# Wx-Alliance-Alliance-Meteo/paradis_model

Measured on AMD Instinct MI355X. Metric: training samples/sec (whole node) on 5.625° ERA5 grid, 1/2/4/8 MI355X, higher is better.
Workload: dtype f32; 1 GPU; era5_5.625deg_32x64_S1_B32; grid=32x64, rollout_steps=1, per_gpu_batch=32, global_batch=32, parameters=60038475, optimizer=adamw, parallelism=dp1, gemm_arithmetic=bf16x3, mode=train, hip_graph=False, activation_checkpointing=False

## Files before the change

include/paradis_hip.h:

```cpp
#ifndef PARADIS_HIP_H
#define PARADIS_HIP_H

#include <stddef.h>
#include <stdint.h>

#ifdef __cplusplus
extern "C" {
#endif

#define PARADIS_ACT_NONE 0
#define PARADIS_ACT_SILU 1
#define PARADIS_ACT_GELU 2
#define PARADIS_INTERP_BILINEAR 1
#define PARADIS_INTERP_BICUBIC 2
#define PARADIS_ADVECT_AUTO 0
#define PARADIS_ADVECT_GENERIC 1
#define PARADIS_ADVECT_TILED 2
#define PARADIS_ADVECT_SEPARABLE 4
#define PARADIS_ADVECT_TILES 8
#define PARADIS_ADVECT_STRIPS 16
#define PARADIS_ADVECT_HALO_SHIFT 8
#define PARADIS_ADVECT_HALO_BWD_SHIFT 16
#define PARADIS_ADVECT_HALO(h) (((h) + 1) << PARADIS_ADVECT_HALO_SHIFT)

int paradis_abi_version(void);
const char* paradis_last_error(void);

int paradis_geocyclic_pad_fwd(const float* x, float* y, int64_t planes, int H, int W, int p, void* stream);
int paradis_geocyclic_pad_bwd(const float* gy, float* gx, int64_t planes, int H, int W, int p, void* stream);

int paradis_sl_advect_fwd(const float* field, const float* u, const float* v, float* out,
                          const float* sin_lat, const float* cos_lat, const float* lat_cells, const float* lon,
                          int B, int K, int H, int W, int64_t f_bs, int64_t uv_bs, int64_t o_bs,
                          float dt, float min_lat, float min_lon, float d_lat, float d_lon,
                          int mode, int flags, void* workspace, void* stream);
size_t paradis_sl_advect_ws_bytes(int B, int K, int H, int W, int flags);
int paradis_sl_advect_bwd(const float* gout, const float* field, const float* u, const float* v,
                          float* gfield, float* gu, float* gv,
                          const float* sin_lat, const float* cos_lat, const float* lat_cells, const float* lon,
                          int B, int K, int H, int W, int64_t go_bs, int64_t f_bs, int64_t uv_bs,
                          int64_t gf_bs, int64_t guv_bs,
                          float dt, float min_lat, float min_lon, float d_lat, float d_lon,
                          int mode, int flags, void* workspace, void* stream);

int paradis_dwconv_geo_fwd(const float* x, const float* w, const float* bias, float* y,
                           int B, int C, int H, int W, int k, void* stream);
int paradis_dwconv_geo_dgrad(const float* gy, const float* w, float* gx,
                             int B, int C, int H, int W, int k, void* stream);
int paradis_dwconv_geo_dgrad_add(const float* gy, const float* w, const float* addend, float* gx,
                                 int B, int C, int H, int W, int k, void* stream);
int paradis_dwconv_geo_bwd(const float* gy, const float* x, const float* w, const float* addend, float* gx,
                           float* gw, float* gbias, int B, int C, int H, int W, int k, void* workspace, void* stream);
size_t paradis_dwconv_geo_wgrad_ws_bytes(int B, int C, int H, int W, int k);
int paradis_dwconv_geo_wgrad(const float* gy, const float* x, float* gw, float* gbias,
                             int B, int C, int H, int W, int k, void* workspace, void* stream);

int paradis_avgpool_geo_fwd(const float* x, float* y, int64_t planes, int H, int W, int stride, void* stream);
int paradis_avgpool_geo_bwd(const float* gy, float* gx, int64_t planes, int H, int W, int stride, void* stream);

int paradis_upsample_lonp_fwd(const float* x, float* y, int64_t planes, int Hc, int Wc, int H, int W, void* stream);
int paradis_upsample_lonp_bwd(const float* gy, float* gx, int64_t planes, int Hc, int Wc, int H, int W, void* stream);

#define PARADIS_GEMM_EXACT 0
#define PARADIS_GEMM_BF16 1
#define PARADIS_GEMM_F16X2 2
#define PARADIS_GEMM_BF16X3 3
#define PARADIS_AMAX_PARTIALS 1024
int paradis_amax_partials(const float* x, int B, int64_t inner, int64_t bs, uint32_t* partials, void* stream);
size_t paradis_pw_gemm_split_bytes(int M, int K, int scheme);
int paradis_pw_gemm_split_weights(const float* W, int M, int K, int transpose, int scheme, void* out, void* stream);
int paradis_pw_gemm_split_weights_pair(const float* W, int M, int K, void* out, void* out_t, void* stream);
int paradis_pw_gemm_split_weights_pair_scheme(const float* W, int M, int K, int scheme, void* out, void* out_t, void* stream);
int paradis_pw_gemm_fwd(const float* Wt, const float* WtT ,
                        const void* Wsplit ,
                        int scheme, const uint32_t* x_amax ,
                        const float* X, const float* bias, const float* map,
                        const float* m8 , const float* pwT , int cin,
                        const float* res, float* Y, float* zpre,
                        int B, int M, int K, int N, int64_t x_bs, int64_t res_bs, int64_t y_bs,
                        int act, void* stream);
int paradis_pw_gemm_fwd_gated(const float* Wt, const float* WtT, const void* Wsplit, int scheme, const uint32_t* x_amax,
                              const float* X, const float* bias, const float* map, const float* m8, const float* pwT,
                              int cin, const float* res, const float* gate, float* Y, float* zpre,
                              int B, int M, int K, int N, int64_t x_bs, int64_t res_bs, int64_t y_bs,
                              int act, void* stream);
int paradis_pw_gemm_dgrad(const float* Wt, const void* WTsplit, int scheme,
                          const uint32_t* dy_amax ,
                          const float* dY, const float* zpre,
                          const float* addend, float* dX, int B, int M, int K, int N, int64_t dy_bs,
                          int64_t z_bs, int64_t add_bs, int64_t dx_bs, int act, void* stream);
size_t paradis_pw_gemm_wgrad_ws_bytes(int B, int M, int K, int N);
int paradis_pw_gemm_wgrad_slabs(int B, int M, int K, int N);
int paradis_pw_gemm_wgrad(const float* dY, const float* X, float* dW, float* gbias,
                          int B, int M, int K, int N, int64_t dy_bs, int64_t x_bs, int scheme,
                          const uint32_t* dy_amax, const uint32_t* x_amax ,
                          void* workspace, void* stream);

#define PARADIS_IO_X16 1
#define PARADIS_IO_Y16 2
#define PARADIS_IO_Z16 4
#define PARADIS_IO_DY16 8
int paradis_pw_gemm_fwd16(const void* Wsplit, const void* X, const float* bias, const float* map, const float* m8,
                          const float* pwT, int cin, const float* res, const float* gate , void* Y,
                          void* zpre, int B, int M, int K, int N, int64_t x_bs, int64_t res_bs, int64_t y_bs, int act,
                          int io16, void* stream);
int paradis_pw_gemm_dgrad16(const void* WTsplit, const void* dY, const void* zpre, void* dX, int B, int M, int K, int N,
                            int64_t dy_bs, int64_t z_bs, int64_t dx_bs, int act, int io16, void* stream);
int paradis_pw_gemm_wgrad16(const void* dY, const void* X, float* dW, float* gbias, int B, int M, int K, int N,
                            int64_t dy_bs, int64_t x_bs, int io16, void* workspace, void* stream);
int paradis_channel_norm_fwd16(const float* x1, const float* x2, const float* w, const float* b, void* y ,
                               float* mean, float* rstd, int B, int C1, int C2, int P, int64_t x1_bs, int64_t x2_bs,
                               float eps, void* stream);
int paradis_dwconv_geo_fwd16(const float* x, const float* w, const float* bias, void* y , int B, int C, int H,
                             int W, int k, void* stream);
int paradis_channel_norm_bwd16_ok(int B, int C, int P);
int paradis_channel_norm_bwd16(const void* gy , const float* x1, const float* x2, const float* w, const float* mean,
                               const float* rstd, float* gx1, float* gx2, float* gw, float* gb, int B, int C1, int C2, int P,
                               int64_t x1_bs, int64_t x2_bs, int64_t gx1_bs, int64_t gx2_bs, const float* addend1,
                               int64_t add1_bs, void* workspace, void* stream);
int paradis_dwconv_geo_bwd16_ok(int H, int W, int k);
int paradis_dwconv_geo_bwd16(const void* gy , const float* x, const float* w, const float* addend, float* gx, float* gw,
                             float* gbias, int B, int C, int H, int W, int k, void* workspace, void* stream);
int paradis_act_bwd16(const float* gy, const float* x, void* gx , int64_t n, int act, void* stream);
int paradis_bias_grads16(const void* dz, float* gmap, float* gbias, int B, int C, int P, int64_t dz_bs, void* stream);

int paradis_channel_norm_fwd(const float* x1, const float* x2, const float* w, const float* b,
                             float* y, float* mean, float* rstd,
                             int B, int C1, int C2, int P, int64_t x1_bs, int64_t x2_bs,
                             float eps, void* stream);
size_t paradis_channel_norm_bwd_ws_bytes(int B, int C, int P);
int paradis_channel_norm_bwd(const float* gy, const float* x1, const float* x2, const float* w,
                             const float* mean, const float* rstd, float* gx1, float* gx2,
                             float* gw, float* gb, int B, int C1, int C2, int P,
                             int64_t x1_bs, int64_t x2_bs, int64_t gx1_bs, int64_t gx2_bs,
                             const float* addend1, int64_t add1_bs, void* workspace, void* stream);

int paradis_global_bias_map_fwd(const float* A, const float* U, const float* V, const float* Pw,
                                float* m8, float* map, int Cin, int Co, int R, int H, int W, void* stream);
size_t paradis_global_bias_map_bwd_ws_bytes(int Cin, int Co, int R, int H, int W);
int paradis_global_bias_map_bwd(const float* gmap, const float* A, const float* U, const float* V,
                                const float* Pw, const float* m8, float* gA, float* gU, float* gV,
                                float* gPw, int Cin, int Co, int R, int H, int W,
                                void* workspace, void* stream);

int paradis_global_bias_m8_fwd(const float* A, const float* U, const float* V, float* m8,
                               int Cin, int R, int H, int W, void* stream);
int paradis_global_bias_m8_bwd(const float* gm8, const float* A, const float* U, const float* V,
                               float* gA, float* gU, float* gV, int Cin, int R, int H, int W,
                               void* workspace, void* stream);
int paradis_global_bias_proj_bwd(const float* gmap, const float* m8, const float* Pw, float* gPw,
                                 float* gm8, int Cin, int Co, int64_t P, void* stream);

int paradis_act_fwd(const float* x, float* y, int64_t n, int act, void* stream);
int paradis_act_bwd(const float* gy, const float* x, float* gx, int64_t n, int act, void* stream);
int paradis_gated_blend_fwd(const float* h, const float* adv, const float* alpha, float* out,
                            int B, int C, int P, void* stream);
size_t paradis_gated_blend_bwd_ws_bytes(int B, int C, int P);
int paradis_gated_blend_bwd(const float* gout, const float* h, const float* adv, const float* alpha,
                            float* gh, float* gadv, float* galpha, int B, int C, int P,
                            void* workspace, void* stream);
int paradis_gated_blend_bwd_out(const float* gout, const float* h, const float* out, const float* alpha,
                                float* gh, float* gadv, float* galpha, int B, int C, int P,
                                void* workspace, void* stream);
int paradis_bias_grads(const float* dz, float* gmap, float* gbias, int B, int C, int P,
                       int64_t dz_bs, void* stream);
int paradis_add(const float* a, const float* b, float* y, int64_t n, void* stream);
int paradis_transpose(const float* in, float* out, int rows, int cols, void* stream);
int paradis_add_bcast(const float* x, const float* m, float* y, int64_t per_sample, int B, void* stream);

int paradis_loss_blocks(int64_t total);
int paradis_loss_fwd_bwd(const float* pred, const float* target, const float* wf, const float* wl,
                         float* loss, float* grad, float* partial, int B, int C, int H, int W,
                         int kind, float delta, void* stream);
int paradis_scale(const float* x, const float* scalar, float* y, int64_t n, void* stream);
int paradis_copy_channels(const float* src, int64_t src_bs, float* dst, int64_t dst_bs, int B,
                          int64_t per_sample, void* stream);
int paradis_adamw_step(float* p, const float* g, float* m, float* v, int64_t n, float lr, float beta1,
                       float beta2, float eps, float weight_decay, int step, void* stream);
int paradis_adamw_chunk(void);
int paradis_adamw_multi(const int64_t* ptrs, const int64_t* numel, const int* chunk_tensor,
                        const int64_t* chunk_off, int n_tensors, int n_chunks, float lr, float beta1,
                        float beta2, float eps, float weight_decay, int step, const int* dev_state, void* stream);
int paradis_adamw_tick(int* dev_state, void* stream);
int paradis_adamw_step_d(float* p, const float* g, float* m, float* v, int64_t n, double lr, double beta1,
                         double beta2, double eps, double weight_decay, int step, void* stream);
int paradis_adamw_multi_d(const int64_t* ptrs, const int64_t* numel, const int* chunk_tensor,
                          const int64_t* chunk_off, int n_tensors, int n_chunks, double lr, double beta1,
                          double beta2, double eps, double weight_decay, int step, const int* dev_state, void* stream);

size_t paradis_amse_table_floats(int H);
size_t paradis_amse_tables_ws_bytes(int H);
int paradis_amse_tables(float* leg, float* twiddle, double* ws, int H, int W, void* stream);
size_t paradis_amse_ws_bytes(int N, int H);
int paradis_amse_loss(const float* pred, const float* target, const float* leg, const float* twiddle, float* loss,
                      float* grad, void* ws, int N, int H, int W, void* stream);

size_t paradis_muon_ws_bytes(int T, int rows, int cols);
int paradis_muon_step(const int64_t* ptrs, int table_stride, int T, int rows, int cols, float lr,
                      float lr_adj, float mu, float beta2, float weight_decay, float eps, int nesterov,
                      int normuon, int split ,
                      void* workspace, void* stream);
int paradis_bgemm(const float* A, const float* AT, const float* B, float* C, int nbatch, int M, int K, int N,
                  int64_t a_bs, int64_t at_bs, int64_t b_bs, int64_t c_bs, void* split_ws, void* stream);

size_t paradis_forcings_ws_bytes(int B, int T);
int paradis_forcings(const int64_t* times_us , const double* lat_deg, const double* lon_deg,
                     int lat_is_f32, int B, int T, int H, int W, int n_time_inputs, const int* var_codes, int n_vars,
                     double toa_mean, double toa_std, float* out, void* workspace, void* stream);
int paradis_normalize_features(float* data, const int* kind, const float* p0, const float* p1,
                               int64_t rows, int C, float eps_q, int inverse, void* stream);

int paradis_forecast_post(const float* output, int64_t out_bs, float* chunk, int64_t chunk_bs, int64_t chunk_off,
                          float* dew, int64_t dew_bs, int64_t dew_off, const int* kind, const float* p0,
                          const float* p1, float eps_q, const int* units, int n_units, const double* plev,
                          int n_levels, const double* trig, int B, int C, int H, int W, void* stream);

size_t paradis_val_score_ws_bytes(int B, int C, int H, int W);
int paradis_val_score(const float* pred, int64_t pred_bs, const float* target, int64_t target_bs, const float* wf,
                      const float* wl, const float* lat_w, int kind, float delta, const int* rep_chan,
                      const int* rep_class, int R, const int* rflag, const int* rcls, const float* rp0,
                      const float* rp1, const int* rchan, float* out, void* workspace, int B, int C, int H, int W,
                      void* stream);

#ifdef __cplusplus
}
#endif
#endif
```

paradis_model_amd/_lib.py:

```python
from __future__ import annotations

import ctypes
import os
from ctypes import c_char_p, c_double, c_float, c_int, c_int64, c_size_t, c_void_p

import torch

_HERE = os.path.dirname(os.path.abspath(__file__))
LIB_PATH = os.environ.get("PARADIS_HIP_LIB") or os.path.join(_HERE, "libparadis_hip.so")

if not os.path.exists(LIB_PATH):
    raise ImportError(
        f"{LIB_PATH} not found: the HIP extension is not built. Run "
        "`python -c 'import __graft_entry__ as g; g.build()'` (or `make -C paradis_model_amd/csrc`). "
        "paradis_model_amd has no CPU/eager fallback by design.")

lib = ctypes.CDLL(LIB_PATH)

P, I, L, F, S, D = c_void_p, c_int, c_int64, c_float, c_size_t, c_double

SIGNATURES = {
    "paradis_abi_version": (I, []),
    "paradis_last_error": (c_char_p, []),
    "paradis_geocyclic_pad_fwd": (I, [P, P, L, I, I, I, P]),
    "paradis_geocyclic_pad_bwd": (I, [P, P, L, I, I, I, P]),
    "paradis_sl_advect_fwd": (I, [P, P, P, P, P, P, P, P, I, I, I, I, L, L, L, F, F, F, F, F, I, I, P, P]),
    "paradis_sl_advect_ws_bytes": (S, [I, I, I, I, I]),
    "paradis_sl_advect_bwd": (I, [P, P, P, P, P, P, P, P, P, P, P, I, I, I, I, L, L, L, L, L,
                                  F, F, F, F, F, I, I, P, P]),
    "paradis_dwconv_geo_fwd": (I, [P, P, P, P, I, I, I, I, I, P]),
    "paradis_dwconv_geo_dgrad": (I, [P, P, P, I, I, I, I, I, P]),
    "paradis_dwconv_geo_dgrad_add": (I, [P, P, P, P, I, I, I, I, I, P]),
    "paradis_dwconv_geo_bwd": (I, [P, P, P, P, P, P, P, I, I, I, I, I, P, P]),
    "paradis_dwconv_geo_wgrad_ws_bytes": (S, [I, I, I, I, I]),
    "paradis_dwconv_geo_wgrad": (I, [P, P, P, P, I, I, I, I, I, P, P]),
    "paradis_avgpool_geo_fwd": (I, [P, P, L, I, I, I, P]),
    "paradis_avgpool_geo_bwd": (I, [P, P, L, I, I, I, P]),
    "paradis_upsample_lonp_fwd": (I, [P, P, L, I, I, I, I, P]),
    "paradis_upsample_lonp_bwd": (I, [P, P, L, I, I, I, I, P]),
    "paradis_amax_partials": (I, [P, I, L, L, P, P]),
    "paradis_pw_gemm_split_bytes": (S, [I, I, I]),
    "paradis_pw_gemm_split_weights": (I, [P, I, I, I, I, P, P]),
    "paradis_pw_gemm_split_weights_pair": (I, [P, I, I, P, P, P]),
    "paradis_pw_gemm_split_weights_pair_scheme": (I, [P, I, I, I, P, P, P]),
    "paradis_pw_gemm_fwd": (I, [P, P, P, I, P, P, P, P, P, P, I, P, P, P, I, I, I, I, L, L, L, I, P]),
    "paradis_pw_gemm_fwd_gated": (I, [P, P, P, I, P, P, P, P, P, P, I, P, P, P, P, I, I, I, I, L, L, L, I, P]),
    "paradis_forcings_ws_bytes": (ctypes.c_size_t, [I, I]),
    "paradis_forcings": (I, [P, P, P, I, I, I, I, I, I, P, I, ctypes.c_double, ctypes.c_double, P, P, P]),
    "paradis_normalize_features": (I, [P, P, P, P, L, I, ctypes.c_float, I, P]),
    "paradis_global_bias_m8_fwd": (I, [P, P, P, P, I, I, I, I, P]),
    "paradis_global_bias_m8_bwd": (I, [P, P, P, P, P, P, P, I, I, I, I, P, P]),
    "paradis_global_bias_proj_bwd": (I, [P, P, P, P, P, I, I, L, P]),
    "paradis_transpose": (I, [P, P, I, I, P]),
    "paradis_pw_gemm_dgrad": (I, [P, P, I, P, P, P, P, P, I, I, I, I, L, L, L, L, I, P]),
    "paradis_pw_gemm_wgrad_ws_bytes": (S, [I, I, I, I]),
    "paradis_pw_gemm_wgrad_slabs": (I, [I, I, I, I]),
    "paradis_pw_gemm_wgrad": (I, [P, P, P, P, I, I, I, I, L, L, I, P, P, P, P]),
    "paradis_pw_gemm_fwd16": (I, [P, P, P, P, P, P, I, P, P, P, P, I, I, I, I, L, L, L, I, I, P]),
    "paradis_pw_gemm_dgrad16": (I, [P, P, P, P, I, I, I, I, L, L, L, I, I, P]),
    "paradis_pw_gemm_wgrad16": (I, [P, P, P, P, I, I, I, I, L, L, I, P, P]),
    "paradis_bias_grads16": (I, [P, P, P, I, I, I, L, P]),
    "paradis_channel_norm_fwd16": (I, [P, P, P, P, P, P, P, I, I, I, I, L, L, F, P]),
    "paradis_dwconv_geo_fwd16": (I, [P, P, P, P, I, I, I, I, I, P]),
    "paradis_channel_norm_bwd16_ok": (I, [I, I, I]),
    "paradis_channel_norm_bwd16": (I, [P, P, P, P, P, P, P, P, P, P, I, I, I, I, L, L, L, L, P, L, P, P]),
    "paradis_dwconv_geo_bwd16_ok": (I, [I, I, I]),
    "paradis_dwconv_geo_bwd16": (I, [P, P, P, P, P, P, P, I, I, I, I, I, P, P]),
    "paradis_channel_norm_fwd": (I, [P, P, P, P, P, P, P, I, I, I, I, L, L, F, P]),
    "paradis_channel_norm_bwd_ws_bytes": (S, [I, I, I]),
    "paradis_channel_norm_bwd": (I, [P, P, P, P, P, P, P, P, P, P, I, I, I, I, L, L, L, L, P, L, P, P]),
    "paradis_global_bias_map_fwd": (I, [P, P, P, P, P, P, I, I, I, I, I, P]),
    "paradis_global_bias_map_bwd_ws_bytes": (S, [I, I, I, I, I]),
    "paradis_global_bias_map_bwd": (I, [P, P, P, P, P, P, P, P, P, P, I, I, I, I, I, P, P]),
    "paradis_act_fwd": (I, [P, P, L, I, P]),
    "paradis_act_bwd": (I, [P, P, P, L, I, P]),
    "paradis_act_bwd16": (I, [P, P, P, L, I, P]),
    "paradis_gated_blend_fwd": (I, [P, P, P, P, I, I, I, P]),
    "paradis_gated_blend_bwd_ws_bytes": (S, [I, I, I]),
    "paradis_gated_blend_bwd": (I, [P, P, P, P, P, P, P, I, I, I, P, P]),
    "paradis_gated_blend_bwd_out": (I, [P, P, P, P, P, P, P, I, I, I, P, P]),
    "paradis_bias_grads": (I, [P, P, P, I, I, I, L, P]),
    "paradis_add": (I, [P, P, P, L, P]),
    "paradis_add_bcast": (I, [P, P, P, L, I, P]),
    "paradis_loss_blocks": (I, [L]),
    "paradis_loss_fwd_bwd": (I, [P, P, P, P, P, P, P, I, I, I, I, I, F, P]),
    "paradis_scale": (I, [P, P, P, L, P]),
    "paradis_copy_channels": (I, [P, L, P, L, I, L, P]),
    "paradis_adamw_step": (I, [P, P, P, P, L, F, F, F, F, F, I, P]),
    "paradis_muon_ws_bytes": (S, [I, I, I]),
    "paradis_muon_step": (I, [P, I, I, I, I, F, F, F, F, F, F, I, I, I, P, P]),
    "paradis_bgemm": (I, [P, P, P, P, I, I, I, I, L, L, L, L, P, P]),
    "paradis_adamw_chunk": (I, []),
    "paradis_adamw_multi": (I, [P, P, P, P, I, I, F, F, F, F, F, I, P, P]),
    "paradis_adamw_tick": (I, [P, P]),
    "paradis_adamw_step_d": (I, [P, P, P, P, L, D, D, D, D, D, I, P]),
    "paradis_adamw_multi_d": (I, [P, P, P, P, I, I, D, D, D, D, D, I, P, P]),
    "paradis_amse_table_floats": (S, [I]),
    "paradis_amse_tables_ws_bytes": (S, [I]),
    "paradis_amse_tables": (I, [P, P, P, I, I, P]),
    "paradis_amse_ws_bytes": (S, [I, I]),
    "paradis_amse_loss": (I, [P, P, P, P, P, P, P, I, I, I, P]),
    "paradis_forecast_post": (I, [P, L, P, L, L, P, L, L, P, P, P, F, P, I, P, I, P, I, I, I, I, P]),
    "paradis_val_score_ws_bytes": (S, [I, I, I, I]),
    "paradis_val_score": (I, [P, L, P, L, P, P, P, I, F, P, P, I, P, P, P, P, P, P, P, I, I, I, I, P]),
}

_missing = []
for _name, (_res, _args) in SIGNATURES.items():
    try:
        _fn = getattr(lib, _name)
    except AttributeError:
        _missing.append(_name)
        continue
    _fn.restype = _res
    _fn.argtypes = _args
if _missing and os.environ.get("PARADIS_DEV_PARTIAL") != "1":
    raise ImportError(f"{LIB_PATH} lacks symbols {_missing}; rebuild the HIP extension")


def last_error() -> str:
    msg = lib.paradis_last_error()
    return msg.decode() if msg else ""


def check(rc: int, name: str) -> None:
    if rc != 0:
        raise RuntimeError(f"{name} failed (code {rc}): {last_error()}")


def dptr(t):
    if t is None:
        return None
    return ctypes.c_void_p(t.data_ptr())


_raw_stream = getattr(torch._C, "_cuda_getCurrentRawStream", None)


def stream_ptr():
    if _raw_stream is not None:
        return ctypes.c_void_p(_raw_stream(torch.cuda.current_device()))
    return ctypes.c_void_p(torch.cuda.current_stream().cuda_stream)


def require_hip(*tensors, any_dtype: bool = False) -> None:
    for t in tensors:
        if t is None:
            continue
        if not t.is_cuda:
            raise RuntimeError("paradis_model_amd ops run on the MI355X only: got a CPU tensor "
                               "(there is no CPU fallback; use oracle/ for CPU checks)")
        if t.dtype != torch.float32 and not any_dtype:
            raise RuntimeError(f"paradis_model_amd ops are fp32; got {t.dtype}")


class LaunchProfiler:

    def __init__(self):
        self.records = {}

    def add(self, name, work, ev0, ev1):
        rec = self.records.setdefault(name, [0.0, []])
        rec[0] += work
        rec[1].append((ev0, ev1))

    def summary(self):
        out = {}
        for name, (work, evs) in self.records.items():
            ms = sum(a.elapsed_time(b) for a, b in evs)
            out[name] = {"launches": len(evs), "work": work, "ms": ms}
        return out


PROFILER = None


def call(name: str, work: float, *args, symbol: str = None) -> None:
    fn = getattr(lib, "paradis_" + (symbol or name))
    prof = PROFILER
    if prof is None:
        check(fn(*args), name)
        return
    ev0 = torch.cuda.Event(enable_timing=True)
    ev1 = torch.cuda.Event(enable_timing=True)
    ev0.record()
    rc = fn(*args)
    ev1.record()
    check(rc, name)
    prof.add(name, work, ev0, ev1)
```

paradis_model_amd/csrc/gemm.hip:

```cpp
#include <algorithm>
#include <cstdlib>
#include "gemm_common.h"


namespace {

constexpr int ld_of(bool kc) { return kc ? BM + 1 : BM + 4; }
constexpr int stage_floats(int bk) { return bk * (BM + 4); }
constexpr size_t lds_bytes(int bk) { return (size_t)4 * stage_floats(bk) * sizeof(float); }
constexpr int nv_of(int bk) { return BM * bk / (256 * 4); }

int g_bk = 16;
int g_wg_per_cu = 4;
int g_stagger = 0;
int g_dma_stages = 3;
int g_wgrad_dma_stages = 2;


template <bool KC, int BK>
__device__ __forceinline__ void slab_load(const float* __restrict__ base, int64_t ld, int row0,
                                          int k0, int rows, int K, bool vec_ok,
                                          float4 (&r)[nv_of(BK)]) {
  constexpr int NV = nv_of(BK);
  constexpr int TPR = BK / 4;
// ... 208 lines not shown
    float a0 = As[0], a1 = As[32], b0 = Bs[0], b1 = Bs[32];
#pragma unroll
    for (int kk = 0; kk < DBK / 2; ++kk) {
      float na0 = 0.f, na1 = 0.f, nb0 = 0.f, nb1 = 0.f;
      if (kk + 1 < DBK / 2) {
        na0 = As[(2 * kk + 2) * BM]; na1 = As[(2 * kk + 2) * BM + 32];
        nb0 = Bs[(2 * kk + 2) * BN]; nb1 = Bs[(2 * kk + 2) * BN + 32];
      }
      acc[0][0] = __builtin_amdgcn_mfma_f32_32x32x2f32(a0, b0, acc[0][0], 0, 0, 0);
      acc[0][1] = __builtin_amdgcn_mfma_f32_32x32x2f32(a0, b1, acc[0][1], 0, 0, 0);
      acc[1][0] = __builtin_amdgcn_mfma_f32_32x32x2f32(a1, b0, acc[1][0], 0, 0, 0);
      acc[1][1] = __builtin_amdgcn_mfma_f32_32x32x2f32(a1, b1, acc[1][1], 0, 0, 0);
      a0 = na0; a1 = na1; b0 = nb0; b1 = nb1;
    }
  }
  gemm_epilogue(g, acc, bz, m0, n0, wm, wn, li, lh);
}

template <int S>
__global__ void __launch_bounds__(256, 4)
pw_gemm_wgrad_dma_kernel(GemmArgs g) {
  extern __shared__ __attribute__((aligned(16))) float lds[];
  const int tid = threadIdx.x, lane = tid & 63, wave = tid >> 6;
  const int wm = wave >> 1, wn = wave & 1;
  const int li = lane & 31, lh = lane >> 5;

  const int MT = (g.M + BM - 1) / BM, NT = (g.N + BN - 1) / BN;
  int L;
  {
    const int nwg = gridDim.x, id = blockIdx.x;
    const int q = nwg >> 3, r = nwg & 7, xcd = id & 7;
    L = (xcd < r ? xcd * (q + 1) : r * (q + 1) + (xcd - r) * q) + (id >> 3);
  }
  const int mt = L % MT, nt = (L / MT) % NT, bz = L / (MT * NT);
  const int m0 = mt * BM, n0 = nt * BN;
  const int KT = g.K / DBK;
  const int64_t total = (int64_t)g.inner * KT;
  const int t_begin = (int)(total * bz / g.nbatch);
  const int T = (int)(total * (bz + 1) / g.nbatch) - t_begin;

  const int prow = lane >> 2, pslot = lane & 3;
  const int chunk = pslot ^ ((prow >> 2) & 3);
  const int ra0 = min(m0 + 16 * (2 * wave) + prow, g.M - 1), ra1 = min(m0 + 16 * (2 * wave + 1) + prow, g.M - 1);
  const int rb0 = min(n0 + 16 * (2 * wave) + prow, g.N - 1), rb1 = min(n0 + 16 * (2 * wave + 1) + prow, g.N - 1);
  const float* pa0 = g.A + (int64_t)ra0 * g.lda + 4 * chunk;
  const float* pa1 = g.A + (int64_t)ra1 * g.lda + 4 * chunk;
  const float* pb0 = g.B + (int64_t)rb0 * g.ldb + 4 * chunk;
  const float* pb1 = g.B + (int64_t)rb1 * g.ldb + 4 * chunk;

  auto issue = [&](int t) {
    const int tt = t_begin + t;
    const int ib = tt / KT, kt = tt - ib * KT;
    const int64_t oa = (int64_t)ib * g.a_is + (int64_t)kt * DBK, ob = (int64_t)ib * g.b_is + (int64_t)kt * DBK;
    float* st = lds + (t % S) * (2 * DTILE);
    float* la = st + (2 * wave) * 256;
    float* lb = st + DTILE + (2 * wave) * 256;
    __builtin_amdgcn_global_load_lds((gbl_ptr_t)(pa0 + oa), (lds_ptr_t)la, 16, 0, 0);
    __builtin_amdgcn_global_load_lds((gbl_ptr_t)(pa1 + oa), (lds_ptr_t)(la + 256), 16, 0, 0);
    __builtin_amdgcn_global_load_lds((gbl_ptr_t)(pb0 + ob), (lds_ptr_t)lb, 16, 0, 0);
    __builtin_amdgcn_global_load_lds((gbl_ptr_t)(pb1 + ob), (lds_ptr_t)(lb + 256), 16, 0, 0);
  };

  f32x16 acc[2][2];
#pragma unroll
  for (int i = 0; i < 2; ++i)
#pragma unroll
    for (int j = 0; j < 2; ++j)
#pragma unroll
      for (int r = 0; r < 16; ++r) acc[i][j][r] = 0.f;

#pragma unroll
  for (int t = 0; t < S - 1; ++t)
    if (t < T) issue(t);

  const bool do_rowsum = g.rowsum != nullptr && nt == 0;
  float rs = 0.f;
  const int rs_off = (tid >> 1) * DBK + (tid & 1) * 8;

  const int sw = (li >> 2) & 3;
  const int offA = (wm * 64 + li) * DBK, offB = DTILE + (wn * 64 + li) * DBK;
  const int s0 = ((0 + lh) ^ sw) * 4, s1 = ((2 + lh) ^ sw) * 4;

  for (int t = 0; t < T; ++t) {
    const int pending = min(S - 2, T - 1 - t);
    if (pending >= 2) asm volatile("s_waitcnt vmcnt(8)\n\ts_barrier" ::: "memory");
    else if (pending == 1) asm volatile("s_waitcnt vmcnt(4)\n\ts_barrier" ::: "memory");
    else asm volatile("s_waitcnt vmcnt(0)\n\ts_barrier" ::: "memory");
    if (t + S - 1 < T) issue(t + S - 1);
    const float* st = lds + (t % S) * (2 * DTILE);
    if (do_rowsum) {
      const float4 q0 = *reinterpret_cast<const float4*>(st + rs_off);
      const float4 q1 = *reinterpret_cast<const float4*>(st + rs_off + 4);
      rs += ((q0.x + q0.y) + (q0.z + q0.w)) + ((q1.x + q1.y) + (q1.z + q1.w));
    }
    const float4 a00 = *reinterpret_cast<const float4*>(st + offA + s0);
    const float4 a10 = *reinterpret_cast<const float4*>(st + offA + 32 * DBK + s0);
    const float4 b00 = *reinterpret_cast<const float4*>(st + offB + s0);
    const float4 b10 = *reinterpret_cast<const float4*>(st + offB + 32 * DBK + s0);
    const float4 a01 = *reinterpret_cast<const float4*>(st + offA + s1);
    const float4 a11 = *reinterpret_cast<const float4*>(st + offA + 32 * DBK + s1);
    const float4 b01 = *reinterpret_cast<const float4*>(st + offB + s1);
    const float4 b11 = *reinterpret_cast<const float4*>(st + offB + 32 * DBK + s1);
#define MFMA4(A0, A1, B0, B1)                                                       \
    acc[0][0] = __builtin_amdgcn_mfma_f32_32x32x2f32(A0, B0, acc[0][0], 0, 0, 0);   \
    acc[0][1] = __builtin_amdgcn_mfma_f32_32x32x2f32(A0, B1, acc[0][1], 0, 0, 0);   \
    acc[1][0] = __builtin_amdgcn_mfma_f32_32x32x2f32(A1, B0, acc[1][0], 0, 0, 0);   \
    acc[1][1] = __builtin_amdgcn_mfma_f32_32x32x2f32(A1, B1, acc[1][1], 0, 0, 0);
    MFMA4(a00.x, a10.x, b00.x, b10.x)
    MFMA4(a00.y, a10.y, b00.y, b10.y)
    MFMA4(a00.z, a10.z, b00.z, b10.z)
    MFMA4(a00.w, a10.w, b00.w, b10.w)
    MFMA4(a01.x, a11.x, b01.x, b11.x)
    MFMA4(a01.y, a11.y, b01.y, b11.y)
    MFMA4(a01.z, a11.z, b01.z, b11.z)
    MFMA4(a01.w, a11.w, b01.w, b11.w)
#undef MFMA4
  }
  if (do_rowsum) {
    rs += __shfl_xor(rs, 1, 64);
    const int m = m0 + (tid >> 1);
    if ((tid & 1) == 0 && m < g.M) g.rowsum[(int64_t)bz * g.M + m] = rs;
  }
  gemm_epilogue(g, acc, bz, m0, n0, wm, wn, li, lh);
}

constexpr int SIMG = simg(3);

__global__ void __launch_bounds__(256)
amax_partials_kernel(const float* __restrict__ x, int B, int64_t inner, int64_t bs, int vec, uint32_t* __restrict__ out) {
  uint32_t m = 0;
  if (vec) {
    const int64_t n4 = inner >> 2, total = n4 * B;
    for (int64_t i = (int64_t)blockIdx.x * 256 + threadIdx.x; i < total; i += (int64_t)gridDim.x * 256) {
      const int64_t b = i / n4, j = i - b * n4;
      const uint4 q = *reinterpret_cast<const uint4*>(x + b * bs + 4 * j);
      m = max(max(m, q.x & 0x7fffffffu), max(q.y & 0x7fffffffu, max(q.z & 0x7fffffffu, q.w & 0x7fffffffu)));
    }
  } else {
    const int64_t total = inner * B;
    for (int64_t i = (int64_t)blockIdx.x * 256 + threadIdx.x; i < total; i += (int64_t)gridDim.x * 256) {
      const int64_t b = i / inner, j = i - b * inner;
      m = max(m, __float_as_uint(x[b * bs + j]) & 0x7fffffffu);
    }
  }
  m = wave_umax_lane63(m);
  __shared__ uint32_t red[4];
  if ((threadIdx.x & 63) == 63) red[threadIdx.x >> 6] = m;
  __syncthreads();
  if (threadIdx.x == 0) out[blockIdx.x] = max(max(red[0], red[1]), max(red[2], red[3]));
}


template <int NP = 3>
__device__ __forceinline__ void split_weights_body(const float* __restrict__ Wb, int64_t rs, int64_t cs, int M, int K,
                                                   int KT, int64_t units, u32x4* __restrict__ ob) {
  for (int64_t u = (int64_t)blockIdx.x * 256 + threadIdx.x; u < units; u += (int64_t)gridDim.x * 256) {
    const int row = (int)(u & 127), half = (int)((u >> 7) & 1);
    const int64_t tile = u >> 8;
    const int kt = (int)(tile % KT), mt = (int)(tile / KT);
    const int m = mt * BM + row;
    float x[8];
#pragma unroll
    for (int j = 0; j < 8; ++j) {
      const int k = kt * SBK + half * 8 + j;
      x[j] = (m < M && k < K) ? Wb[(int64_t)m * rs + (int64_t)k * cs] : 0.f;
      if (SPLIT_SIGNED && (row & 32)) x[j] = -x[j];
    }
    if constexpr (NP == 3) {
      u32x4 h, mm, l;
      split8(x, h, mm, l);
      u32x4* o = ob + tile * SIMG + half * SCH + row;
      o[0] = h; o[2 * SCH] = mm; o[4 * SCH] = l;
    } else {
      ob[tile * simg(1) + half * SCH + row] = round8(x);
    }
  }
}

template <int NP>
__global__ void __launch_bounds__(256)
split_weights_kernel(const float* __restrict__ W, int64_t rs, int64_t cs, int M, int K, int KT, int64_t units,
                     int64_t w_bs, int64_t out_bs, u32x4* __restrict__ out) {
  split_weights_body<NP>(W + (int64_t)blockIdx.y * w_bs, rs, cs, M, K, KT, units, out + (int64_t)blockIdx.y * out_bs);
}

template <int NP>
__global__ void __launch_bounds__(256)
split_weights_pair_kernel(const float* __restrict__ W, int M, int K, int KT, int KTt, int64_t units, int64_t units_t,
                          u32x4* __restrict__ out, u32x4* __restrict__ out_t) {
  if (blockIdx.y == 0) split_weights_body<NP>(W, K, 1, M, K, KT, units, out);
  else split_weights_body<NP>(W, 1, K, K, M, KTt, units_t, out_t);
}

__global__ void __launch_bounds__(256)
split_weights_f16_kernel(const float* __restrict__ W, int64_t rs, int64_t cs, int M, int K, int KT, int64_t units,
                         u32x4* __restrict__ out, uint32_t* __restrict__ tail) {
  const uint32_t amax = reduce_amax_partials(tail + 4);
  if (blockIdx.x == 0 && threadIdx.x == 0) tail[0] = amax;
  float sc, inv;
  scale_from_amax(amax, sc, inv);
  for (int64_t u = (int64_t)blockIdx.x * 256 + threadIdx.x; u < units; u += (int64_t)gridDim.x * 256) {
    const int row = (int)(u & 127), half = (int)((u >> 7) & 1);
    const int64_t tile = u >> 8;
    const int kt = (int)(tile % KT), mt = (int)(tile / KT);
    const int m = mt * BM + row;
    float x[8];
#pragma unroll
    for (int j = 0; j < 8; ++j) {
      const int k = kt * SBK + half * 8 + j;
      x[j] = (m < M && k < K) ? W[(int64_t)m * rs + (int64_t)k * cs] : 0.f;
    }
    u32x4 h, l;
    split8_f16(x, (SPLIT_SIGNED && (row & 32)) ? -sc : sc, h, l);
    u32x4* o = out + tile * simg(2) + half * SCH + row;
    o[0] = h; o[2 * SCH] = l;
  }
}

#ifndef SPLIT_ASTAGES_F16
#define SPLIT_ASTAGES_F16 2
#endif
constexpr int split_astages(int np) { return np == 2 ? SPLIT_ASTAGES_F16 : 2; }
template <int NP>
__global__ void __launch_bounds__(256, 3)
pw_gemm_split_kernel(GemmArgs g) {
  extern __shared__ __attribute__((aligned(16))) float lds[];
  constexpr int SIMG = simg(NP);
  u32x4* img = reinterpret_cast<u32x4*>(lds);
  constexpr int SA = split_astages(NP), DA = SA - 1;
  const int tid = threadIdx.x, lane = tid & 63, wave = tid >> 6;
  const int wm = wave >> 1, wn = wave & 1;
  const int li = lane & 31, lh = lane >> 5;

  const int MT = (g.M + BM - 1) / BM, NT = (g.N + BN - 1) / BN;
  int L;
  {
    const int nwg = gridDim.x, id = blockIdx.x;
    const int q = nwg >> 3, r = nwg & 7, xcd = id & 7;
    L = (xcd < r ? xcd * (q + 1) : r * (q + 1) + (xcd - r) * q) + (id >> 3);
  }
  const int mt = L % MT, nt = (L / MT) % NT, bz = L / (MT * NT);
  const int m0 = mt * BM, n0 = nt * BN;
  const int T = (g.K + SBK - 1) / SBK;

  const u32x4* Ag = reinterpret_cast<const u32x4*>(g.A) + (int64_t)bz * g.a_bs + (int64_t)mt * T * SIMG + tid;
  const int bh = __builtin_amdgcn_readfirstlane(tid >> 7);
  const float* Bb;
  {
    const uint64_t a = reinterpret_cast<uint64_t>(g.B + (int64_t)bz * g.b_bs);
    const uint32_t lo = __builtin_amdgcn_readfirstlane((uint32_t)a), hi = __builtin_amdgcn_readfirstlane((uint32_t)(a >> 32));
    Bb = reinterpret_cast<const float*>(((uint64_t)hi << 32) | lo);
  }
  const int bn = min(n0 + (tid & 127), g.N - 1);

  float sc_b = 1.f, inv_a = 1.f, inv_b = 1.f;
  if constexpr (NP == 2) {
    float sc_a;
    scale_from_amax(reduce_amax_partials(g.b_amax), sc_b, inv_b);
    scale_from_amax(g.a_amax[0], sc_a, inv_a);
  }

  const uint32_t flip = split_flip_mask(tid & 127);
  if constexpr (NP == 2) sc_b = __uint_as_float(__float_as_uint(sc_b) ^ flip);
  float xb[2][8] = {};
  auto issueA = [&](int t) __attribute__((always_inline)) {
    const u32x4* a = Ag + (int64_t)t * SIMG;
    u32x4* la = img + (2 + t % SA) * SIMG + wave * 64;
#pragma unroll
    for (int i = 0; i < NP; ++i)
      __builtin_amdgcn_global_load_lds((gbl_ptr_t)(a + i * 256), (lds_ptr_t)(la + i * 256), 16, 0, 0);
  };
  auto split_store = [&](const float (&x)[8], u32x4* o) __attribute__((always_inline)) {
    if constexpr (NP == 3) {
      u32x4 h, m, l;
      float xs[8];
      flip8(xs, x, flip);
      split8(xs, h, m, l);
      o[0] = h; o[2 * SCH] = m; o[4 * SCH] = l;
    } else {
      u32x4 h, l;
      split8_f16(x, sc_b, h, l);
      o[0] = h; o[2 * SCH] = l;
    }
  };
  const uint32_t boff = (uint32_t)bn * 4u;
  auto fetchB = [&](int t, float (&x)[8]) __attribute__((always_inline)) {
    const int k0 = t * SBK + bh * 8;
    const float* p = Bb + (int64_t)min(k0, g.K - 1) * g.ldb;
#pragma unroll
    for (int j = 0; j < 8; ++j) {
      asm volatile("global_load_dword %0, %1, %2" : "=&v"(x[j]) : "v"(boff), "s"(p) : "memory");
      p += (k0 + j + 1 < g.K) ? g.ldb : 0;
    }
  };
#define USE_X(x, N) do { asm volatile("s_waitcnt vmcnt(" #N ")" :: "v"(x[0]), "v"(x[1]), "v"(x[2]), "v"(x[3]), \
                                      "v"(x[4]), "v"(x[5]), "v"(x[6]), "v"(x[7]) : "memory");                  \
                         __builtin_amdgcn_sched_barrier(0); } while (0)
  u32x4* const Bst = img + bh * SCH + (tid & 127);

  f32x16 acc[2][2];
#pragma unroll
  for (int i = 0; i < 2; ++i)
#pragma unroll
    for (int j = 0; j < 2; ++j)
#pragma unroll
      for (int r = 0; r < 16; ++r) acc[i][j][r] = 0.f;

  for (int u = 0; u < DA && u < T; ++u) issueA(u);
  fetchB(0, xb[0]);
  USE_X(xb[0], 0);
  if (T > 1) fetchB(1, xb[1]);
  split_store(xb[0], Bst);
  if (T > 1) asm volatile("s_waitcnt vmcnt(8) lgkmcnt(0)\n\ts_barrier" ::: "memory");
  else asm volatile("s_waitcnt vmcnt(0) lgkmcnt(0)\n\ts_barrier" ::: "memory");
  auto step = [&](int t, int cur, float (&xload)[8], float (&xsplit)[8]) __attribute__((always_inline)) {
    const u32x4* As = img + (2 + t % SA) * SIMG + lh * SCH + wm * 64 + li;
    const u32x4* Bs = img + cur * SIMG + lh * SCH + wn * 64 + li;
    const bool dmaA = t + DA < T, ldB = t + 2 < T;
    if (dmaA) issueA(t + DA);
    if (ldB) fetchB(t + 2, xload);
    if (dmaA && ldB) { if constexpr (NP == 3) USE_X(xsplit, 11); else USE_X(xsplit, 10); }
    else if (ldB) USE_X(xsplit, 8);
    else USE_X(xsplit, 0);
    SplitFrags<NP> f;
    split_tile_read<NP, 2 * SCH, 2 * SCH>(As, Bs, f);
    split_tile_mfma<NP>(f, acc);
    split_store(xsplit, Bst + (cur ^ 1) * SIMG);
    __builtin_amdgcn_sched_group_barrier(0x100, 4 * NP, 0);
#pragma unroll
// ... 293 lines not shown
  return 0;
}

template <bool A_KC, bool B_KC>
int launch_gemm(const GemmArgs& g, int grid, hipStream_t st) {
  return g_bk == 32 ? launch_gemm_bk<A_KC, B_KC, 32>(g, grid, st)
                    : launch_gemm_bk<A_KC, B_KC, 16>(g, grid, st);
}

constexpr size_t split_lds(int np) { return (size_t)(2 + split_astages(np)) * simg(np) * 16; }
constexpr size_t split_lds_wgrad(int np) { return (size_t)2 * 2 * simgp(np) * 16; }
constexpr int AMAX_WORDS = PARADIS_AMAX_PARTIALS;
constexpr size_t F16_TAIL_BYTES = 16 + (size_t)AMAX_WORDS * 4;

int split_image_ktiles(int K, int np) {
  const int kt = (K + SBK - 1) / SBK;
  return np == 1 ? (kt + 1) & ~1 : kt;
}
int64_t split_image_chunks(int M, int K, int np = 3) {
  return (int64_t)((M + BM - 1) / BM) * split_image_ktiles(K, np) * simg(np);
}

bool known_scheme(int scheme) {
  return scheme == PARADIS_GEMM_EXACT || scheme == PARADIS_GEMM_BF16X3 || scheme == PARADIS_GEMM_F16X2 ||
         scheme == PARADIS_GEMM_BF16;
}

int launch_amax(const float* x, int B, int64_t inner, int64_t bs, uint32_t* out, hipStream_t st) {
  const int vec = (inner % 4 == 0) && (bs % 4 == 0) && ((reinterpret_cast<uintptr_t>(x) & 15) == 0);
  hipLaunchKernelGGL(amax_partials_kernel, dim3(AMAX_WORDS), dim3(256), 0, st, x, B, inner, bs, vec, out);
  return 0;
}

template <int NP>
int launch_split_np(const GemmArgs& d, hipStream_t st) {
  const int grid = ((d.M + BM - 1) / BM) * ((d.N + BN - 1) / BN) * d.nbatch;
  static PerDeviceOnce once;
  if (split_lds(NP) > 64 * 1024)
    if (int e = reserve_lds(once, {&pw_gemm_split_kernel<NP>}, split_lds(NP), "pw_gemm(split)")) return e;
  hipLaunchKernelGGL(pw_gemm_split_kernel<NP>, dim3(grid), dim3(256), split_lds(NP), st, d);
  return 0;
}
constexpr size_t split_wide_lds(int nsub, int np = 2) { return (size_t)(2 * nsub + 2) * simg(np) * 16; }
constexpr int SPLIT_WIDE_NSUB = 2;
#ifndef SPLIT_WIDE_BF16X3
#define SPLIT_WIDE_BF16X3 1
#endif
template <int NP>
int launch_split_wide(const GemmArgs& d, int NT, hipStream_t st) {
  constexpr int NSUB = SPLIT_WIDE_NSUB;
  static PerDeviceOnce once;
  if (split_wide_lds(NSUB, NP) > 64 * 1024)
    if (int e = reserve_lds(once, {&pw_gemm_split_wide_kernel<NSUB, NP>}, split_wide_lds(NSUB, NP), "pw_gemm(split)")) return e;
  const int grid = ((d.M + BM - 1) / BM) * ((NT + NSUB - 1) / NSUB) * d.nbatch;
  hipLaunchKernelGGL((pw_gemm_split_wide_kernel<NSUB, NP>), dim3(grid), dim3(256 * NSUB), split_wide_lds(NSUB, NP), st, d);
  return 0;
}
int launch_split(const GemmArgs& d, int scheme, hipStream_t st) {
  const int NT = (d.N + BN - 1) / BN;
  if (scheme == PARADIS_GEMM_BF16) return pd_amp_launch_fwd(d, st);
  if (scheme != PARADIS_GEMM_F16X2) {
#if SPLIT_WIDE_BF16X3
    if (NT >= 2) return launch_split_wide<3>(d, NT, st);
#endif
    return launch_split_np<3>(d, st);
  }
  if (NT < 2) return launch_split_np<2>(d, st);
  return launch_split_wide<2>(d, NT, st);
}

int check_gemm(const char* name, int B, int M, int K, int N) {
  PD_REQUIRE(B >= 0 && M >= 1 && K >= 1 && N >= 1, "%s: bad shape B=%d M=%d K=%d N=%d", name, B, M, K, N);
  const int64_t tiles = (int64_t)((M + BM - 1) / BM) * ((N + BN - 1) / BN) * std::max(B, 1);
  PD_REQUIRE(tiles < (1ll << 31), "%s: too many tiles", name);
  return 0;
}

}

#ifdef PARADIS_DEV_KNOBS
extern "C" void paradis_debug_set_gemm(int bk, int wg_per_cu) {
  if (bk == 16 || bk == 32) g_bk = bk;
  if (wg_per_cu >= 1 && wg_per_cu <= 4) g_wg_per_cu = wg_per_cu;
}
extern "C" void paradis_debug_set_gemm_stagger(int units) { g_stagger = units < 0 ? 0 : units; }
extern "C" void paradis_debug_set_gemm_dma(int stages) { g_dma_stages = stages < 2 ? 0 : (stages > 4 ? 4 : stages); }
extern "C" void paradis_debug_set_wgrad_dma(int stages) { g_wgrad_dma_stages = stages < 2 ? 0 : (stages > 3 ? 3 : stages); }
#endif

extern "C" size_t paradis_pw_gemm_split_bytes(int M, int K, int scheme) {
  if (M < 1 || K < 1) return 0;
  if (scheme == PARADIS_GEMM_F16X2) return (size_t)split_image_chunks(M, K, 2) * 16 + F16_TAIL_BYTES;
  if (scheme == PARADIS_GEMM_BF16) return (size_t)split_image_chunks(M, K, 1) * 16;
  return scheme == PARADIS_GEMM_BF16X3 ? (size_t)split_image_chunks(M, K, 3) * 16 : 0;
}

extern "C" int paradis_amax_partials(const float* x, int B, int64_t inner, int64_t bs, uint32_t* partials,
                                     void* stream) {
  PD_REQUIRE(partials != nullptr && B >= 0 && inner >= 0 && (x != nullptr || B == 0 || inner == 0),
             "amax_partials: bad arguments");
  launch_amax(x, B, inner, bs, partials, (hipStream_t)stream);
  PD_CHECK_LAUNCH("amax_partials");
  return 0;
}

extern "C" int paradis_pw_gemm_split_weights(const float* W, int M, int K, int transpose, int scheme, void* out,
                                             void* stream) {
  PD_REQUIRE(W != nullptr && out != nullptr && M >= 1 && K >= 1, "pw_gemm_split_weights: bad arguments");
  PD_REQUIRE(scheme == PARADIS_GEMM_BF16X3 || scheme == PARADIS_GEMM_F16X2 || scheme == PARADIS_GEMM_BF16,
             "pw_gemm_split_weights: unknown scheme %d", scheme);
  const int AM = transpose ? K : M, AK = transpose ? M : K;
  const int KT = split_image_ktiles(AK, scheme == PARADIS_GEMM_BF16 ? 1 : 3);
  const int64_t units = (int64_t)((AM + BM - 1) / BM) * KT * 256;
  const int blocks = (int)std::min<int64_t>((units + 255) / 256, 4096);
  if (scheme == PARADIS_GEMM_F16X2) {
    uint32_t* tail = reinterpret_cast<uint32_t*>((char*)out + (size_t)split_image_chunks(AM, AK, 2) * 16);
    launch_amax(W, 1, (int64_t)M * K, 0, tail + 4, (hipStream_t)stream);
    hipLaunchKernelGGL(split_weights_f16_kernel, dim3(blocks), dim3(256), 0, (hipStream_t)stream, W,
                       (int64_t)(transpose ? 1 : K), (int64_t)(transpose ? K : 1), AM, AK, KT, units, (u32x4*)out, tail);
  } else if (scheme == PARADIS_GEMM_BF16) {
    hipLaunchKernelGGL(split_weights_kernel<1>, dim3(blocks, 1), dim3(256), 0, (hipStream_t)stream, W,
                       (int64_t)(transpose ? 1 : K), (int64_t)(transpose ? K : 1), AM, AK, KT, units,
                       (int64_t)0, (int64_t)0, (u32x4*)out);
  } else {
    hipLaunchKernelGGL(split_weights_kernel<3>, dim3(blocks, 1), dim3(256), 0, (hipStream_t)stream, W,
                       (int64_t)(transpose ? 1 : K), (int64_t)(transpose ? K : 1), AM, AK, KT, units,
                       (int64_t)0, (int64_t)0, (u32x4*)out);
  }
  PD_CHECK_LAUNCH("pw_gemm_split_weights");
  return 0;
}

extern "C" int paradis_pw_gemm_split_weights_pair_scheme(const float* W, int M, int K, int scheme, void* out, void* out_t,
                                                         void* stream) {
  PD_REQUIRE(W != nullptr && out != nullptr && out_t != nullptr && out != out_t && M >= 1 && K >= 1,
             "pw_gemm_split_weights_pair: bad arguments");
  PD_REQUIRE(scheme == PARADIS_GEMM_BF16X3 || scheme == PARADIS_GEMM_BF16,
             "pw_gemm_split_weights_pair: scheme %d has no paired images", scheme);
  const int np = scheme == PARADIS_GEMM_BF16 ? 1 : 3;
  const int KT = split_image_ktiles(K, np), KTt = split_image_ktiles(M, np);
  const int64_t units = (int64_t)((M + BM - 1) / BM) * KT * 256, units_t = (int64_t)((K + BM - 1) / BM) * KTt * 256;
  const int blocks = (int)std::min<int64_t>((std::max(units, units_t) + 255) / 256, 4096);
  if (scheme == PARADIS_GEMM_BF16X3)
    hipLaunchKernelGGL(split_weights_pair_kernel<3>, dim3(blocks, 2), dim3(256), 0, (hipStream_t)stream, W, M, K, KT, KTt,
                       units, units_t, (u32x4*)out, (u32x4*)out_t);
  else
    hipLaunchKernelGGL(split_weights_pair_kernel<1>, dim3(blocks, 2), dim3(256), 0, (hipStream_t)stream, W, M, K, KT, KTt,
                       units, units_t, (u32x4*)out, (u32x4*)out_t);
  PD_CHECK_LAUNCH("pw_gemm_split_weights_pair");
  return 0;
}
extern "C" int paradis_pw_gemm_split_weights_pair(const float* W, int M, int K, void* out, void* out_t, void* stream) {
  return paradis_pw_gemm_split_weights_pair_scheme(W, M, K, PARADIS_GEMM_BF16X3, out, out_t, stream);
}

namespace {
int run_split(GemmArgs d, const void* img, int AM, int AK, int scheme, const uint32_t* b_amax, const char* what,
              hipStream_t st) {
  d.A = (const float*)img; d.a_bs = 0;
  if (scheme == PARADIS_GEMM_F16X2) {
    if (b_amax == nullptr) { paradis_set_error(what); return 1; }
    d.a_amax = reinterpret_cast<const uint32_t*>((const char*)img + (size_t)split_image_chunks(AM, AK, 2) * 16);
    d.b_amax = b_amax;
  }
  return launch_split(d, scheme, st);
}
int check_io16(const char* name, int io16, int scheme, const void* Bop, int64_t b_bs, int N, bool has_res) {
  if (io16 == 0) return 0;
  PD_REQUIRE(scheme == PARADIS_GEMM_BF16, "%s: bf16-stored tensors need the PARADIS_GEMM_BF16 scheme", name);
  PD_REQUIRE((io16 & ~(IO_B16 | IO_C16 | IO_ZM16 | IO_A16)) == 0, "%s: unknown io16 bits %d", name, io16);
  PD_REQUIRE(!(io16 & IO_C16) || !has_res, "%s: a bf16 output cannot carry the fp32 residual", name);
  if (io16 & IO_B16)
    PD_REQUIRE(N % 8 == 0 && N >= 8 && b_bs % 8 == 0 && (reinterpret_cast<uintptr_t>(Bop) & 15) == 0,
               "%s: a bf16 activation operand needs N %% 8 == 0 and 16-byte aligned planes", name);
  return 0;
}
}

static int pw_gemm_fwd_impl(const float* Wt, const float* WtT, const void* Wsplit, int scheme,
                            const uint32_t* x_amax, const float* X,
                            const float* bias, const float* map, const float* m8,
                            const float* pwT, int cin, const float* res, const float* gate, float* Y, float* zpre,
                            int B, int M, int K, int N, int64_t x_bs, int64_t res_bs,
                            int64_t y_bs, int act, void* stream, int io16 = 0) {
  if (int e = check_gemm("pw_gemm_fwd", B, M, K, N)) return e;
  if (int e = check_io16("pw_gemm_fwd", io16, scheme, X, x_bs, N, res != nullptr)) return e;
  PD_REQUIRE(gate == nullptr || res != nullptr || B == 0, "pw_gemm_fwd: a gate needs the tensor it blends with (res)");
  PD_REQUIRE(act >= 0 && act <= 2, "pw_gemm_fwd: unknown activation code %d", act);
  PD_REQUIRE(known_scheme(scheme) && (Wsplit != nullptr) == (scheme != PARADIS_GEMM_EXACT),
             "pw_gemm_fwd: scheme %d needs %s weight image", scheme, scheme ? "a" : "no");
  PD_REQUIRE((m8 == nullptr) == (pwT == nullptr) && (pwT == nullptr || (cin >= 1 && M % 4 == 0)),
             "pw_gemm_fwd: projected bias needs m8, pwT, cin >= 1 and M %% 4 == 0");
  if (B == 0) return 0;
  GemmArgs g{};
  g.m8 = m8; g.pw = pwT; g.cin = cin;
  g.A = Wt; g.B = X; g.C = Y; g.M = M; g.N = N; g.K = K;
  g.lda = K; g.ldb = N; g.ldc = N;
  g.a_bs = 0; g.b_bs = x_bs; g.c_bs = y_bs; g.nbatch = B; g.inner = 0;
  g.bias = bias; g.map = map; g.res = res; g.res_bs = res_bs; g.zmul = nullptr; g.zout = zpre;
  g.zout_bs = (int64_t)M * N; g.act = act; g.gate = gate;
  g.stagger = g_stagger;
  g.io16 = io16;
  const int grid = ((M + BM - 1) / BM) * ((N + BN - 1) / BN) * B;
  if (Wsplit != nullptr) {
    if (int e = run_split(g, Wsplit, M, K, scheme, x_amax, "pw_gemm_fwd: the f16x2 scheme needs x_amax",
                          (hipStream_t)stream)) return e;
    PD_CHECK_LAUNCH("pw_gemm_fwd(split)");
    return 0;
  }
  if (WtT != nullptr) {
    GemmArgs d = g;
    d.A = WtT; d.lda = M;
    if (dma_eligible(d)) {
      launch_gemm_dma(d, grid, (hipStream_t)stream);
      PD_CHECK_LAUNCH("pw_gemm_fwd(dma)");
      return 0;
    }
  }
  if (int e = launch_gemm<true, false>(g, grid, (hipStream_t)stream)) return e;
  PD_CHECK_LAUNCH("pw_gemm_fwd");
  return 0;
}

extern "C" int paradis_pw_gemm_fwd(const float* Wt, const float* WtT, const void* Wsplit, int scheme,
                                   const uint32_t* x_amax, const float* X,
                                   const float* bias, const float* map, const float* m8,
                                   const float* pwT, int cin, const float* res, float* Y, float* zpre,
                                   int B, int M, int K, int N, int64_t x_bs, int64_t res_bs,
                                   int64_t y_bs, int act, void* stream) {
  return pw_gemm_fwd_impl(Wt, WtT, Wsplit, scheme, x_amax, X, bias, map, m8, pwT, cin, res, nullptr, Y, zpre, B, M, K, N,
                          x_bs, res_bs, y_bs, act, stream);
}

extern "C" int paradis_pw_gemm_fwd_gated(const float* Wt, const float* WtT, const void* Wsplit, int scheme,
                                         const uint32_t* x_amax, const float* X,
                                         const float* bias, const float* map, const float* m8,
                                         const float* pwT, int cin, const float* res, const float* gate, float* Y,
                                         float* zpre, int B, int M, int K, int N, int64_t x_bs, int64_t res_bs,
                                         int64_t y_bs, int act, void* stream) {
  PD_REQUIRE(gate != nullptr && (res != nullptr || B == 0), "pw_gemm_fwd_gated: gate [M] and res required");
  return pw_gemm_fwd_impl(Wt, WtT, Wsplit, scheme, x_amax, X, bias, map, m8, pwT, cin, res, gate, Y, zpre, B, M, K, N,
                          x_bs, res_bs, y_bs, act, stream);
}

extern "C" int paradis_pw_gemm_fwd16(const void* Wsplit, const void* X, const float* bias, const float* map,
                                     const float* m8, const float* pwT, int cin, const float* res, const float* gate,
                                     void* Y, void* zpre, int B, int M, int K, int N, int64_t x_bs, int64_t res_bs,
                                     int64_t y_bs, int act, int io16, void* stream) {
  PD_REQUIRE((io16 & ~(IO_B16 | IO_C16)) == 0, "pw_gemm_fwd16: io16 may name X (1) and Y (2)");
  PD_REQUIRE(Wsplit != nullptr, "pw_gemm_fwd16: weight image required");
  return pw_gemm_fwd_impl(nullptr, nullptr, Wsplit, PARADIS_GEMM_BF16, nullptr, (const float*)X, bias, map, m8, pwT, cin,
                          res, gate, (float*)Y, (float*)zpre, B, M, K, N, x_bs, res_bs, y_bs, act, stream, io16);
}

extern "C" int paradis_bgemm(const float* A, const float* AT, const float* Bm, float* C, int nbatch, int M,
                             int K, int N, int64_t a_bs, int64_t at_bs, int64_t b_bs, int64_t c_bs,
                             void* split_ws, void* stream) {
  PD_REQUIRE(nbatch >= 0 && M >= 1 && K >= 1 && N >= 1, "bgemm: bad shape");
  if (nbatch == 0) return 0;
  GemmArgs g{};
  g.A = A; g.B = Bm; g.C = C; g.M = M; g.N = N; g.K = K;
  g.lda = K; g.ldb = N; g.ldc = N;
  g.a_bs = a_bs; g.b_bs = b_bs; g.c_bs = c_bs; g.nbatch = nbatch; g.inner = 0;
  g.stagger = g_stagger;
  const int64_t tiles = (int64_t)((M + BM - 1) / BM) * ((N + BN - 1) / BN) * nbatch;
  PD_REQUIRE(tiles < (1ll << 31), "bgemm: too many tiles");
  const int grid = (int)tiles;
  if (split_ws != nullptr) {
    PD_REQUIRE(nbatch <= 65535, "bgemm: too many batches for the split path");
    const int KT = (K + SBK - 1) / SBK;
    const int64_t chunks = split_image_chunks(M, K), units = (int64_t)((M + BM - 1) / BM) * KT * 256;
    const int blocks = (int)std::min<int64_t>((units + 255) / 256, 1024);
    hipLaunchKernelGGL(split_weights_kernel<3>, dim3(blocks, nbatch), dim3(256), 0, (hipStream_t)stream, A,
                       (int64_t)K, (int64_t)1, M, K, KT, units, a_bs, chunks, (u32x4*)split_ws);
    GemmArgs d = g;
    d.A = (const float*)split_ws; d.a_bs = chunks;
    if (int e = launch_split(d, PARADIS_GEMM_BF16X3, (hipStream_t)stream)) return e;
    PD_CHECK_LAUNCH("bgemm(split)");
    return 0;
  }
  if (AT != nullptr) {
    GemmArgs d = g;
    d.A = AT; d.lda = M; d.a_bs = at_bs;
    if (dma_eligible(d)) {
      launch_gemm_dma(d, grid, (hipStream_t)stream);
      PD_CHECK_LAUNCH("bgemm(dma)");
      return 0;
    }
  }
  if (int e = launch_gemm<true, false>(g, grid, (hipStream_t)stream)) return e;
  PD_CHECK_LAUNCH("bgemm");
  return 0;
}

static int pw_gemm_dgrad_impl(const float* Wt, const void* WTsplit, int scheme, const uint32_t* dy_amax,
                              const float* dY, const float* zpre,
                              const float* addend, float* dX, int B, int M, int K, int N,
                              int64_t dy_bs, int64_t z_bs, int64_t add_bs, int64_t dx_bs,
                              int act, void* stream, int io16) {
  if (int e = check_gemm("pw_gemm_dgrad", B, K, M, N)) return e;
  if (int e = check_io16("pw_gemm_dgrad", io16, scheme, dY, dy_bs, N, addend != nullptr)) return e;
  PD_REQUIRE(act >= 0 && act <= 2, "pw_gemm_dgrad: unknown activation code %d", act);
  PD_REQUIRE(known_scheme(scheme) && (WTsplit != nullptr) == (scheme != PARADIS_GEMM_EXACT),
             "pw_gemm_dgrad: scheme %d needs %s weight image", scheme, scheme ? "a" : "no");
  if (B == 0) return 0;
  GemmArgs g{};
// ... 144 lines not shown
```

paradis_model_amd/csrc/misc.hip:

```cpp
#include <algorithm>
#include "common.h"

namespace {

inline int stream_blocks(int64_t n_items) {
  return (int)std::max<int64_t>(1, std::min<int64_t>((n_items + 255) / 256, 256 * 16));
}

__global__ void __launch_bounds__(256)
gbias_m8_kernel(const float* __restrict__ A, const float* __restrict__ U, const float* __restrict__ V,
                float* __restrict__ m8, int Cin, int R, int H, int W) {
  __shared__ float part[4][64];
  const int tx = threadIdx.x & 63, q = threadIdx.x >> 6;
  const int w = min(blockIdx.x * 64 + tx, W - 1), h = blockIdx.y, c = blockIdx.z;
  const int rq = (R + 3) / 4, r1 = min(R, (q + 1) * rq);
  float acc = 0.f;
  int r = q * rq;
  for (; r + 8 <= r1; r += 8) {
    float a[8], u[8], v[8];
#pragma unroll
    for (int j = 0; j < 8; ++j) { a[j] = A[c * R + r + j]; u[j] = U[(r + j) * H + h]; v[j] = V[(r + j) * W + w]; }
#pragma unroll
    for (int j = 0; j < 8; ++j) acc += a[j] * u[j] * v[j];
  }
  for (; r < r1; ++r) acc += A[c * R + r] * U[r * H + h] * V[r * W + w];
  part[q][tx] = acc;
  __syncthreads();
  if (q == 0 && blockIdx.x * 64 + tx < W)
    m8[((int64_t)c * H + h) * W + w] = ((part[0][tx] + part[1][tx]) + part[2][tx]) + part[3][tx];
}

constexpr int GM8_MAXR = 256;
template <int ROWS>
__global__ void __launch_bounds__(256)
gbias_m8_rows_kernel(const float* __restrict__ A, const float* __restrict__ U, const float* __restrict__ V,
                     float* __restrict__ m8, int Cin, int R, int H, int W) {
  __shared__ float part[4][ROWS][64];
  __shared__ float coef[GM8_MAXR][ROWS];
  const int tx = threadIdx.x & 63, q = threadIdx.x >> 6;
  const int w = min(blockIdx.x * 64 + tx, W - 1), h0 = blockIdx.y * ROWS, c = blockIdx.z;
  for (int i = threadIdx.x; i < R * ROWS; i += 256) {
    const int r = i / ROWS, j = i - r * ROWS;
    coef[r][j] = A[c * R + r] * U[r * H + min(h0 + j, H - 1)];
  }
  __syncthreads();
  const int rq = (R + 3) / 4, r1 = min(R, (q + 1) * rq);
  float acc[ROWS];
#pragma unroll
  for (int j = 0; j < ROWS; ++j) acc[j] = 0.f;
  int r = q * rq;
  for (; r + 8 <= r1; r += 8) {
    float v[8];
#pragma unroll
    for (int k = 0; k < 8; ++k) v[k] = V[(r + k) * W + w];
#pragma unroll
    for (int k = 0; k < 8; ++k)
#pragma unroll
      for (int j = 0; j < ROWS; ++j) acc[j] += coef[r + k][j] * v[k];
  }
  for (; r < r1; ++r) {
    const float v = V[r * W + w];
#pragma unroll
    for (int j = 0; j < ROWS; ++j) acc[j] += coef[r][j] * v;
  }
#pragma unroll
  for (int j = 0; j < ROWS; ++j) part[q][j][tx] = acc[j];
  __syncthreads();
  if (q == 0 && blockIdx.x * 64 + tx < W) {
#pragma unroll
    for (int j = 0; j < ROWS; ++j)
      if (h0 + j < H)
        m8[((int64_t)c * H + h0 + j) * W + w] = ((part[0][j][tx] + part[1][j][tx]) + part[2][j][tx]) + part[3][j][tx];
  }
}

__global__ void __launch_bounds__(256)
small_mix_kernel(const float* __restrict__ Wm, int ldo, int ldc, const float* __restrict__ in,
                 float* __restrict__ out, int Cout, int Cin, int64_t P) {
  const int64_t p = (int64_t)blockIdx.x * 256 + threadIdx.x;
  const int o = blockIdx.y;
  if (p >= P) return;
  float acc = 0.f;
  for (int c = 0; c < Cin; ++c) acc += Wm[(int64_t)o * ldo + (int64_t)c * ldc] * in[(int64_t)c * P + p];
  out[(int64_t)o * P + p] = acc;
}

constexpr int GM8_SLICES = 16;
#ifndef GM8_BATCH
#define GM8_BATCH 16
#endif
template <int CIN>
__global__ void __launch_bounds__(64 * GM8_SLICES)
gbias_gm8_kernel(const float* __restrict__ Pw, const float* __restrict__ gmap, float* __restrict__ gm8,
                 int Cin, int Co, int64_t P) {
  __shared__ float part[GM8_SLICES][CIN][64];
  const int px = threadIdx.x & 63;
  const int slice = __builtin_amdgcn_readfirstlane(threadIdx.x >> 6);
  const int64_t p = (int64_t)blockIdx.x * 64 + px;
  const int64_t pc = min(p, P - 1);
  const int per = (Co + GM8_SLICES - 1) / GM8_SLICES, o0 = slice * per, o1 = min(o0 + per, Co);
  float acc[CIN];
#pragma unroll
  for (int c = 0; c < CIN; ++c) acc[c] = 0.f;
  int o = o0;
  for (; o + GM8_BATCH <= o1; o += GM8_BATCH) {
    float g[GM8_BATCH];
#pragma unroll
    for (int j = 0; j < GM8_BATCH; ++j) g[j] = gmap[(int64_t)(o + j) * P + pc];
#pragma unroll
    for (int j = 0; j < GM8_BATCH; ++j)
#pragma unroll
      for (int c = 0; c < CIN; ++c)
        if (c < Cin) acc[c] += Pw[(int64_t)(o + j) * Cin + c] * g[j];
  }
  for (; o + 8 <= o1; o += 8) {
    float g[8];
#pragma unroll
    for (int j = 0; j < 8; ++j) g[j] = gmap[(int64_t)(o + j) * P + pc];
#pragma unroll
    for (int j = 0; j < 8; ++j)
#pragma unroll
      for (int c = 0; c < CIN; ++c)
        if (c < Cin) acc[c] += Pw[(int64_t)(o + j) * Cin + c] * g[j];
  }
  for (; o < o1; ++o) {
    const float g = gmap[(int64_t)o * P + pc];
#pragma unroll
    for (int c = 0; c < CIN; ++c)
      if (c < Cin) acc[c] += Pw[(int64_t)o * Cin + c] * g;
  }
#pragma unroll
  for (int c = 0; c < CIN; ++c) part[slice][c][px] = acc[c];
  __syncthreads();
  if (slice < Cin && p < P) {
    float s = 0.f;
#pragma unroll
    for (int k = 0; k < GM8_SLICES; ++k) s += part[k][slice][px];
    gm8[(int64_t)slice * P + p] = s;
  }
}

__global__ void __launch_bounds__(256)
gbias_gpw_kernel(const float* __restrict__ gmap, const float* __restrict__ m8,
                 float* __restrict__ gPw, int Cin, int64_t P) {
  __shared__ float red[4];
  const int o = blockIdx.x / Cin, c = blockIdx.x - o * Cin;
  float acc = 0.f;
  for (int64_t p = threadIdx.x; p < P; p += 256) acc += gmap[(int64_t)o * P + p] * m8[(int64_t)c * P + p];
  acc = wave_sum(acc);
  if ((threadIdx.x & 63) == 0) red[threadIdx.x >> 6] = acc;
  __syncthreads();
  if (threadIdx.x == 0) gPw[blockIdx.x] = red[0] + red[1] + red[2] + red[3];
}

template <int RW, int CIN>
__global__ void __launch_bounds__(256)
gbias_gpw_rows_kernel(const float* __restrict__ gmap, const float* __restrict__ m8, float* __restrict__ gPw, int Cin,
                      int Co, int64_t P4) {
  __shared__ float red[4][RW * CIN];
  const int o0 = blockIdx.x * RW;
  float acc[RW][CIN];
#pragma unroll
  for (int j = 0; j < RW; ++j)
#pragma unroll
    for (int c = 0; c < CIN; ++c) acc[j][c] = 0.f;
  const float4* g4 = reinterpret_cast<const float4*>(gmap);
  const float4* m4 = reinterpret_cast<const float4*>(m8);
  for (int64_t q = threadIdx.x; q < P4; q += 256) {
    float4 m[CIN], g[RW];
#pragma unroll
    for (int c = 0; c < CIN; ++c) m[c] = m4[(int64_t)min(c, Cin - 1) * P4 + q];
#pragma unroll
    for (int j = 0; j < RW; ++j) g[j] = g4[(int64_t)min(o0 + j, Co - 1) * P4 + q];
#pragma unroll
    for (int j = 0; j < RW; ++j)
#pragma unroll
      for (int c = 0; c < CIN; ++c)
        acc[j][c] += (g[j].x * m[c].x + g[j].y * m[c].y) + (g[j].z * m[c].z + g[j].w * m[c].w);
  }
  const int lane = threadIdx.x & 63, wave = threadIdx.x >> 6;
#pragma unroll
  for (int j = 0; j < RW; ++j)
#pragma unroll
    for (int c = 0; c < CIN; ++c) {
      const float sum = wave_sum_dpp(acc[j][c]);
      if (lane == 0) red[wave][j * CIN + c] = sum;
    }
  __syncthreads();
  if (threadIdx.x < RW * CIN) {
    const int j = threadIdx.x / CIN, c = threadIdx.x - j * CIN;
    if (o0 + j < Co && c < Cin)
      gPw[(int64_t)(o0 + j) * Cin + c] = (red[0][threadIdx.x] + red[1][threadIdx.x]) + (red[2][threadIdx.x] + red[3][threadIdx.x]);
  }
}

__global__ void __launch_bounds__(256)
gbias_t1_kernel(const float* __restrict__ gm8, const float* __restrict__ V, float* __restrict__ T1,
                int Cin, int R, int H, int W) {
  const int64_t wid = ((int64_t)blockIdx.x * 256 + threadIdx.x) >> 6;
  if (wid >= (int64_t)Cin * R * H) return;
  const int h = (int)(wid % H), r = (int)((wid / H) % R), c = (int)(wid / ((int64_t)H * R));
  float acc = 0.f;
  for (int w = threadIdx.x & 63; w < W; w += 64) acc += gm8[((int64_t)c * H + h) * W + w] * V[r * W + w];
  acc = wave_sum(acc);
  if ((threadIdx.x & 63) == 0) T1[wid] = acc;
}

__global__ void __launch_bounds__(256)
gbias_t2_kernel(const float* __restrict__ gm8, const float* __restrict__ U, float* __restrict__ T2,
                int Cin, int R, int H, int W) {
  const int64_t total = (int64_t)Cin * R * W;
  for (int64_t idx = (int64_t)blockIdx.x * 256 + threadIdx.x; idx < total;
       idx += (int64_t)gridDim.x * 256) {
    const int w = (int)(idx % W), r = (int)((idx / W) % R), c = (int)(idx / ((int64_t)W * R));
    float acc = 0.f;
    for (int h = 0; h < H; ++h) acc += gm8[((int64_t)c * H + h) * W + w] * U[r * H + h];
    T2[idx] = acc;
  }
}

__global__ void __launch_bounds__(256)
gbias_finish_kernel(const float* __restrict__ T1, const float* __restrict__ T2,
                    const float* __restrict__ A, const float* __restrict__ U,
                    float* __restrict__ gA, float* __restrict__ gU, float* __restrict__ gV, int Cin,
                    int R, int H, int W) {
  const int nA = Cin * R, nU = R * H, nV = R * W;
  const int wavesA = (nA + 3) / 4;
  if ((int)blockIdx.x < wavesA) {
    const int idx = blockIdx.x * 4 + (threadIdx.x >> 6), lane = threadIdx.x & 63;
    if (idx >= nA) return;
    const int c = idx / R, r = idx - c * R;
    float acc = 0.f;
    for (int h = lane; h < H; h += 64) acc += T1[((int64_t)c * R + r) * H + h] * U[r * H + h];
    acc = wave_sum_dpp(acc);
    if (lane == 0) gA[idx] = acc;
    return;
  }
  const int idx = ((int)blockIdx.x - wavesA) * 256 + threadIdx.x;
  if (idx < nU) {
    const int r = idx / H, h = idx - r * H;
    float acc = 0.f;
    for (int c = 0; c < Cin; ++c) acc += T1[((int64_t)c * R + r) * H + h] * A[c * R + r];
    gU[idx] = acc;
  } else if (idx < nU + nV) {
    const int j = idx - nU, r = j / W, w = j - r * W;
    float acc = 0.f;
    for (int c = 0; c < Cin; ++c) acc += T2[((int64_t)c * R + r) * W + w] * A[c * R + r];
    gV[j] = acc;
  }
}

template <bool BWD, bool O16 = false>
__global__ void __launch_bounds__(256)
act_kernel(const float* __restrict__ gy, const float* __restrict__ x, float* __restrict__ out,
           int64_t n, int act, bool vec) {
  if constexpr (O16) {
    const int64_t n4 = n >> 2;
    for (int64_t i = (int64_t)blockIdx.x * 256 + threadIdx.x; i < n4; i += (int64_t)gridDim.x * 256) {
      const float4 v = reinterpret_cast<const float4*>(x)[i], g = reinterpret_cast<const float4*>(gy)[i];
      const float o[4] = {g.x * act_grad(v.x, act), g.y * act_grad(v.y, act), g.z * act_grad(v.z, act), g.w * act_grad(v.w, act)};
      uint2 r;
      r.x = (uint32_t)__builtin_bit_cast(uint16_t, (__bf16)o[0]) | ((uint32_t)__builtin_bit_cast(uint16_t, (__bf16)o[1]) << 16);
      r.y = (uint32_t)__builtin_bit_cast(uint16_t, (__bf16)o[2]) | ((uint32_t)__builtin_bit_cast(uint16_t, (__bf16)o[3]) << 16);
      reinterpret_cast<uint2*>(out)[i] = r;
    }
    return;
  }
  if (vec) {
    const int64_t n4 = n >> 2;
    for (int64_t i = (int64_t)blockIdx.x * 256 + threadIdx.x; i < n4; i += (int64_t)gridDim.x * 256) {
      const float4 v = reinterpret_cast<const float4*>(x)[i];
      float4 o;
      if (BWD) {
        const float4 g = reinterpret_cast<const float4*>(gy)[i];
        o = make_float4(g.x * act_grad(v.x, act), g.y * act_grad(v.y, act), g.z * act_grad(v.z, act),
                        g.w * act_grad(v.w, act));
      } else {
        o = make_float4(act_apply(v.x, act), act_apply(v.y, act), act_apply(v.z, act), act_apply(v.w, act));
      }
      reinterpret_cast<float4*>(out)[i] = o;
    }
  } else {
    for (int64_t i = (int64_t)blockIdx.x * 256 + threadIdx.x; i < n; i += (int64_t)gridDim.x * 256) {
      const float o = BWD ? gy[i] * act_grad(x[i], act) : act_apply(x[i], act);
      out[i] = o;
    }
  }
}

__global__ void __launch_bounds__(256)
add_kernel(const float* __restrict__ a, const float* __restrict__ b, float* __restrict__ y, int64_t n,
           bool vec) {
  if (vec) {
    const int64_t n4 = n >> 2;
    for (int64_t i = (int64_t)blockIdx.x * 256 + threadIdx.x; i < n4; i += (int64_t)gridDim.x * 256) {
      const float4 u = reinterpret_cast<const float4*>(a)[i], v = reinterpret_cast<const float4*>(b)[i];
      reinterpret_cast<float4*>(y)[i] = make_float4(u.x + v.x, u.y + v.y, u.z + v.z, u.w + v.w);
    }
  } else {
    for (int64_t i = (int64_t)blockIdx.x * 256 + threadIdx.x; i < n; i += (int64_t)gridDim.x * 256)
      y[i] = a[i] + b[i];
  }
}

__global__ void __launch_bounds__(256)
add_bcast_kernel(const float* __restrict__ x, const float* __restrict__ m, float* __restrict__ y,
                 int64_t per, int64_t total) {
  for (int64_t i = (int64_t)blockIdx.x * 256 + threadIdx.x; i < total; i += (int64_t)gridDim.x * 256)
    y[i] = x[i] + m[i % per];
}

__global__ void __launch_bounds__(256)
transpose_kernel(const float* __restrict__ in, float* __restrict__ out, int rows, int cols) {
  __shared__ float tile[32][33];
  const int tx = threadIdx.x & 31, ty = threadIdx.x >> 5;
  const int c0 = blockIdx.x * 32, r0 = blockIdx.y * 32;
  for (int i = ty; i < 32; i += 8)
    if (r0 + i < rows && c0 + tx < cols) tile[i][tx] = in[(int64_t)(r0 + i) * cols + c0 + tx];
  __syncthreads();
  for (int i = ty; i < 32; i += 8)
    if (c0 + i < cols && r0 + tx < rows) out[(int64_t)(c0 + i) * rows + r0 + tx] = tile[tx][i];
}

__global__ void __launch_bounds__(256)
gated_blend_fwd_kernel(const float* __restrict__ h, const float* __restrict__ adv,
                       const float* __restrict__ alpha, float* __restrict__ out, int C, int P) {
  const int c = blockIdx.x % C;
  const float g = 1.0f / (1.0f + expf(-alpha[c]));
  const int64_t base = (int64_t)blockIdx.x * P;
  for (int p = threadIdx.x; p < P; p += 256) {
    const float hv = h[base + p];
    out[base + p] = fmaf(g, adv[base + p] - hv, hv);
  }
}

__global__ void __launch_bounds__(256)
gated_blend_bwd_kernel(const float* __restrict__ gout, const float* __restrict__ h,
                       const float* __restrict__ adv, const float* __restrict__ alpha,
                       float* __restrict__ gh, float* __restrict__ gadv, float* __restrict__ partial,
                       int C, int P) {
  __shared__ float red[4];
  const int c = blockIdx.x % C;
  const float g = 1.0f / (1.0f + expf(-alpha[c]));
  const int64_t base = (int64_t)blockIdx.x * P;
  float acc = 0.f;
  for (int p = threadIdx.x; p < P; p += 256) {
    const float go = gout[base + p];
    gh[base + p] = (1.0f - g) * go;
    gadv[base + p] = g * go;
    acc += go * (adv[base + p] - h[base + p]);
  }
  acc = wave_sum(acc);
  if ((threadIdx.x & 63) == 0) red[threadIdx.x >> 6] = acc;
  __syncthreads();
  if (threadIdx.x == 0) partial[blockIdx.x] = red[0] + red[1] + red[2] + red[3];
}

__global__ void __launch_bounds__(256)
gated_blend_finish(const float* __restrict__ partial, const float* __restrict__ alpha,
                   float* __restrict__ galpha, int B, int C, int from_out) {
  const int c = blockIdx.x * 256 + threadIdx.x;
  if (c >= C) return;
  float s = 0.f;
  for (int b = 0; b < B; ++b) s += partial[(int64_t)b * C + c];
  const float g = 1.0f / (1.0f + expf(-alpha[c]));
  galpha[c] = from_out ? s * (1.0f - g) : s * g * (1.0f - g);
}

__global__ void __launch_bounds__(256)
bias_grads_kernel(const float* __restrict__ dz, float* __restrict__ gmap, float* __restrict__ gbias,
                  int B, int C, int P, int64_t bs, int pchunks) {
  __shared__ float red[4];
  const int c = blockIdx.x / pchunks, chunk = blockIdx.x - c * pchunks;
  float acc = 0.f;
  for (int p = chunk * 256 + threadIdx.x; p < P; p += pchunks * 256) {
    float s = 0.f;
    for (int b = 0; b < B; ++b) s += dz[(int64_t)b * bs + (int64_t)c * P + p];
    if (gmap) gmap[(int64_t)c * P + p] = s;
    acc += s;
  }
  if (!gbias) return;
  acc = wave_sum(acc);
  if ((threadIdx.x & 63) == 0) red[threadIdx.x >> 6] = acc;
  __syncthreads();
  if (threadIdx.x == 0) atomicAdd(&gbias[c], red[0] + red[1] + red[2] + red[3]);
}

__global__ void __launch_bounds__(256)
bias_grads_vec4_kernel(const float* __restrict__ dz, float* __restrict__ gmap, float* __restrict__ gbias,
                       int B, int C, int P4, int64_t bs, int pchunks) {
  __shared__ float red[4];
  const int c = blockIdx.x / pchunks, chunk = blockIdx.x - c * pchunks;
  const float4* src = reinterpret_cast<const float4*>(dz + (int64_t)c * P4 * 4);
  const int64_t bs4 = bs / 4;
  float acc = 0.f;
  for (int q = chunk * 256 + threadIdx.x; q < P4; q += pchunks * 256) {
    float4 s = {0.f, 0.f, 0.f, 0.f};
    int b = 0;
    for (; b + 8 <= B; b += 8) {
      float4 v[8];
#pragma unroll
      for (int j = 0; j < 8; ++j) v[j] = src[(int64_t)(b + j) * bs4 + q];
#pragma unroll
      for (int j = 0; j < 8; ++j) { s.x += v[j].x; s.y += v[j].y; s.z += v[j].z; s.w += v[j].w; }
    }
    for (; b < B; ++b) {
      const float4 v = src[(int64_t)b * bs4 + q];
      s.x += v.x; s.y += v.y; s.z += v.z; s.w += v.w;
    }
    if (gmap) reinterpret_cast<float4*>(gmap + (int64_t)c * P4 * 4)[q] = s;
    acc += (s.x + s.y) + (s.z + s.w);
  }
  if (!gbias) return;
  acc = wave_sum_dpp(acc);
  if ((threadIdx.x & 63) == 0) red[threadIdx.x >> 6] = acc;
  __syncthreads();
  if (threadIdx.x == 0) atomicAdd(&gbias[c], red[0] + red[1] + red[2] + red[3]);
}

bool aligned16(const void* p) { return (reinterpret_cast<uintptr_t>(p) & 15) == 0; }

void launch_gm8(const float* Pw, const float* gmap, float* gm8, int Cin, int Co, int64_t P, hipStream_t st) {
  const dim3 grid((unsigned)((P + 63) / 64)), block(64 * GM8_SLICES);
  if (Cin <= 8) hipLaunchKernelGGL(gbias_gm8_kernel<8>, grid, block, 0, st, Pw, gmap, gm8, Cin, Co, P);
  else hipLaunchKernelGGL(gbias_gm8_kernel<16>, grid, block, 0, st, Pw, gmap, gm8, Cin, Co, P);
}
#ifndef GBIAS_GPW_ROWS
#define GBIAS_GPW_ROWS 1
#endif
#ifndef GBIAS_GPW_ROWS_MINP
#define GBIAS_GPW_ROWS_MINP 2048
#endif
void launch_gpw(const float* gmap, const float* m8, float* gPw, int Cin, int Co, int64_t P, hipStream_t st) {
  if (GBIAS_GPW_ROWS && Cin <= 8 && P % 4 == 0 && P >= GBIAS_GPW_ROWS_MINP && aligned16(gmap) && aligned16(m8)) {
    if (Co >= 1024)
      hipLaunchKernelGGL((gbias_gpw_rows_kernel<4, 8>), dim3((Co + 3) / 4), dim3(256), 0, st, gmap, m8, gPw, Cin, Co, P / 4);
    else
      hipLaunchKernelGGL((gbias_gpw_rows_kernel<2, 8>), dim3((Co + 1) / 2), dim3(256), 0, st, gmap, m8, gPw, Cin, Co, P / 4);
    return;
  }
  hipLaunchKernelGGL(gbias_gpw_kernel, dim3(Co * Cin), dim3(256), 0, st, gmap, m8, gPw, Cin, P);
}

}

extern "C" int paradis_global_bias_map_fwd(const float* A, const float* U, const float* V,
                                           const float* Pw, float* m8, float* map, int Cin, int Co,
                                           int R, int H, int W, void* stream) {
  PD_REQUIRE(Cin >= 1 && Co >= 1 && R >= 1 && H >= 1 && W >= 1, "global_bias_map_fwd: bad shape");
  PD_REQUIRE(Pw != nullptr || Cin == Co, "global_bias_map_fwd: projection required when Cin != Co");
  hipStream_t st = (hipStream_t)stream;
  const int64_t P = (int64_t)H * W;
  float* m8_dst = Pw ? m8 : map;
  PD_REQUIRE(H <= 65535 && Cin <= 65535 && Co <= 65535, "global_bias_map_fwd: grid too large");
  if ((int64_t)H * W >= (1 << 17) && R <= GM8_MAXR)
    hipLaunchKernelGGL(gbias_m8_rows_kernel<8>, dim3((W + 63) / 64, (H + 7) / 8, Cin), dim3(256), 0, st, A, U, V, m8_dst,
                       Cin, R, H, W);
  else
    hipLaunchKernelGGL(gbias_m8_kernel, dim3((W + 63) / 64, H, Cin), dim3(256), 0, st, A, U, V, m8_dst, Cin, R, H, W);
  if (Pw)
    hipLaunchKernelGGL(small_mix_kernel, dim3((unsigned)((P + 255) / 256), Co), dim3(256), 0, st, Pw, Cin, 1,
                       m8, map, Co, Cin, P);
  PD_CHECK_LAUNCH("global_bias_map_fwd");
  return 0;
}

extern "C" size_t paradis_global_bias_map_bwd_ws_bytes(int Cin, int Co, int R, int H, int W) {
  (void)Co;
  return ((size_t)Cin * H * W + (size_t)Cin * R * H + (size_t)Cin * R * W) * sizeof(float) + 256;
}

extern "C" int paradis_global_bias_map_bwd(const float* gmap, const float* A, const float* U,
                                           const float* V, const float* Pw, const float* m8, float* gA,
                                           float* gU, float* gV, float* gPw, int Cin, int Co, int R,
                                           int H, int W, void* workspace, void* stream) {
  PD_REQUIRE(Cin >= 1 && Co >= 1 && R >= 1 && H >= 1 && W >= 1, "global_bias_map_bwd: bad shape");
  PD_REQUIRE(workspace != nullptr, "global_bias_map_bwd: workspace required");
  PD_REQUIRE(Pw != nullptr || Cin == Co, "global_bias_map_bwd: projection required when Cin != Co");
  hipStream_t st = (hipStream_t)stream;
  const int64_t P = (int64_t)H * W;
  float* gm8 = (float*)workspace;
  float* T1 = gm8 + (size_t)Cin * P;
  float* T2 = T1 + (size_t)Cin * R * H;
  const float* gm8_src = gmap;
  if (Pw) {
    PD_REQUIRE(m8 != nullptr && gPw != nullptr, "global_bias_map_bwd: m8/gPw required with projection");
    launch_gpw(gmap, m8, gPw, Cin, Co, P, st);
    if (Cin <= 16) {
      launch_gm8(Pw, gmap, gm8, Cin, Co, P, st);
    } else {
      hipLaunchKernelGGL(small_mix_kernel, dim3((unsigned)((P + 255) / 256), Cin), dim3(256), 0, st, Pw, 1,
                         Cin, gmap, gm8, Cin, Co, P);
    }
    gm8_src = gm8;
  }
  const int64_t nwaves = (int64_t)Cin * R * H;
  hipLaunchKernelGGL(gbias_t1_kernel, dim3((unsigned)((nwaves * 64 + 255) / 256)), dim3(256), 0, st,
                     gm8_src, V, T1, Cin, R, H, W);
  hipLaunchKernelGGL(gbias_t2_kernel, dim3(stream_blocks((int64_t)Cin * R * W)), dim3(256), 0, st, gm8_src,
                     U, T2, Cin, R, H, W);
  const int nfin = (Cin * R + 3) / 4 + (R * H + R * W + 255) / 256;
  hipLaunchKernelGGL(gbias_finish_kernel, dim3(nfin), dim3(256), 0, st, T1, T2, A, U, gA, gU,
                     gV, Cin, R, H, W);
  PD_CHECK_LAUNCH("global_bias_map_bwd");
  return 0;
}

extern "C" int paradis_act_fwd(const float* x, float* y, int64_t n, int act, void* stream) {
  PD_REQUIRE(n >= 0 && act >= 0 && act <= 2, "act_fwd: bad arguments");
  if (n == 0) return 0;
  const bool vec = (n % 4 == 0) && aligned16(x) && aligned16(y);
  hipLaunchKernelGGL(act_kernel<false>, dim3(stream_blocks(vec ? n / 4 : n)), dim3(256), 0,
                     (hipStream_t)stream, nullptr, x, y, n, act, vec);
  PD_CHECK_LAUNCH("act_fwd");
  return 0;
}

extern "C" int paradis_act_bwd(const float* gy, const float* x, float* gx, int64_t n, int act, void* stream) {
  PD_REQUIRE(n >= 0 && act >= 0 && act <= 2, "act_bwd: bad arguments");
  if (n == 0) return 0;
  const bool vec = (n % 4 == 0) && aligned16(x) && aligned16(gy) && aligned16(gx);
  hipLaunchKernelGGL(act_kernel<true>, dim3(stream_blocks(vec ? n / 4 : n)), dim3(256), 0,
                     (hipStream_t)stream, gy, x, gx, n, act, vec);
  PD_CHECK_LAUNCH("act_bwd");
  return 0;
}

extern "C" int paradis_act_bwd16(const float* gy, const float* x, void* gx, int64_t n, int act, void* stream) {
  PD_REQUIRE(n >= 0 && act >= 0 && act <= 2, "act_bwd16: bad arguments");
  if (n == 0) return 0;
  PD_REQUIRE(n % 4 == 0 && aligned16(x) && aligned16(gy) && (reinterpret_cast<uintptr_t>(gx) & 7) == 0,
             "act_bwd16: n %% 4 == 0 and aligned tensors required");
  hipLaunchKernelGGL((act_kernel<true, true>), dim3(stream_blocks(n / 4)), dim3(256), 0, (hipStream_t)stream, gy, x,
                     (float*)gx, n, act, true);
  PD_CHECK_LAUNCH("act_bwd16");
  return 0;
}

extern "C" int paradis_add(const float* a, const float* b, float* y, int64_t n, void* stream) {
  PD_REQUIRE(n >= 0, "add: bad arguments");
  if (n == 0) return 0;
  const bool vec = (n % 4 == 0) && aligned16(a) && aligned16(b) && aligned16(y);
  hipLaunchKernelGGL(add_kernel, dim3(stream_blocks(vec ? n / 4 : n)), dim3(256), 0, (hipStream_t)stream,
                     a, b, y, n, vec);
  PD_CHECK_LAUNCH("add");
  return 0;
}

extern "C" int paradis_gated_blend_fwd(const float* h, const float* adv, const float* alpha,
                                       float* out, int B, int C, int P, void* stream) {
  PD_REQUIRE(B >= 0 && C >= 1 && P >= 1, "gated_blend_fwd: bad shape");
  if (B == 0) return 0;
  hipLaunchKernelGGL(gated_blend_fwd_kernel, dim3((unsigned)((int64_t)B * C)), dim3(256), 0,
                     (hipStream_t)stream, h, adv, alpha, out, C, P);
  PD_CHECK_LAUNCH("gated_blend_fwd");
  return 0;
}

extern "C" size_t paradis_gated_blend_bwd_ws_bytes(int B, int C, int P) {
  (void)P;
  return (size_t)std::max(B, 1) * C * sizeof(float) + 256;
}

static int gated_blend_bwd_impl(const float* gout, const float* h, const float* third, const float* alpha, float* gh,
                                float* gadv, float* galpha, int B, int C, int P, void* workspace, void* stream,
                                int from_out) {
  PD_REQUIRE(B >= 0 && C >= 1 && P >= 1, "gated_blend_bwd: bad shape");
  PD_REQUIRE(workspace != nullptr, "gated_blend_bwd: workspace required");
  hipStream_t st = (hipStream_t)stream;
  float* partial = (float*)workspace;
  if (B > 0)
    hipLaunchKernelGGL(gated_blend_bwd_kernel, dim3((unsigned)((int64_t)B * C)), dim3(256), 0, st, gout, h,
                       third, alpha, gh, gadv, partial, C, P);
  hipLaunchKernelGGL(gated_blend_finish, dim3((C + 255) / 256), dim3(256), 0, st, partial, alpha, galpha, B, C,
                     from_out);
  PD_CHECK_LAUNCH("gated_blend_bwd");
  return 0;
}

extern "C" int paradis_gated_blend_bwd(const float* gout, const float* h, const float* adv,
                                       const float* alpha, float* gh, float* gadv, float* galpha, int B,
                                       int C, int P, void* workspace, void* stream) {
  return gated_blend_bwd_impl(gout, h, adv, alpha, gh, gadv, galpha, B, C, P, workspace, stream, 0);
}

__global__ void __launch_bounds__(256)
bias_grads_b16_kernel(const uint16_t* __restrict__ dz, float* __restrict__ gmap, float* __restrict__ gbias,
                      int B, int C, int P8, int64_t bs, int pchunks) {
  __shared__ float red[4];
  const int c = blockIdx.x / pchunks, chunk = blockIdx.x - c * pchunks;
  const uint4* src = reinterpret_cast<const uint4*>(dz + (int64_t)c * P8 * 8);
  const int64_t bs8 = bs / 8;
  float acc = 0.f;
  for (int q = chunk * 256 + threadIdx.x; q < P8; q += pchunks * 256) {
    float s[8] = {0.f, 0.f, 0.f, 0.f, 0.f, 0.f, 0.f, 0.f};
    for (int b0 = 0; b0 < B; b0 += 8) {
      uint4 v[8];
#pragma unroll
      for (int j = 0; j < 8; ++j) v[j] = src[(int64_t)min(b0 + j, B - 1) * bs8 + q];
#pragma unroll
      for (int j = 0; j < 8; ++j) {
        if (b0 + j < B) {
          const uint32_t w[4] = {v[j].x, v[j].y, v[j].z, v[j].w};
#pragma unroll
          for (int i = 0; i < 4; ++i) {
            s[2 * i] += __uint_as_float(w[i] << 16);
            s[2 * i + 1] += __uint_as_float(w[i] & 0xffff0000u);
          }
        }
      }
    }
    if (gmap) {
      float4* o = reinterpret_cast<float4*>(gmap + (int64_t)c * P8 * 8) + 2 * q;
      o[0] = make_float4(s[0], s[1], s[2], s[3]);
      o[1] = make_float4(s[4], s[5], s[6], s[7]);
    }
    acc += ((s[0] + s[1]) + (s[2] + s[3])) + ((s[4] + s[5]) + (s[6] + s[7]));
  }
  if (!gbias) return;
  acc = wave_sum_dpp(acc);
  if ((threadIdx.x & 63) == 0) red[threadIdx.x >> 6] = acc;
  __syncthreads();
  if (threadIdx.x == 0) atomicAdd(&gbias[c], red[0] + red[1] + red[2] + red[3]);
}

extern "C" int paradis_gated_blend_bwd_out(const float* gout, const float* h, const float* out,
                                           const float* alpha, float* gh, float* gadv, float* galpha, int B,
                                           int C, int P, void* workspace, void* stream) {
  return gated_blend_bwd_impl(gout, h, out, alpha, gh, gadv, galpha, B, C, P, workspace, stream, 1);
}

extern "C" int paradis_bias_grads(const float* dz, float* gmap, float* gbias, int B, int C, int P,
                                  int64_t dz_bs, void* stream) {
  PD_REQUIRE(B >= 0 && C >= 1 && P >= 1, "bias_grads: bad shape");
  hipStream_t st = (hipStream_t)stream;
  if (gbias && pd_zero_async(gbias, (size_t)C * sizeof(float), st) != hipSuccess) {
    paradis_set_error("bias_grads: memset failed");
    return 2;
  }
  if (!gmap && !gbias) return 0;
  if (P % 4 == 0 && dz_bs % 4 == 0 && aligned16(dz) && (!gmap || aligned16(gmap))) {
    const int P4 = P / 4;
    int pch = std::max(1, std::min(2, std::min((P4 + 255) / 256, std::max(1, 2048 / C))));
    if (paradis_deterministic()) pch = 1;
    hipLaunchKernelGGL(bias_grads_vec4_kernel, dim3((unsigned)((int64_t)C * pch)), dim3(256), 0, st, dz, gmap,
                       gbias, B, C, P4, dz_bs, pch);
    PD_CHECK_LAUNCH("bias_grads");
    return 0;
  }
  int pchunks = std::max(1, std::min(2, std::min((P + 255) / 256, std::max(1, 2048 / C))));
  if (paradis_deterministic()) pchunks = 1;
  hipLaunchKernelGGL(bias_grads_kernel, dim3((unsigned)((int64_t)C * pchunks)), dim3(256), 0, st, dz, gmap,
                     gbias, B, C, P, dz_bs, pchunks);
  PD_CHECK_LAUNCH("bias_grads");
  return 0;
}

extern "C" int paradis_bias_grads16(const void* dz, float* gmap, float* gbias, int B, int C, int P,
                                    int64_t dz_bs, void* stream) {
  PD_REQUIRE(B >= 0 && C >= 1 && P >= 1, "bias_grads16: bad shape");
// ... 60 lines not shown
```

paradis_model_amd/model/blocks.py:

```python
from collections import OrderedDict
from collections.abc import Sequence
from typing import Optional, Tuple, Type, Union

import torch
from torch import nn

from .. import ops
from .padding import GeoCyclicPadding

_ACT_TYPES = (nn.SiLU, nn.GELU)


def init_conv2d_default(conv: nn.Conv2d, *, scale: float = 1.0) -> None:
    nn.init.kaiming_normal_(conv.weight, mode="fan_in", nonlinearity="relu")
    if scale != 1.0:
        with torch.no_grad():
            conv.weight.mul_(scale)
    if conv.bias is not None:
        nn.init.constant_(conv.bias, 0.0)


def init_module_convs(m: nn.Module, *, last_conv_scale: float = 1.0) -> None:
    convs = [mod for mod in m.modules()
             if not isinstance(mod, GlobalBias) and isinstance(mod, nn.Conv2d)]
    for i, conv in enumerate(convs):
        init_conv2d_default(conv, scale=last_conv_scale if i == len(convs) - 1 else 1.0)


class PhysicalDownsample(nn.Module):

    def __init__(self, stride=4):
        super().__init__()
        self.stride = stride
        self.pool = nn.AvgPool2d(kernel_size=5, stride=stride, count_include_pad=False)
        self.padding = GeoCyclicPadding(2)

    def forward(self, x: torch.Tensor) -> torch.Tensor:
        return ops.avgpool_geo(x, self.stride)


FUSE_BIAS_PROJECTION = True
FUSE_BIAS_PROJECTION_MIN_POINTS = 8192


class CLinear(nn.Module):

    def __init__(self, input_dim: int, output_dim: int, mesh_size: tuple, kernel_size: int = 1,
                 bias: bool = True):
        super().__init__()
        self.conv = nn.Conv2d(input_dim, output_dim, kernel_size=1, bias=bias)

    def forward(self, x, bias_map=None, act: Optional[str] = None, residual=None, x_pre=None,
                x_act=None, defer_act_grad=False, bias_proj=None, gate=None, out_bf16: bool = False):
        return ops.pointwise(x, self.conv.weight, self.conv.bias, bias_map, residual, act, x_pre, x_act,
                             defer_act_grad, bias_proj, gate=gate, out_bf16=out_bf16)


class SepConv(nn.Module):

    def __init__(self, input_dim: int, output_dim: int, mesh_size: tuple, kernel_size: int = 3,
                 bias: bool = True):
        super().__init__()
        if kernel_size % 2 == 0 or not 1 <= kernel_size <= 11:
            raise NotImplementedError("SepConv: the HIP depthwise stencil supports odd kernel_size 1..11; "
                                      f"got {kernel_size}")
        self.padding = (kernel_size - 1) // 2
        self.geo_padding = GeoCyclicPadding(self.padding)
        self.depthwise = nn.Conv2d(input_dim, input_dim, kernel_size, groups=input_dim, bias=False)
        self.pointwise = nn.Conv2d(input_dim, output_dim, kernel_size=1, bias=bias)

    def forward(self, x, bias_map=None, act: Optional[str] = None, residual=None, bias_proj=None,
                with_skip: bool = False, gate=None):
        skip = None
        if with_skip:
            x, skip = ops.dwconv_geo_skip(x, self.depthwise.weight, self.depthwise.bias, out_bf16=True)
        else:
            x = ops.dwconv_geo(x, self.depthwise.weight, self.depthwise.bias, out_bf16=True)
        out = ops.pointwise(x, self.pointwise.weight, self.pointwise.bias, bias_map, residual, act,
                            bias_proj=bias_proj, gate=gate)
        return (out, skip) if with_skip else out


class ChannelNorm(nn.Module):

    def __init__(self, input_dim: int, output_dim: int):
        super().__init__()
        assert input_dim == output_dim
        self.eps = 1e-5
        self.weight = nn.Parameter(torch.ones(input_dim), requires_grad=True)
        self.bias = nn.Parameter(torch.zeros(input_dim), requires_grad=True)

    def forward(self, x, x_extra=None, with_skip: bool = False, out_bf16: bool = False):
        if with_skip:
            return ops.channel_norm_skip(x, self.weight, self.bias, self.eps, x_extra, out_bf16=out_bf16)
        return ops.channel_norm(x, self.weight, self.bias, self.eps, x_extra, out_bf16=out_bf16)


class GlobalBias(nn.Module):

    def __init__(self, input_dim: int, output_dim: int, *, bias: bool = True, kernel_size: int = 0,
                 mesh_size: Tuple[int, int], rank: int = 128):
        super().__init__()
        self.input_dim = input_dim
        self.output_dim = output_dim
        self.rank = rank
        self.height, self.width = mesh_size
        self.A = nn.Parameter(torch.zeros(input_dim, rank), requires_grad=True)
        self.U = nn.Parameter(torch.zeros(rank, self.height), requires_grad=True)
        self.V = nn.Parameter(torch.zeros(rank, self.width), requires_grad=True)
        with torch.no_grad():
            nn.init.normal_(self.A, mean=0.0, std=1e-3)
            nn.init.normal_(self.U, mean=0.0, std=1e-3)
            nn.init.normal_(self.V, mean=0.0, std=1e-3)
        self.projection = (nn.Linear(input_dim, output_dim, bias=False)
                           if input_dim != output_dim else None)

    def bias_terms(self):
        big = self.U.shape[1] * self.V.shape[1] >= FUSE_BIAS_PROJECTION_MIN_POINTS
        if (FUSE_BIAS_PROJECTION and big and self.projection is not None and self.input_dim <= 16
                and self.output_dim % 4 == 0):
            return None, (ops.global_bias_m8(self.A, self.U, self.V), self.projection.weight)
        return self.bias_map(), None

    def bias_map(self) -> torch.Tensor:
        pw = self.projection.weight if self.projection is not None else None
        return ops.global_bias_map(self.A, self.U, self.V, pw)

    def forward(self, x: torch.Tensor) -> torch.Tensor:
        return ops.add_bias_map(x, self.bias_map())


BLOCK_REGISTRY = {
    "SepConv": SepConv,
    "CLinear": CLinear,
    "ChannelNorm": ChannelNorm,
    "GlobalBias": GlobalBias,
}


class GMBlock(nn.Sequential):

    def __init__(self, layers: Sequence[Union[str, Type[nn.Module]]], input_dim: int, output_dim: int,
                 mesh_size: Tuple[int, int], kernel_size: Union[Sequence[int], int] = 5,
                 hidden_dim: Union[Sequence, int] = 0, activation_fn: Type[nn.Module] = nn.SiLU,
                 bias_channels: int = 0, activation: Union[Sequence, bool] = False,
                 pre_normalize: bool = False):
        depth = len(layers)
        if depth == 0:
            raise ValueError("GMBlock: must specify at least one layer")

        def per_layer(value, count, what):
            if isinstance(value, Sequence) and not isinstance(value, str):
                if len(value) != count:
                    raise AssertionError(f"GMBlock: {what} needs {count} entries, got {len(value)}")
                return tuple(value)
            return (value,) * count

        activation = (per_layer(activation, depth, "activation") if isinstance(activation, Sequence)
                      else (True,) * (depth - 1) + (bool(activation),))
        if not isinstance(hidden_dim, Sequence) and hidden_dim <= 0:
            hidden_dim = max(input_dim, output_dim)
        hidden_dim = per_layer(hidden_dim, depth - 1, "hidden_dim")
        kernel_size = per_layer(kernel_size, depth, "kernel_size")
        num_layers = depth

        children = []
        if pre_normalize:
            children.append(("0-ChannelNorm", ChannelNorm(input_dim=input_dim, output_dim=input_dim)))
        width_in = input_dim
        for idx, spec in enumerate(layers):
            if isinstance(spec, str):
                if spec not in BLOCK_REGISTRY:
                    raise ValueError(
                        f"Unknown layer type: {spec}. Available: {list(BLOCK_REGISTRY.keys())}")
                cls = BLOCK_REGISTRY[spec]
            else:
                cls = spec
            width_out = output_dim if idx == num_layers - 1 else hidden_dim[idx]
            children.append((f"{idx}-{cls.__name__}",
                             cls(input_dim=width_in, output_dim=width_out, mesh_size=mesh_size,
                                 kernel_size=kernel_size[idx])))
            if idx == 0 and bias_channels > 0:
                children.append(("0-GlobalBias", GlobalBias(input_dim=bias_channels,
                                                            output_dim=width_out,
                                                            mesh_size=mesh_size)))
            if activation[idx]:
                children.append((f"{idx}-{activation_fn.__name__}", activation_fn()))
            width_in = width_out

        super().__init__(OrderedDict(children))
        init_module_convs(self, last_conv_scale=0.1)

    def forward(self, x, residual=None, x_extra=None, return_skip: bool = False, gate=None):
        if gate is not None and residual is None:
            raise ValueError("GMBlock: a gate needs the residual it blends with")
        mods = list(self.children())
        n = len(mods)
        i = 0
        skip, x_in = None, x
        fuse_skip = (n > 0 and isinstance(mods[0], ChannelNorm) and torch.is_grad_enabled()
                     and x.requires_grad and (return_skip or residual is x))
        stencil_skip = (n > 0 and isinstance(mods[0], SepConv) and torch.is_grad_enabled() and x.requires_grad
                        and return_skip and residual is None and x_extra is None)
        if x_extra is not None and not (n and isinstance(mods[0], ChannelNorm)):
            x = torch.cat([x, x_extra], dim=1)
            x_extra = None
        pre = pre_act = None
        while i < n:
            m = mods[i]
            if isinstance(m, ChannelNorm):
                to_gemm = i + 1 < n and isinstance(mods[i + 1], CLinear)
                if i == 0 and fuse_skip:
                    res_is_x = residual is x
                    x, skip = m(x, x_extra, with_skip=True, out_bf16=to_gemm)
                    if res_is_x:
                        residual = skip
                else:
                    x = m(x, x_extra, out_bf16=to_gemm)
                x_extra = None
                i += 1
            elif isinstance(m, (CLinear, SepConv)):
                j = i + 1
                bias_map = bias_proj = act = None
                if j < n and isinstance(mods[j], GlobalBias):
                    bias_map, bias_proj = mods[j].bias_terms()
                    j += 1
                if j < n and isinstance(mods[j], _ACT_TYPES):
                    act = type(mods[j]).__name__
                    j += 1
                res = residual if j == n else None
                hand_off = (act is not None and res is None and j < n and isinstance(mods[j], CLinear)
                            and isinstance(m, CLinear) and torch.is_grad_enabled())
                g = gate if res is not None else None
                chain16 = (act is not None and res is None and j < n and isinstance(mods[j], CLinear)
                           and isinstance(m, CLinear))
                if isinstance(m, CLinear):
                    out = m(x, bias_map=bias_map, act=act, residual=res, x_pre=pre, x_act=pre_act,
                            defer_act_grad=hand_off, bias_proj=bias_proj, gate=g, out_bf16=chain16)
                elif i == 0 and stencil_skip:
                    out, skip = m(x, bias_map=bias_map, act=act, residual=res, bias_proj=bias_proj, with_skip=True)
                else:
                    out = m(x, bias_map=bias_map, act=act, residual=res, bias_proj=bias_proj, gate=g)
                if hand_off:
                    x, pre = out
                    pre_act = act
                else:
                    x, pre, pre_act = out, None, None
                if res is not None:
                    residual = None
                i = j
            elif isinstance(m, _ACT_TYPES):
                x = ops.activation(x, type(m).__name__)
                i += 1
            else:
                x = m(x)
                i += 1
        if residual is not None:
            x = ops.add(x, residual) if gate is None else ops.gated_blend(residual, x, gate)
        if return_skip:
            return x, (skip if skip is not None else x_in)
        return x
```

paradis_model_amd/model/paradis.py:

```python
import torch
from torch import nn
from torch.utils.checkpoint import checkpoint

from .. import ops
from .advection import NeuralSemiLagrangian
from .blocks import GMBlock, PhysicalDownsample, SepConv
from .padding import GeoCyclicPadding

EARTH_ROTATION_RATE = 7.29212e-5


def get_scaled_timestep(original_timestep_seconds: float) -> float:
    return original_timestep_seconds * EARTH_ROTATION_RATE


_ACTIVATIONS = {"SiLU": nn.SiLU, "GELU": nn.GELU}


def _get_activation_cls(name: str):
    if name not in _ACTIVATIONS:
        raise ValueError(f"Unknown activation_fn '{name}'. Allowed: {list(_ACTIVATIONS.keys())}")
    return _ACTIVATIONS[name]


class StaticEncoder(nn.Sequential):

    def __init__(self, n_static: int, static_dim: int, mesh_size):
        super().__init__(
            SepConv(n_static, 64, mesh_size, kernel_size=7),
            nn.SiLU(),
            GeoCyclicPadding(3),
            nn.Conv2d(64, 64, groups=64, kernel_size=7),
            nn.SiLU(),
            SepConv(64, static_dim, mesh_size, kernel_size=5),
        )

    def forward(self, x):
        x = self[0](x, act="SiLU")
        x = ops.dwconv_geo(x, self[3].weight, self[3].bias)
        x = ops.activation(x, "SiLU")
        return self[5](x)


class Paradis(nn.Module):

    def __init__(self, datamodule, cfg, lat_grid, lon_grid):
        super().__init__()
        mcfg, pb = cfg.model, cfg.model.physblock
        self.nlat, self.nlon = (int(n) for n in lat_grid.shape)
        mesh_size = (self.nlat, self.nlon)
        stride = mcfg.get("coarsening_factor", 1)
        if stride < 1:
            raise ValueError("Coarsening factor must be >=1")
        self.nlat_coarse, self.nlon_coarse = (self.nlat - 1) // stride + 1, self.nlon // stride
        mesh_coarse = (self.nlat_coarse, self.nlon_coarse)

        self.num_layers = max(1, mcfg.num_layers)
        self.num_vels = mcfg.get("velocity_vectors")
        self.dt = get_scaled_timestep(mcfg.get("base_dt")) / self.num_layers
        self.activation_function = act = _get_activation_cls(mcfg.activation)
        hidden_dim, bias_channels = mcfg.get("latent_size"), mcfg.get("bias_channels", 4)
        adv_interpolation = mcfg.get("adv_interpolation")
        static_dim = 128

        ds = datamodule.dataset
        input_dim = ds.num_in_dyn_features + ds.num_in_static_features
        self.num_common_features, self.n_inputs = datamodule.num_common_features, cfg.dataset.n_time_inputs
        self.n_static = len(cfg.features.input.constants)

        self.gradient_checkpoint = bool(cfg.compute.get("gradient_checkpointing", False))
        self.step_fn = self._checkpointed_step if self.gradient_checkpoint else self._layer_step

        self.input_proj = GMBlock(layers=pb.input_proj.layers, input_dim=input_dim,
                                  output_dim=hidden_dim, hidden_dim=pb.input_proj.hidden_dim,
                                  mesh_size=mesh_size, activation=True, activation_fn=act,
                                  pre_normalize=False, bias_channels=0)
        self.velocity_nets = nn.ModuleList([
            GMBlock(layers=pb.velocity_net.layers, input_dim=hidden_dim,
                    output_dim=2 * self.num_vels, hidden_dim=pb.velocity_net.hidden_dim,
                    mesh_size=mesh_coarse, bias_channels=bias_channels, activation_fn=act,
                    pre_normalize=True)
            for _ in range(self.num_layers)])
        self.advection = nn.ModuleList([
            NeuralSemiLagrangian(cfg, hidden_dim, mesh_coarse, num_vels=self.num_vels,
                                 lat_grid=lat_grid[::stride, ::stride],
                                 lon_grid=lon_grid[::stride, ::stride],
                                 interpolation=adv_interpolation)
            for _ in range(self.num_layers)])
        self.diffusion = nn.ModuleList([
            GMBlock(layers=pb.diffusion.layers, input_dim=hidden_dim, output_dim=hidden_dim,
                    hidden_dim=pb.diffusion.hidden_dim, mesh_size=mesh_coarse, pre_normalize=True,
                    activation_fn=act, bias_channels=bias_channels)
            for _ in range(self.num_layers)])
        self.reaction = nn.ModuleList([
            GMBlock(layers=pb.reaction.layers, input_dim=hidden_dim + static_dim,
                    output_dim=hidden_dim, hidden_dim=pb.reaction.hidden_dim, mesh_size=mesh_coarse,
                    pre_normalize=True, activation_fn=act, bias_channels=bias_channels)
            for _ in range(self.num_layers)])
        self.output_proj = GMBlock(pre_normalize=True, layers=pb.output_proj.layers,
                                   input_dim=hidden_dim, output_dim=datamodule.num_out_features,
                                   hidden_dim=pb.output_proj.hidden_dim, mesh_size=mesh_size,
                                   activation=False, activation_fn=act, bias_channels=bias_channels)

        self.alpha_adv = nn.Parameter(torch.full((self.num_layers, hidden_dim), -1.0))
        self.downsample = PhysicalDownsample(stride=stride)
        self.static_encoder = StaticEncoder(self.n_static, static_dim, mesh_size)

    def _checkpointed_step(self, i, h, hs):
        return checkpoint(self._layer_step, i, h, hs, use_reentrant=False)

    def _compile(self):
        self._layer_step = torch.compile(self._layer_step)
        self.static_encoder = torch.compile(self.static_encoder)
        self.input_proj = torch.compile(self.input_proj)
        self.output_proj = torch.compile(self.output_proj)
        self.step_fn = self._checkpointed_step if self.gradient_checkpoint else self._layer_step


    def upsample(self, x: torch.Tensor) -> torch.Tensor:
        return ops.upsample_lonp(x, self.nlat, self.nlon)

    def _apply_checkpoint(self, func, *args):
        if self.gradient_checkpoint:
            return checkpoint(func, *args, use_reentrant=False)
        return func(*args)

    def _layer_step(self, i: int, hidden: torch.Tensor, hidden_static: torch.Tensor) -> torch.Tensor:
        velocities, hidden = self.velocity_nets[i](hidden, return_skip=True)

        hidden = self.advection[i].transport(hidden, velocities, self.dt, self.alpha_adv[i])

        hidden = self.diffusion[i](hidden, residual=hidden)

        hidden = self.reaction[i](hidden, residual=hidden, x_extra=hidden_static)
        return hidden

    def forward(self, fields):
        hidden = self._apply_checkpoint(self.input_proj, fields)
        hidden_static = self._apply_checkpoint(self.static_encoder, fields[:, -self.n_static:])

        skip = hidden
        hidden = self.downsample(hidden)
        hidden_static = self.downsample(hidden_static)

        for i in range(self.num_layers):
            hidden = self.step_fn(i, hidden, hidden_static)

        hidden = ops.add(self.upsample(hidden), skip)
        return self._apply_checkpoint(self.output_proj, hidden)
```

paradis_model_amd/ops.py:

```python
from __future__ import annotations

import os
import threading
import weakref
from typing import List, Optional, Sequence, Tuple

import torch
from torch import Tensor

from . import _lib
from ._lib import check, dptr, lib, stream_ptr

ACT_CODES = {None: 0, "none": 0, "SiLU": 1, "GELU": 2}
MODE_CODES = {"bilinear": 1, "bicubic": 2}

_DEF = torch.library.Library("paradis", "DEF")
OPS = {}
RAW = {}


_dispatch_modes = getattr(torch._C, "_len_torch_dispatch_stack", None)
_functorch_top = getattr(getattr(torch._C, "_functorch", None), "peek_interpreter_stack", None)
_CAN_BE_PLAIN = _dispatch_modes is not None and _functorch_top is not None


def _plain(t) -> bool:
    return (_CAN_BE_PLAIN and type(t) is Tensor and not torch.is_grad_enabled()
            and _dispatch_modes() == 0
            and _functorch_top() is None)


def _all_plain(args) -> bool:
    if not (_CAN_BE_PLAIN and _dispatch_modes() == 0 and _functorch_top() is None):
        return False
    for a in args:
        if isinstance(a, Tensor) and type(a) is not Tensor and type(a) is not torch.nn.Parameter:
            return False
    return True


def _widen_for_autocast(args):
    if not torch.is_autocast_enabled("cuda"):
        return args
    return tuple(a.float() if (isinstance(a, Tensor) and a.is_floating_point() and a.dtype != torch.float32) else a
                 for a in args)


def _eager_forward(name: str, op, *args):
    if not torch.is_grad_enabled() and _all_plain(args) and (name == "pointwise" or not torch.is_autocast_enabled("cuda")):
        return RAW[name](*args)
    return op(*args)


def _selective_autocast(name: str, keep16: Tuple[int, ...], scheme_idx: Optional[int]) -> None:
    op = getattr(torch.ops.paradis, name).default
    keyset = (torch._C.DispatchKeySet(torch._C.DispatchKey.AutocastCPU)
              | torch._C.DispatchKeySet(torch._C.DispatchKey.AutocastCUDA))

    def cast(args):
        mixed = scheme_idx is None or args[scheme_idx] == GEMM_BF16
        return tuple(a.float() if (isinstance(a, Tensor) and a.is_floating_point() and a.dtype != torch.float32
                                   and not (mixed and i in keep16 and a.dtype == torch.bfloat16)) else a
                     for i, a in enumerate(args))

    def py_impl(*args, **kwargs):
        assert not kwargs, "custom ops take positional arguments here"
        with torch._C._ExcludeDispatchKeyGuard(keyset):
            return op(*cast(args))

    try:
        op.py_impl(torch._C.DispatchKey.AutocastCUDA)(py_impl)
    except Exception:
        pass
    _DEF.impl(name, lambda _ks, *args, **kwargs: py_impl(*args, **kwargs), "AutocastCUDA", with_keyset=True)


def _define(schema: str, autocast=True):
    name = schema[: schema.index("(")]
    _DEF.define(schema)

    def deco(fn):
        RAW[name] = fn
        _DEF.impl(name, fn, "CUDA")
        if autocast is True:
            torch.library.register_autocast(f"paradis::{name}", "cuda", torch.float32)
        elif autocast:
            _selective_autocast(name, tuple(autocast[0]), autocast[1])
        ov = getattr(torch.ops.paradis, name).default
        OPS[name] = ov
        return ov
    return deco


def _fake(name: str):
    return torch.library.register_fake(f"paradis::{name}")


def _autograd(name: str, setup, backward) -> None:
    torch.library.register_autograd(f"paradis::{name}", backward, setup_context=setup)


def require_hip(*tensors) -> None:
    for t in tensors:
        if t is not None and not t.is_cuda:
            raise RuntimeError("paradis_model_amd ops run on the MI355X only: got a CPU tensor "
                               "(there is no CPU fallback; use oracle/ for CPU checks)")


def _f32(*tensors) -> None:
    for t in tensors:
        if t is not None and t.dtype != torch.float32:
            raise RuntimeError(f"paradis_model_amd ops are fp32; got {t.dtype}")


def _f32_or_bf16(scheme: int, *tensors) -> None:
    for t in tensors:
        if t is not None and t.dtype != torch.float32 and not (t.dtype == torch.bfloat16 and scheme == GEMM_BF16):
            raise RuntimeError(f"paradis_model_amd ops are fp32 (bf16 tensors only in the bf16-mixed GEMM scheme); got {t.dtype}")


def _is16(t) -> bool:
    return t is not None and t.dtype == torch.bfloat16


def _cotangent(gy, takes_bf16: bool):
    if gy is None or gy.dtype == torch.float32 or (takes_bf16 and gy.dtype == torch.bfloat16):
        return gy
    return gy.float()


def _want_bf16_out(x: Tensor, out_bf16: bool) -> bool:
    return (bool(out_bf16) and BF16_STORAGE and autocast_scheme(GEMM_SCHEME) == GEMM_BF16
            and (x.shape[-2] * x.shape[-1]) % 16 == 0 and not torch.compiler.is_compiling())


def _ws(nbytes: int, device) -> Optional[Tensor]:
    if nbytes <= 0:
        return None
    return torch.empty((nbytes + 3) // 4, dtype=torch.float32, device=device)


def _planes_hw(x: Tensor) -> Tuple[int, int, int]:
    H, W = x.shape[-2:]
    return x.numel() // (H * W), H, W


def _none_if_empty(t: Tensor) -> Optional[Tensor]:
    return t if t.numel() else None


def _plane_view(t: Tensor) -> Tuple[Tensor, int]:
    B, C, H, W = t.shape
    if t.stride(3) == 1 and t.stride(2) == W and t.stride(1) == H * W:
        return t, (t.stride(0) if B > 1 else C * H * W)
# ... 728 lines not shown
@_define("global_bias_m8(Tensor A, Tensor U, Tensor V) -> Tensor")
def _global_bias_m8(A, U, V):
    _f32(A, U, V)
    A, U, V = A.contiguous(), U.contiguous(), V.contiguous()
    Cin, R = A.shape
    H, W = U.shape[1], V.shape[1]
    m8 = torch.empty(Cin, H, W, dtype=A.dtype, device=A.device)
    check(lib.paradis_global_bias_m8_fwd(dptr(A), dptr(U), dptr(V), dptr(m8), Cin, R, H, W, stream_ptr()),
          "global_bias_m8_fwd")
    return m8


@_fake("global_bias_m8")
def _(A, U, V):
    return A.new_empty(A.shape[0], U.shape[1], V.shape[1])


@_define("global_bias_m8_backward(Tensor gm8, Tensor A, Tensor U, Tensor V) -> (Tensor, Tensor, Tensor)")
def _global_bias_m8_backward(gm8, A, U, V):
    _f32(gm8)
    A, U, V = A.contiguous(), U.contiguous(), V.contiguous()
    Cin, R = A.shape
    H, W = U.shape[1], V.shape[1]
    gm8 = gm8.contiguous()
    gA, gU, gV = torch.empty_like(A), torch.empty_like(U), torch.empty_like(V)
    ws = _ws(lib.paradis_global_bias_map_bwd_ws_bytes(Cin, Cin, R, H, W), A.device)
    check(lib.paradis_global_bias_m8_bwd(dptr(gm8), dptr(A), dptr(U), dptr(V), dptr(gA), dptr(gU), dptr(gV),
                                         Cin, R, H, W, dptr(ws), stream_ptr()), "global_bias_m8_bwd")
    return gA, gU, gV


@_fake("global_bias_m8_backward")
def _(gm8, A, U, V):
    return A.new_empty(A.shape), U.new_empty(U.shape), V.new_empty(V.shape)


def _gb8_setup(ctx, inputs, output):
    ctx.save_for_backward(*inputs)


def _gb8_backward(ctx, gm8):
    return _global_bias_m8_backward(gm8, *ctx.saved_tensors)


_autograd("global_bias_m8", _gb8_setup, _gb8_backward)


def global_bias_m8(A, U, V):
    require_hip(A, U, V)
    return _global_bias_m8(A, U, V)


GEMM_EXACT, GEMM_BF16, GEMM_F16X2, GEMM_BF16X3 = 0, 1, 2, 3
BF16_STORAGE = os.environ.get("PARADIS_BF16_STORAGE", "1") != "0"
IO_X16, IO_Y16, IO_Z16, IO_DY16 = 1, 2, 4, 8
_SCHEMES = {"exact": GEMM_EXACT, "f16x2": GEMM_F16X2, "bf16x3": GEMM_BF16X3, "split": GEMM_BF16X3}
AMAX_PARTIALS = 1024


def _scheme_from_env() -> int:
    name = os.environ.get("PARADIS_GEMM", "bf16x3")
    if name not in _SCHEMES:
        raise ValueError(f"PARADIS_GEMM={name!r}: choose between {'|'.join(_SCHEMES)}")
    return _SCHEMES[name]


GEMM_SCHEME = _scheme_from_env()


def gemm_scheme_name() -> str:
    return {GEMM_EXACT: "exact", GEMM_BF16: "bf16", GEMM_F16X2: "f16x2", GEMM_BF16X3: "bf16x3"}[GEMM_SCHEME]


def autocast_scheme(default: int) -> int:
    if torch.is_autocast_enabled("cuda") and torch.get_autocast_dtype("cuda") == torch.bfloat16:
        return GEMM_BF16
    return default


WEIGHT_EPOCH = 0
FROZEN_WEIGHTS = False
_IMAGES = {}
_TLS = threading.local()


class frozen_weights:

    def __init__(self, enabled: bool = True):
        self.enabled = bool(enabled)

    def __enter__(self):
        global FROZEN_WEIGHTS
        self.prev = FROZEN_WEIGHTS
        FROZEN_WEIGHTS = self.enabled
        return self

    def __exit__(self, *exc):
        global FROZEN_WEIGHTS
        FROZEN_WEIGHTS = self.prev
        if not FROZEN_WEIGHTS:
            _IMAGES.clear()
        return False


def weights_updated() -> None:
    global WEIGHT_EPOCH
    WEIGHT_EPOCH += 1


def _optimizer_step_hook(optimizer, args, kwargs) -> None:
    weights_updated()


_STEP_HOOK = None


def _ensure_step_hook() -> None:
    global _STEP_HOOK
    if _STEP_HOOK is None:
        from torch.optim.optimizer import register_optimizer_step_post_hook
        _STEP_HOOK = register_optimizer_step_post_hook(_optimizer_step_hook)


def _drop_images(wid: int) -> None:
    for scheme in (GEMM_BF16, GEMM_F16X2, GEMM_BF16X3):
        _IMAGES.pop((wid, False, scheme), None)
        _IMAGES.pop((wid, True, scheme), None)


def _version_of(t: Tensor) -> int:
    return 0 if t.is_inference() else t._version


_PAIRED_SCHEMES = (GEMM_BF16X3, GEMM_BF16)


def _build_images(weight: Tensor, Co: int, Ci: int, transpose: bool, scheme: int, pair: bool):
    w2 = weight.reshape(Co, Ci).contiguous()
    nbytes = lib.paradis_pw_gemm_split_bytes(Ci, Co, scheme) if transpose else \
        lib.paradis_pw_gemm_split_bytes(Co, Ci, scheme)
    out = torch.empty(nbytes, dtype=torch.uint8, device=weight.device)
    if pair and not transpose and scheme in _PAIRED_SCHEMES:
        out_t = torch.empty(lib.paradis_pw_gemm_split_bytes(Ci, Co, scheme), dtype=torch.uint8, device=weight.device)
        check(lib.paradis_pw_gemm_split_weights_pair_scheme(dptr(w2), Co, Ci, scheme, dptr(out), dptr(out_t), stream_ptr()),
              "pw_gemm_split_weights_pair")
        return out, out_t
    check(lib.paradis_pw_gemm_split_weights(dptr(w2), Co, Ci, 1 if transpose else 0, scheme, dptr(out),
                                            stream_ptr()), "pw_gemm_split_weights")
    return out, None


def _split_image(weight: Tensor, Co: int, Ci: int, transpose: bool, scheme: int, want_wt: bool = False):
    if not FROZEN_WEIGHTS:
        return _build_images(weight, Co, Ci, transpose, scheme, want_wt)
    key = (id(weight), transpose, scheme)
    ver = _version_of(weight)

    def valid(ent):
        return (ent is not None and ent[0]() is weight and ent[1] == weight.data_ptr() and ent[2] == ver
                and ent[3] == WEIGHT_EPOCH)
    ent = _IMAGES.get(key)
    ent_t = _IMAGES.get((id(weight), True, scheme)) if (want_wt and not transpose) else None
    if valid(ent) and (not (want_wt and not transpose and scheme in _PAIRED_SCHEMES) or valid(ent_t)):
        return ent[4], (ent_t[4] if valid(ent_t) else None)
    out, out_t = _build_images(weight, Co, Ci, transpose, scheme, want_wt)
    if isinstance(weight, torch.nn.Parameter) or weight.is_leaf:
        wid = id(weight)
        _ensure_step_hook()
        try:
            ref = weakref.ref(weight, lambda _r, wid=wid: _drop_images(wid))
            _IMAGES[key] = (ref, weight.data_ptr(), ver, WEIGHT_EPOCH, out)
            if out_t is not None:
                _IMAGES[(wid, True, scheme)] = (ref, weight.data_ptr(), ver, WEIGHT_EPOCH, out_t)
        except TypeError:
            pass
    return out, out_t


def _stash_wt(weight: Tensor, image: Optional[Tensor]) -> None:
    _TLS.wt = (weight, image) if image is not None else None


def _take_wt(weight: Tensor) -> Optional[Tensor]:
    ent = getattr(_TLS, "wt", None)
    _TLS.wt = None
    return ent[1] if (ent is not None and ent[0] is weight) else None


@_define("amax_partials(Tensor x) -> Tensor")
def _amax_partials(x):
    _f32(x)
    x, x_bs = _plane_view(x)
    B, C, H, W = x.shape
    out = torch.empty(AMAX_PARTIALS, dtype=torch.int32, device=x.device)
    check(lib.paradis_amax_partials(dptr(x), B, C * H * W, x_bs, dptr(out), stream_ptr()), "amax_partials")
    return out


@_fake("amax_partials")
def _(x):
    return x.new_empty(AMAX_PARTIALS, dtype=torch.int32)


@_define("pointwise(Tensor x, Tensor weight, Tensor? bias, Tensor? bmap, Tensor? residual, int act, "
         "Tensor? x_pre, int x_act, bool defer_act_grad, Tensor? m8, Tensor? pw, bool save_z, int scheme, "
         "Tensor? gate, bool want_wt_image=False, bool out_bf16=False) -> (Tensor, Tensor, Tensor)", autocast=((0, 6), 12))
def _pointwise(x, weight, bias, bmap, residual, act, x_pre, x_act, defer_act_grad, m8, pw, save_z, scheme, gate,
               want_wt_image=False, out_bf16=False):
    _f32(weight, bias, bmap, residual, m8, pw, gate)
    _f32_or_bf16(scheme, x)
    x, x_bs = _plane_view(x)
    B, Ci, H, W = x.shape
    Co = weight.shape[0]
    P = H * W
    assert weight.numel() == Co * Ci, "weight/in-channel mismatch"
    x16 = _is16(x)
    if x16 or out_bf16:
        if scheme != GEMM_BF16 or (out_bf16 and residual is not None):
            raise RuntimeError("bf16-stored tensors need the bf16-mixed GEMM scheme (and a bf16 output no residual)")
        if x16 and (P % 8 or x_bs % 8 or x.data_ptr() % 16):
            raise RuntimeError("a bf16-stored GEMM input needs H W % 8 == 0 and 16-byte aligned planes")
    if gate is not None:
        assert residual is not None and gate.numel() == Co, "a gate needs the residual it blends with, one value per channel"
        gate = gate.reshape(Co).contiguous()
    res_bs = 0
    if residual is not None:
        residual, res_bs = _plane_view(residual)
    if bmap is not None:
        bmap = bmap.contiguous()
    y = torch.empty(B, Co, H, W, dtype=torch.bfloat16 if out_bf16 else torch.float32, device=x.device)
    cin, pwt = 0, None
    if pw is not None:
        m8, pw = m8.contiguous(), pw.contiguous()
        cin = pw.shape[1]
        assert pw.shape[0] == Co and m8.shape == (cin, H, W) and bmap is None
        assert Co % 4 == 0 and cin <= 16, "fused GlobalBias projection needs Co % 4 == 0 and <= 16 bias channels"
        pwt = pw.t().contiguous()
    z = torch.empty_like(y) if (save_z and act != 0) else y.new_empty(0)
    w2 = w2t = wsp = None
    x_amax = x.new_empty(0, dtype=torch.int32)
    _stash_wt(weight, None)
    if scheme != GEMM_EXACT:
        wsp, wtsp_out = _split_image(weight, Co, Ci, False, scheme, bool(want_wt_image))
        _stash_wt(weight, wtsp_out)
        if scheme == GEMM_F16X2:
            x_amax = torch.empty(AMAX_PARTIALS, dtype=torch.int32, device=x.device)
            check(lib.paradis_amax_partials(dptr(x), B, Ci * P, x_bs, dptr(x_amax), stream_ptr()), "amax_partials")
    else:
        w2 = weight.reshape(Co, Ci).contiguous()
        if Ci % 16 == 0 and Co % 4 == 0 and Co * Ci >= 4096:
            w2t = torch.empty(Ci, Co, dtype=torch.float32, device=x.device)
            check(lib.paradis_transpose(dptr(w2), dptr(w2t), Co, Ci, stream_ptr()), "transpose")
    if w2 is None:
        w2 = weight.reshape(Co, Ci)
        if not w2.is_contiguous():
            w2 = w2.contiguous()
    head = (dptr(w2), dptr(w2t), dptr(wsp), scheme, dptr(x_amax) if x_amax.numel() else None, dptr(x), dptr(bias),
            dptr(bmap), dptr(m8) if cin else None, dptr(pwt) if cin else None, cin, dptr(residual))
    tail = (dptr(y), dptr(z) if z.numel() else None, B, Co, Ci, P, x_bs, res_bs, Co * P, act, stream_ptr())
    if x16 or out_bf16:
        _lib.call("pw_gemm_fwd", 2.0 * B * Co * Ci * P, dptr(wsp), dptr(x), dptr(bias), dptr(bmap),
                  dptr(m8) if cin else None, dptr(pwt) if cin else None, cin, dptr(residual), dptr(gate), dptr(y),
                  dptr(z) if z.numel() else None, B, Co, Ci, P, x_bs, res_bs, Co * P, act,
                  (IO_X16 if x16 else 0) | (IO_Y16 if out_bf16 else 0), stream_ptr(), symbol="pw_gemm_fwd16")
        return y, z, x_amax
    if gate is None:
        _lib.call("pw_gemm_fwd", 2.0 * B * Co * Ci * P, *head, *tail)
    else:
        _lib.call("pw_gemm_fwd", 2.0 * B * Co * Ci * P, *head, dptr(gate), *tail, symbol="pw_gemm_fwd_gated")
    return y, z, x_amax


@_fake("pointwise")
def _(x, weight, bias, bmap, residual, act, x_pre, x_act, defer_act_grad, m8, pw, save_z, scheme, gate,
      want_wt_image=False, out_bf16=False):
    B, _, H, W = x.shape
    y = x.new_empty(B, weight.shape[0], H, W, dtype=torch.bfloat16 if out_bf16 else torch.float32)
    return (y, (y.new_empty(y.shape) if (save_z and act != 0) else y.new_empty(0)),
            x.new_empty(AMAX_PARTIALS if scheme == GEMM_F16X2 else 0, dtype=torch.int32))


@_define("act_backward(Tensor gy, Tensor z, int act, bool out_bf16=False) -> Tensor")
def _act_backward(gy, z, act, out_bf16=False):
    _f32(gy, z)
    gy, z = gy.contiguous(), z.contiguous()
    if out_bf16 and gy.numel() % 4 == 0:
        dz = torch.empty(gy.shape, dtype=torch.bfloat16, device=gy.device)
        check(lib.paradis_act_bwd16(dptr(gy), dptr(z), dptr(dz), gy.numel(), act, stream_ptr()), "act_bwd16")
        return dz
    dz = torch.empty_like(gy)
    check(lib.paradis_act_bwd(dptr(gy), dptr(z), dptr(dz), gy.numel(), act, stream_ptr()), "act_bwd")
    return dz


@_fake("act_backward")
def _(gy, z, act, out_bf16=False):
    return gy.new_empty(gy.shape, dtype=torch.bfloat16 if (out_bf16 and gy.numel() % 4 == 0) else gy.dtype)


@_define("pw_gemm_dgrad(Tensor dz, Tensor weight, Tensor? zmul, int x_act, Tensor? dz_amax, int scheme, "
         "Tensor? wt_image=None, bool out_bf16=False) -> Tensor", autocast=((0, 2), 5))
def _pw_gemm_dgrad(dz, weight, zmul, x_act, dz_amax, scheme, wt_image=None, out_bf16=False):
    _f32(weight)
    _f32_or_bf16(scheme, dz, zmul)
    dz = dz.contiguous()
    B, Co, H, W = dz.shape
# ... 119 lines not shown
    ctx.wt_image = _take_wt(weight)
    ctx.mark_non_differentiable(z, x_amax)
    ctx.set_materialize_grads(False)


class WgradSide:
    LAG = 6
    enabled = os.environ.get("PARADIS_WGRAD_STREAM", "0") == "1"
    PRIORITY = int(os.environ.get("PARADIS_WGRAD_STREAM_PRIORITY", "0"))
    _streams = {}
    _pending = []
    _callback_queued = False

    @classmethod
    def stream(cls, device) -> "torch.cuda.Stream":
        idx = device.index if device.index is not None else torch.cuda.current_device()
        st = cls._streams.get(idx)
        if st is None:
            st = cls._streams[idx] = torch.cuda.Stream(device=idx, priority=cls.PRIORITY)
        return st

    @classmethod
    def launch(cls, fn, dz, x, *rest):
        side = cls.stream(dz.device)
        ready = torch.cuda.Event()
        ready.record()
        side.wait_event(ready)
        with torch.cuda.stream(side):
            out = fn(dz, x, *rest)
            done = torch.cuda.Event()
            done.record()
        cur = torch.cuda.current_stream()
        cls._pending.append((done, cur, (dz, x, rest)))
        while len(cls._pending) > cls.LAG:
            ev, st, _refs = cls._pending.pop(0)
            st.wait_event(ev)
        if not cls._callback_queued:
            try:
                torch.autograd.Variable._execution_engine.queue_callback(cls.join)
                cls._callback_queued = True
            except RuntimeError:
                cls.join()
        return out

    @classmethod
    def join(cls) -> None:
        cls._callback_queued = False
        for ev, st, _refs in cls._pending:
            st.wait_event(ev)
        cls._pending.clear()


def _pw_backward(ctx, gy, gz=None, gamax=None, raw=False):
    saved = ctx.saved_tensors
    if raw is None:
        raw = gy is not None and _plain(gy) and _all_plain(saved)
    K = RAW if raw else OPS
    x, weight, z, x_pre, m8, pw, x_amax, res_saved, y_saved, gate = saved
    act, has_bias, has_map, has_res, x_act, deferred, scheme = ctx.meta
    need = ctx.needs_input_grad
    if gy is None:
        return (None,) * 16
    want = torch.bfloat16 if getattr(ctx, "out16", False) else torch.float32
    if gy.dtype != want:
        gy = gy.to(want)
    has_proj = pw is not None
    ggate = None
    if gate is not None:
        gres, gy, ggate = K["gated_blend_backward_out"](gy, res_saved, y_saved, gate)
        ggate = ggate.reshape(gate.shape)
    else:
        gres = gy if has_res else None
    if act != 0 and not deferred:
        dz16 = (scheme == GEMM_BF16 and BF16_STORAGE and gy.dtype == torch.float32 and (gy.shape[-2] * gy.shape[-1]) % 16 == 0)
        dz = K["act_backward"](gy, z, act, dz16)
    else:
        dz = gy
    gx = gw = gb = gmap = gm8 = gpw = None
    dz_amax = K["amax_partials"](dz) if (scheme == GEMM_F16X2 and (need[0] or need[1])) else None
    if need[0]:
        gx = K["pw_gemm_dgrad"](dz, weight, x_pre if x_act != 0 else None, x_act, dz_amax, scheme,
                                getattr(ctx, "wt_image", None), x.dtype == torch.bfloat16)
    want_b = has_bias and need[2]
    want_p = has_proj and (need[9] or need[10])
    want_m = (has_map and need[3]) or want_p
    if need[1]:
        fused_b = want_b and not want_m
        if raw and WgradSide.enabled:
            gw, gbf = WgradSide.launch(K["pw_gemm_wgrad"], dz, x, fused_b, dz_amax, x_amax, scheme)
        else:
            gw, gbf = K["pw_gemm_wgrad"](dz, x, fused_b, dz_amax, x_amax, scheme)
        gw = gw.reshape(weight.shape)
        if fused_b:
            gb, want_b = gbf, False
    if want_b or want_m:
        gb2, gmap = K["bias_grads"](dz, want_b, want_m)
        if want_b:
            gb = gb2
        if not want_m:
            gmap = None
    if want_p:
        gpw, gm8 = K["global_bias_proj_backward"](gmap, m8, pw)
        gmap = None
    return gx, gw, gb, gmap, gres, None, None, None, None, gm8, gpw, None, None, ggate, None, None


_autograd("pointwise", _pw_setup, _pw_backward)


class _PointwiseEager(torch.autograd.Function):

    @staticmethod
    def forward(ctx, *args):
        out = _eager_forward("pointwise", _pointwise, *args)
        _pw_setup(ctx, args, out)
        return out

    @staticmethod
    def backward(ctx, gy, gz=None, gamax=None):
        return _pw_backward(ctx, gy, gz, gamax, raw=None)


def pointwise(x, weight, bias=None, bias_map=None, residual=None, act=None, x_pre=None, x_act=None,
              defer_act_grad=False, bias_proj=None, scheme: Optional[int] = None, gate=None, out_bf16: bool = False):
    if defer_act_grad and (act is None or residual is not None):
        raise ValueError("defer_act_grad needs an activation and no residual")
    if gate is not None and residual is None:
        raise ValueError("a gate needs the residual it blends with")
    m8, pw = bias_proj if bias_proj is not None else (None, None)
    require_hip(x, weight, bias, bias_map, residual, x_pre, m8, pw, gate)
    sch = autocast_scheme(GEMM_SCHEME) if scheme is None else int(scheme)
    P = x.shape[-2] * x.shape[-1]
    ok16 = sch == GEMM_BF16 and P % 16 == 0 and BF16_STORAGE
    if x.dtype != torch.float32 and not (ok16 and x.dtype == torch.bfloat16):
        x = x.float()
    if x_pre is not None and x_pre.dtype != torch.float32 and not (ok16 and x_pre.dtype == torch.bfloat16):
        x_pre = x_pre.float()
    weight, bias, bias_map, residual, m8, pw, gate = (
        t.float() if (t is not None and t.dtype != torch.float32) else t
        for t in (weight, bias, bias_map, residual, m8, pw, gate))
    out16 = bool(out_bf16) and ok16 and residual is None and (bool(defer_act_grad) or not torch.is_grad_enabled())
    code = ACT_CODES[act]
    save_z = bool(defer_act_grad)
    if code != 0 and not save_z and torch.is_grad_enabled():
        save_z = any(t is not None and t.requires_grad for t in (x, weight, bias, bias_map, m8, pw))
    eager = not torch.compiler.is_compiling()
    want_wt = eager and torch.is_grad_enabled() and (x.requires_grad or (x_pre is not None and x_pre.requires_grad))
    args = (x, weight, bias, bias_map, residual, code, x_pre, ACT_CODES[x_act], bool(defer_act_grad), m8, pw,
            save_z, sch, gate, bool(want_wt), out16)
    y, z, _ = _PointwiseEager.apply(*args) if (eager and torch.is_grad_enabled()) else _pointwise(*args)
    return (y, z) if defer_act_grad else y


@_define("activation(Tensor x, int act) -> Tensor")
def _activation(x, act):
    _f32(x)
    x = x.contiguous()
    y = torch.empty_like(x)
    check(lib.paradis_act_fwd(dptr(x), dptr(y), x.numel(), act, stream_ptr()), "act_fwd")
    return y


@_fake("activation")
def _(x, act):
    return x.new_empty(x.shape)


def _act_setup(ctx, inputs, output):
    ctx.save_for_backward(inputs[0])
    ctx.act = inputs[1]


def _act_bwd(ctx, gy):
    return _act_backward(gy, ctx.saved_tensors[0], ctx.act), None


_autograd("activation", _act_setup, _act_bwd)


def activation(x, name: str):
    if name not in ("SiLU", "GELU"):
        raise ValueError(f"Unknown activation_fn '{name}'. Allowed: ['SiLU', 'GELU']")
    require_hip(x)
    return _activation(x, ACT_CODES[name])


@_define("gated_blend(Tensor h, Tensor adv, Tensor alpha) -> Tensor")
def _gated_blend(h, adv, alpha):
    _f32(h, adv, alpha)
    h, adv, alpha = h.contiguous(), adv.contiguous(), alpha.contiguous()
    B, C, H, W = h.shape
    out = torch.empty_like(h)
    check(lib.paradis_gated_blend_fwd(dptr(h), dptr(adv), dptr(alpha), dptr(out), B, C, H * W, stream_ptr()),
          "gated_blend_fwd")
    return out


@_fake("gated_blend")
def _(h, adv, alpha):
    return h.new_empty(h.shape)


@_define("gated_blend_backward(Tensor gout, Tensor h, Tensor adv, Tensor alpha) -> (Tensor, Tensor, Tensor)")
def _gated_blend_backward(gout, h, adv, alpha):
    _f32(gout)
    h, adv, alpha, gout = h.contiguous(), adv.contiguous(), alpha.contiguous(), gout.contiguous()
    B, C, H, W = h.shape
    gh, gadv, galpha = torch.empty_like(h), torch.empty_like(h), torch.empty_like(alpha)
    ws = _ws(lib.paradis_gated_blend_bwd_ws_bytes(B, C, H * W), h.device)
    check(lib.paradis_gated_blend_bwd(dptr(gout), dptr(h), dptr(adv), dptr(alpha), dptr(gh), dptr(gadv),
                                      dptr(galpha), B, C, H * W, dptr(ws), stream_ptr()), "gated_blend_bwd")
    return gh, gadv, galpha


@_fake("gated_blend_backward")
def _(gout, h, adv, alpha):
    return h.new_empty(h.shape), h.new_empty(h.shape), alpha.new_empty(alpha.shape)


@_define("gated_blend_backward_out(Tensor gout, Tensor h, Tensor out, Tensor alpha) -> (Tensor, Tensor, Tensor)")
def _gated_blend_backward_out(gout, h, out, alpha):
    _f32(gout, h, out, alpha)
    gout, h, out = gout.contiguous(), h.contiguous(), out.contiguous()
    B, C, H, W = h.shape
    alpha = alpha.reshape(C).contiguous()
    gh, gadv = torch.empty_like(h), torch.empty_like(h)
    galpha = torch.empty(C, dtype=h.dtype, device=h.device)
    ws = _ws(lib.paradis_gated_blend_bwd_ws_bytes(B, C, H * W), h.device)
    check(lib.paradis_gated_blend_bwd_out(dptr(gout), dptr(h), dptr(out), dptr(alpha), dptr(gh), dptr(gadv),
                                          dptr(galpha), B, C, H * W, dptr(ws), stream_ptr()), "gated_blend_bwd_out")
    return gh, gadv, galpha


@_fake("gated_blend_backward_out")
def _(gout, h, out, alpha):
    return h.new_empty(h.shape), h.new_empty(h.shape), alpha.new_empty(alpha.numel())


def _blend_setup(ctx, inputs, output):
    ctx.save_for_backward(*inputs)


def _blend_backward(ctx, gout):
    return _gated_blend_backward(gout, *ctx.saved_tensors)


_autograd("gated_blend", _blend_setup, _blend_backward)


def gated_blend(h, adv, alpha):
    require_hip(h, adv, alpha)
    return _gated_blend(h, adv, alpha)


@_define("add(Tensor a, Tensor b) -> Tensor")
def _add(a, b):
    _f32(a, b)
    assert a.shape == b.shape
    a, b = a.contiguous(), b.contiguous()
    y = torch.empty_like(a)
    check(lib.paradis_add(dptr(a), dptr(b), dptr(y), a.numel(), stream_ptr()), "add")
    return y


@_fake("add")
def _(a, b):
    return a.new_empty(a.shape)


_autograd("add", lambda ctx, inputs, output: None, lambda ctx, gy: (gy, gy))


def add(a, b):
    require_hip(a, b)
    return _add(a, b)


@_define("add_bias_map(Tensor x, Tensor bmap) -> Tensor")
def _add_bias_map(x, bmap):
    _f32(x, bmap)
    x, bmap = x.contiguous(), bmap.contiguous()
    assert x.shape[1:] == bmap.shape
    y = torch.empty_like(x)
    check(lib.paradis_add_bcast(dptr(x), dptr(bmap), dptr(y), bmap.numel(), x.shape[0], stream_ptr()), "add_bcast")
    return y


@_fake("add_bias_map")
def _(x, bmap):
    return x.new_empty(x.shape)


def _abm_backward(ctx, gy):
    gmap = None
    if ctx.needs_input_grad[1]:
        gmap = _bias_grads(gy, False, True)[1]
    return gy, gmap


_autograd("add_bias_map", lambda ctx, inputs, output: None, _abm_backward)


def add_bias_map(x, bmap):
    require_hip(x, bmap)
    return _add_bias_map(x, bmap)

# ... 215 lines not shown
```

Measured before the change: 212.5 samples/s.

## Batch per-step weight splitting and global-bias maps into single multi-job launches

Adds plan-based multi-job kernels that split all GEMM weights into bf16x3 images (plus their transposes) in one launch per step, and compute every global-bias map (and its backward) in one grouped launch. A step-batch context caches the plans keyed on pointers and shapes and routes modules to the precomputed images and maps. This replaces many small per-layer launches and the host overhead that comes with them. In exchange it adds plan bookkeeping, dynamic job lookup inside the kernels, and cache-key fragility, and it is skipped during stream capture.

```diff
diff --git a/include/paradis_hip.h b/include/paradis_hip.h
--- a/include/paradis_hip.h
+++ b/include/paradis_hip.h
@@ -71,6 +71,10 @@
 int paradis_pw_gemm_split_weights(const float* W, int M, int K, int transpose, int scheme, void* out, void* stream);
 int paradis_pw_gemm_split_weights_pair(const float* W, int M, int K, void* out, void* out_t, void* stream);
 int paradis_pw_gemm_split_weights_pair_scheme(const float* W, int M, int K, int scheme, void* out, void* out_t, void* stream);
+size_t paradis_pw_gemm_split_multi_plan_bytes(int n);
+int paradis_pw_gemm_split_multi_plan(const float* const* W, const int* M, const int* K, int n, int scheme, int with_t,
+                                     void* plan, size_t* offsets, size_t* image_bytes);
+int paradis_pw_gemm_split_weights_multi(const void* plan_host, const void* plan_dev, void* images, void* stream);
 int paradis_pw_gemm_fwd(const float* Wt, const float* WtT ,
                         const void* Wsplit ,
                         int scheme, const uint32_t* x_amax ,
@@ -151,6 +155,18 @@
 int paradis_global_bias_proj_bwd(const float* gmap, const float* m8, const float* Pw, float* gPw,
                                  float* gm8, int Cin, int Co, int64_t P, void* stream);
 
+typedef struct {
+  const float *A, *U, *V, *Pw;
+  int Cin, Co, R, H, W;
+} paradis_gbias_desc;
+size_t paradis_global_bias_multi_plan_bytes(int n);
+int paradis_global_bias_multi_plan(const paradis_gbias_desc* desc, int n, void* plan);
+int paradis_global_bias_multi_offsets(const void* plan, int64_t* out);
+size_t paradis_global_bias_multi_bwd_ws_bytes(const void* plan);
+int paradis_global_bias_multi_fwd(const void* plan_host, const void* plan_dev, float* out, void* stream);
+int paradis_global_bias_multi_bwd(const void* plan_host, const void* plan_dev, const float* const* gmaps,
+                                  const float* fwd, float* grads, void* workspace, void* stream);
+
 int paradis_act_fwd(const float* x, float* y, int64_t n, int act, void* stream);
 int paradis_act_bwd(const float* gy, const float* x, float* gx, int64_t n, int act, void* stream);
 int paradis_gated_blend_fwd(const float* h, const float* adv, const float* alpha, float* out,
diff --git a/paradis_model_amd/_lib.py b/paradis_model_amd/_lib.py
--- a/paradis_model_amd/_lib.py
+++ b/paradis_model_amd/_lib.py
@@ -43,6 +43,9 @@
     "paradis_pw_gemm_split_weights": (I, [P, I, I, I, I, P, P]),
     "paradis_pw_gemm_split_weights_pair": (I, [P, I, I, P, P, P]),
     "paradis_pw_gemm_split_weights_pair_scheme": (I, [P, I, I, I, P, P, P]),
+    "paradis_pw_gemm_split_multi_plan_bytes": (S, [I]),
+    "paradis_pw_gemm_split_multi_plan": (I, [P, P, P, I, I, I, P, P, P]),
+    "paradis_pw_gemm_split_weights_multi": (I, [P, P, P, P]),
     "paradis_pw_gemm_fwd": (I, [P, P, P, I, P, P, P, P, P, P, I, P, P, P, I, I, I, I, L, L, L, I, P]),
     "paradis_pw_gemm_fwd_gated": (I, [P, P, P, I, P, P, P, P, P, P, I, P, P, P, P, I, I, I, I, L, L, L, I, P]),
     "paradis_forcings_ws_bytes": (ctypes.c_size_t, [I, I]),
@@ -72,6 +75,12 @@
     "paradis_global_bias_map_fwd": (I, [P, P, P, P, P, P, I, I, I, I, I, P]),
     "paradis_global_bias_map_bwd_ws_bytes": (S, [I, I, I, I, I]),
     "paradis_global_bias_map_bwd": (I, [P, P, P, P, P, P, P, P, P, P, I, I, I, I, I, P, P]),
+    "paradis_global_bias_multi_plan_bytes": (S, [I]),
+    "paradis_global_bias_multi_plan": (I, [P, I, P]),
+    "paradis_global_bias_multi_offsets": (I, [P, P]),
+    "paradis_global_bias_multi_bwd_ws_bytes": (S, [P]),
+    "paradis_global_bias_multi_fwd": (I, [P, P, P, P]),
+    "paradis_global_bias_multi_bwd": (I, [P, P, P, P, P, P, P]),
     "paradis_act_fwd": (I, [P, P, L, I, P]),
     "paradis_act_bwd": (I, [P, P, P, L, I, P]),
     "paradis_act_bwd16": (I, [P, P, P, L, I, P]),
diff --git a/paradis_model_amd/csrc/gemm.hip b/paradis_model_amd/csrc/gemm.hip
--- a/paradis_model_amd/csrc/gemm.hip
+++ b/paradis_model_amd/csrc/gemm.hip
@@ -384,9 +384,9 @@
 
 
 template <int NP = 3>
-__device__ __forceinline__ void split_weights_body(const float* __restrict__ Wb, int64_t rs, int64_t cs, int M, int K,
-                                                   int KT, int64_t units, u32x4* __restrict__ ob) {
-  for (int64_t u = (int64_t)blockIdx.x * 256 + threadIdx.x; u < units; u += (int64_t)gridDim.x * 256) {
+__device__ __forceinline__ void split_weights_unit(const float* __restrict__ Wb, int64_t rs, int64_t cs, int M, int K,
+                                                   int KT, int64_t u, u32x4* __restrict__ ob) {
+  {
     const int row = (int)(u & 127), half = (int)((u >> 7) & 1);
     const int64_t tile = u >> 8;
     const int kt = (int)(tile % KT), mt = (int)(tile / KT);
@@ -407,6 +407,36 @@
       ob[tile * simg(1) + half * SCH + row] = round8(x);
     }
   }
+}
+
+template <int NP = 3>
+__device__ __forceinline__ void split_weights_body(const float* __restrict__ Wb, int64_t rs, int64_t cs, int M, int K,
+                                                   int KT, int64_t units, u32x4* __restrict__ ob) {
+  for (int64_t u = (int64_t)blockIdx.x * 256 + threadIdx.x; u < units; u += (int64_t)gridDim.x * 256)
+    split_weights_unit<NP>(Wb, rs, cs, M, K, KT, u, ob);
+}
+
+struct SplitJob {
+  const float* W;
+  int64_t rs, cs;
+  int M, K, KT, pad;
+  int64_t units;
+  int64_t out_chunk;
+  int64_t pad2;
+};
+template <int NP>
+__global__ void __launch_bounds__(256)
+split_weights_multi_kernel(const SplitJob* __restrict__ jobs, const int* __restrict__ starts, int njobs,
+                           u32x4* __restrict__ images) {
+  __shared__ int found;
+  const int vb = blockIdx.x;
+  for (int j = threadIdx.x; j < njobs; j += 256)
+    if (vb >= starts[j] && vb < starts[j + 1]) found = j;
+  __syncthreads();
+  const int j = __builtin_amdgcn_readfirstlane(found);
+  const SplitJob jb = jobs[j];
+  const int64_t u = (int64_t)(vb - starts[j]) * 256 + threadIdx.x;
+  if (u < jb.units) split_weights_unit<NP>(jb.W, jb.rs, jb.cs, jb.M, jb.K, jb.KT, u, images + jb.out_chunk);
 }
 
 template <int NP>
@@ -1006,6 +1036,84 @@
 }
 extern "C" int paradis_pw_gemm_split_weights_pair(const float* W, int M, int K, void* out, void* out_t, void* stream) {
   return paradis_pw_gemm_split_weights_pair_scheme(W, M, K, PARADIS_GEMM_BF16X3, out, out_t, stream);
+}
+
+namespace {
+constexpr uint32_t SPLIT_PLAN_MAGIC = 0x504d5350u;
+struct SplitPlanHeader {
+  uint32_t magic;
+  int njobs, scheme, total_blocks;
+  uint64_t image_bytes;
+  int n, with_t;
+  uint64_t pad[4];
+};
+static_assert(sizeof(SplitPlanHeader) == 64 && sizeof(SplitJob) == 64, "split plan layout");
+}
+
+extern "C" size_t paradis_pw_gemm_split_multi_plan_bytes(int n) {
+  if (n < 1) return 0;
+  return (sizeof(SplitPlanHeader) + (size_t)2 * n * sizeof(SplitJob) + ((size_t)2 * n + 1) * sizeof(int) + 15) & ~(size_t)15;
+}
+
+extern "C" int paradis_pw_gemm_split_multi_plan(const float* const* W, const int* M, const int* K, int n, int scheme,
+                                                int with_t, void* plan, size_t* offsets, size_t* image_bytes) {
+  PD_REQUIRE(W != nullptr && M != nullptr && K != nullptr && plan != nullptr && offsets != nullptr &&
+                 image_bytes != nullptr && n >= 1,
+             "pw_gemm_split_multi_plan: bad arguments");
+  PD_REQUIRE(scheme == PARADIS_GEMM_BF16X3 || scheme == PARADIS_GEMM_BF16,
+             "pw_gemm_split_multi_plan: scheme %d has no paired images", scheme);
+  const int np = scheme == PARADIS_GEMM_BF16 ? 1 : 3;
+  SplitPlanHeader* hd = static_cast<SplitPlanHeader*>(plan);
+  SplitJob* jobs = reinterpret_cast<SplitJob*>(hd + 1);
+  const int njobs = with_t ? 2 * n : n;
+  int* starts = reinterpret_cast<int*>(jobs + 2 * n);
+  int64_t blocks = 0;
+  size_t bytes = 0;
+  int j = 0;
+  for (int i = 0; i < n; ++i) {
+    PD_REQUIRE(W[i] != nullptr && M[i] >= 1 && K[i] >= 1, "pw_gemm_split_multi_plan: bad weight %d", i);
+    for (int t = 0; t < (with_t ? 2 : 1); ++t, ++j) {
+      const int AM = t ? K[i] : M[i], AK = t ? M[i] : K[i];
+      SplitJob& jb = jobs[j];
+      jb.W = W[i];
+      jb.rs = t ? 1 : K[i];
+      jb.cs = t ? K[i] : 1;
+      jb.M = AM; jb.K = AK; jb.KT = split_image_ktiles(AK, np); jb.pad = 0; jb.pad2 = 0;
+      jb.units = (int64_t)((AM + BM - 1) / BM) * jb.KT * 256;
+      jb.out_chunk = (int64_t)(bytes / 16);
+      offsets[2 * i + t] = bytes;
+      starts[j] = (int)blocks;
+      blocks += jb.units / 256;
+      bytes += paradis_pw_gemm_split_bytes(AM, AK, scheme);
+      PD_REQUIRE(blocks < (int64_t)1 << 30, "pw_gemm_split_multi_plan: weight list too large");
+    }
+    if (!with_t) offsets[2 * i + 1] = (size_t)-1;
+  }
+  starts[njobs] = (int)blocks;
+  hd->magic = SPLIT_PLAN_MAGIC;
+  hd->njobs = njobs; hd->scheme = scheme; hd->total_blocks = (int)blocks;
+  hd->image_bytes = bytes; hd->n = n; hd->with_t = with_t ? 1 : 0;
+  for (uint64_t& p : hd->pad) p = 0;
+  *image_bytes = bytes;
+  return 0;
+}
+
+extern "C" int paradis_pw_gemm_split_weights_multi(const void* plan_host, const void* plan_dev, void* images, void* stream) {
+  PD_REQUIRE(plan_host != nullptr && plan_dev != nullptr && images != nullptr, "pw_gemm_split_weights_multi: bad arguments");
+  const SplitPlanHeader* hd = static_cast<const SplitPlanHeader*>(plan_host);
+  PD_REQUIRE(hd->magic == SPLIT_PLAN_MAGIC && hd->njobs >= 1 && hd->total_blocks >= 1 && hd->n >= 1,
+             "pw_gemm_split_weights_multi: not a plan of paradis_pw_gemm_split_multi_plan");
+  PD_REQUIRE((reinterpret_cast<uintptr_t>(images) & 15) == 0, "pw_gemm_split_weights_multi: image buffer not 16-byte aligned");
+  const SplitJob* jobs = reinterpret_cast<const SplitJob*>(static_cast<const char*>(plan_dev) + sizeof(SplitPlanHeader));
+  const int* starts = reinterpret_cast<const int*>(jobs + 2 * hd->n);
+  if (hd->scheme == PARADIS_GEMM_BF16X3)
+    hipLaunchKernelGGL(split_weights_multi_kernel<3>, dim3(hd->total_blocks), dim3(256), 0, (hipStream_t)stream, jobs, starts,
+                       hd->njobs, (u32x4*)images);
+  else
+    hipLaunchKernelGGL(split_weights_multi_kernel<1>, dim3(hd->total_blocks), dim3(256), 0, (hipStream_t)stream, jobs, starts,
+                       hd->njobs, (u32x4*)images);
+  PD_CHECK_LAUNCH("pw_gemm_split_weights_multi");
+  return 0;
 }
 
 namespace {
diff --git a/paradis_model_amd/csrc/misc.hip b/paradis_model_amd/csrc/misc.hip
--- a/paradis_model_amd/csrc/misc.hip
+++ b/paradis_model_amd/csrc/misc.hip
@@ -7,12 +7,12 @@
   return (int)std::max<int64_t>(1, std::min<int64_t>((n_items + 255) / 256, 256 * 16));
 }
 
-__global__ void __launch_bounds__(256)
-gbias_m8_kernel(const float* __restrict__ A, const float* __restrict__ U, const float* __restrict__ V,
-                float* __restrict__ m8, int Cin, int R, int H, int W) {
+__device__ __forceinline__ void
+gbias_m8_body(const float* __restrict__ A, const float* __restrict__ U, const float* __restrict__ V,
+              float* __restrict__ m8, int Cin, int R, int H, int W, int bx, int by, int bz) {
   __shared__ float part[4][64];
   const int tx = threadIdx.x & 63, q = threadIdx.x >> 6;
-  const int w = min(blockIdx.x * 64 + tx, W - 1), h = blockIdx.y, c = blockIdx.z;
+  const int w = min(bx * 64 + tx, W - 1), h = by, c = bz;
   const int rq = (R + 3) / 4, r1 = min(R, (q + 1) * rq);
   float acc = 0.f;
   int r = q * rq;
@@ -26,19 +26,24 @@
   for (; r < r1; ++r) acc += A[c * R + r] * U[r * H + h] * V[r * W + w];
   part[q][tx] = acc;
   __syncthreads();
-  if (q == 0 && blockIdx.x * 64 + tx < W)
+  if (q == 0 && bx * 64 + tx < W)
     m8[((int64_t)c * H + h) * W + w] = ((part[0][tx] + part[1][tx]) + part[2][tx]) + part[3][tx];
+}
+__global__ void __launch_bounds__(256)
+gbias_m8_kernel(const float* __restrict__ A, const float* __restrict__ U, const float* __restrict__ V,
+                float* __restrict__ m8, int Cin, int R, int H, int W) {
+  gbias_m8_body(A, U, V, m8, Cin, R, H, W, blockIdx.x, blockIdx.y, blockIdx.z);
 }
 
 constexpr int GM8_MAXR = 256;
 template <int ROWS>
-__global__ void __launch_bounds__(256)
-gbias_m8_rows_kernel(const float* __restrict__ A, const float* __restrict__ U, const float* __restrict__ V,
-                     float* __restrict__ m8, int Cin, int R, int H, int W) {
+__device__ __forceinline__ void
+gbias_m8_rows_body(const float* __restrict__ A, const float* __restrict__ U, const float* __restrict__ V,
+                   float* __restrict__ m8, int Cin, int R, int H, int W, int bx, int by, int bz) {
   __shared__ float part[4][ROWS][64];
   __shared__ float coef[GM8_MAXR][ROWS];
   const int tx = threadIdx.x & 63, q = threadIdx.x >> 6;
-  const int w = min(blockIdx.x * 64 + tx, W - 1), h0 = blockIdx.y * ROWS, c = blockIdx.z;
+  const int w = min(bx * 64 + tx, W - 1), h0 = by * ROWS, c = bz;
   for (int i = threadIdx.x; i < R * ROWS; i += 256) {
     const int r = i / ROWS, j = i - r * ROWS;
     coef[r][j] = A[c * R + r] * U[r * H + min(h0 + j, H - 1)];
@@ -66,23 +71,34 @@
 #pragma unroll
   for (int j = 0; j < ROWS; ++j) part[q][j][tx] = acc[j];
   __syncthreads();
-  if (q == 0 && blockIdx.x * 64 + tx < W) {
+  if (q == 0 && bx * 64 + tx < W) {
 #pragma unroll
     for (int j = 0; j < ROWS; ++j)
       if (h0 + j < H)
         m8[((int64_t)c * H + h0 + j) * W + w] = ((part[0][j][tx] + part[1][j][tx]) + part[2][j][tx]) + part[3][j][tx];
   }
 }
-
-__global__ void __launch_bounds__(256)
-small_mix_kernel(const float* __restrict__ Wm, int ldo, int ldc, const float* __restrict__ in,
-                 float* __restrict__ out, int Cout, int Cin, int64_t P) {
-  const int64_t p = (int64_t)blockIdx.x * 256 + threadIdx.x;
-  const int o = blockIdx.y;
+template <int ROWS>
+__global__ void __launch_bounds__(256)
+gbias_m8_rows_kernel(const float* __restrict__ A, const float* __restrict__ U, const float* __restrict__ V,
+                     float* __restrict__ m8, int Cin, int R, int H, int W) {
+  gbias_m8_rows_body<ROWS>(A, U, V, m8, Cin, R, H, W, blockIdx.x, blockIdx.y, blockIdx.z);
+}
+
+__device__ __forceinline__ void
+small_mix_body(const float* __restrict__ Wm, int ldo, int ldc, const float* __restrict__ in,
+               float* __restrict__ out, int Cout, int Cin, int64_t P, int bx, int by) {
+  const int64_t p = (int64_t)bx * 256 + threadIdx.x;
+  const int o = by;
   if (p >= P) return;
   float acc = 0.f;
   for (int c = 0; c < Cin; ++c) acc += Wm[(int64_t)o * ldo + (int64_t)c * ldc] * in[(int64_t)c * P + p];
   out[(int64_t)o * P + p] = acc;
+}
+__global__ void __launch_bounds__(256)
+small_mix_kernel(const float* __restrict__ Wm, int ldo, int ldc, const float* __restrict__ in,
+                 float* __restrict__ out, int Cout, int Cin, int64_t P) {
+  small_mix_body(Wm, ldo, ldc, in, out, Cout, Cin, P, blockIdx.x, blockIdx.y);
 }
 
 constexpr int GM8_SLICES = 16;
@@ -90,13 +106,13 @@
 #define GM8_BATCH 16
 #endif
 template <int CIN>
-__global__ void __launch_bounds__(64 * GM8_SLICES)
-gbias_gm8_kernel(const float* __restrict__ Pw, const float* __restrict__ gmap, float* __restrict__ gm8,
-                 int Cin, int Co, int64_t P) {
+__device__ __forceinline__ void
+gbias_gm8_body(const float* __restrict__ Pw, const float* __restrict__ gmap, float* __restrict__ gm8,
+               int Cin, int Co, int64_t P, int bx) {
   __shared__ float part[GM8_SLICES][CIN][64];
   const int px = threadIdx.x & 63;
   const int slice = __builtin_amdgcn_readfirstlane(threadIdx.x >> 6);
-  const int64_t p = (int64_t)blockIdx.x * 64 + px;
+  const int64_t p = (int64_t)bx * 64 + px;
   const int64_t pc = min(p, P - 1);
   const int per = (Co + GM8_SLICES - 1) / GM8_SLICES, o0 = slice * per, o1 = min(o0 + per, Co);
   float acc[CIN];
@@ -139,26 +155,37 @@
     gm8[(int64_t)slice * P + p] = s;
   }
 }
-
-__global__ void __launch_bounds__(256)
-gbias_gpw_kernel(const float* __restrict__ gmap, const float* __restrict__ m8,
-                 float* __restrict__ gPw, int Cin, int64_t P) {
+template <int CIN>
+__global__ void __launch_bounds__(64 * GM8_SLICES)
+gbias_gm8_kernel(const float* __restrict__ Pw, const float* __restrict__ gmap, float* __restrict__ gm8,
+                 int Cin, int Co, int64_t P) {
+  gbias_gm8_body<CIN>(Pw, gmap, gm8, Cin, Co, P, blockIdx.x);
+}
+
+__device__ __forceinline__ void
+gbias_gpw_body(const float* __restrict__ gmap, const float* __restrict__ m8,
+               float* __restrict__ gPw, int Cin, int64_t P, int bx) {
   __shared__ float red[4];
-  const int o = blockIdx.x / Cin, c = blockIdx.x - o * Cin;
+  const int o = bx / Cin, c = bx - o * Cin;
   float acc = 0.f;
   for (int64_t p = threadIdx.x; p < P; p += 256) acc += gmap[(int64_t)o * P + p] * m8[(int64_t)c * P + p];
   acc = wave_sum(acc);
   if ((threadIdx.x & 63) == 0) red[threadIdx.x >> 6] = acc;
   __syncthreads();
-  if (threadIdx.x == 0) gPw[blockIdx.x] = red[0] + red[1] + red[2] + red[3];
+  if (threadIdx.x == 0) gPw[bx] = red[0] + red[1] + red[2] + red[3];
+}
+__global__ void __launch_bounds__(256)
+gbias_gpw_kernel(const float* __restrict__ gmap, const float* __restrict__ m8,
+                 float* __restrict__ gPw, int Cin, int64_t P) {
+  gbias_gpw_body(gmap, m8, gPw, Cin, P, blockIdx.x);
 }
 
 template <int RW, int CIN>
-__global__ void __launch_bounds__(256)
-gbias_gpw_rows_kernel(const float* __restrict__ gmap, const float* __restrict__ m8, float* __restrict__ gPw, int Cin,
-                      int Co, int64_t P4) {
+__device__ __forceinline__ void
+gbias_gpw_rows_body(const float* __restrict__ gmap, const float* __restrict__ m8, float* __restrict__ gPw, int Cin,
+                    int Co, int64_t P4, int bx) {
   __shared__ float red[4][RW * CIN];
-  const int o0 = blockIdx.x * RW;
+  const int o0 = bx * RW;
   float acc[RW][CIN];
 #pragma unroll
   for (int j = 0; j < RW; ++j)
@@ -193,11 +220,17 @@
       gPw[(int64_t)(o0 + j) * Cin + c] = (red[0][threadIdx.x] + red[1][threadIdx.x]) + (red[2][threadIdx.x] + red[3][threadIdx.x]);
   }
 }
-
-__global__ void __launch_bounds__(256)
-gbias_t1_kernel(const float* __restrict__ gm8, const float* __restrict__ V, float* __restrict__ T1,
-                int Cin, int R, int H, int W) {
-  const int64_t wid = ((int64_t)blockIdx.x * 256 + threadIdx.x) >> 6;
+template <int RW, int CIN>
+__global__ void __launch_bounds__(256)
+gbias_gpw_rows_kernel(const float* __restrict__ gmap, const float* __restrict__ m8, float* __restrict__ gPw, int Cin,
+                      int Co, int64_t P4) {
+  gbias_gpw_rows_body<RW, CIN>(gmap, m8, gPw, Cin, Co, P4, blockIdx.x);
+}
+
+__device__ __forceinline__ void
+gbias_t1_body(const float* __restrict__ gm8, const float* __restrict__ V, float* __restrict__ T1,
+              int Cin, int R, int H, int W, int bx) {
+  const int64_t wid = ((int64_t)bx * 256 + threadIdx.x) >> 6;
   if (wid >= (int64_t)Cin * R * H) return;
   const int h = (int)(wid % H), r = (int)((wid / H) % R), c = (int)(wid / ((int64_t)H * R));
   float acc = 0.f;
@@ -205,29 +238,39 @@
   acc = wave_sum(acc);
   if ((threadIdx.x & 63) == 0) T1[wid] = acc;
 }
-
-__global__ void __launch_bounds__(256)
-gbias_t2_kernel(const float* __restrict__ gm8, const float* __restrict__ U, float* __restrict__ T2,
+__global__ void __launch_bounds__(256)
+gbias_t1_kernel(const float* __restrict__ gm8, const float* __restrict__ V, float* __restrict__ T1,
                 int Cin, int R, int H, int W) {
+  gbias_t1_body(gm8, V, T1, Cin, R, H, W, blockIdx.x);
+}
+
+__device__ __forceinline__ void
+gbias_t2_body(const float* __restrict__ gm8, const float* __restrict__ U, float* __restrict__ T2,
+              int Cin, int R, int H, int W, int bx, int nbx) {
   const int64_t total = (int64_t)Cin * R * W;
-  for (int64_t idx = (int64_t)blockIdx.x * 256 + threadIdx.x; idx < total;
-       idx += (int64_t)gridDim.x * 256) {
+  for (int64_t idx = (int64_t)bx * 256 + threadIdx.x; idx < total;
+       idx += (int64_t)nbx * 256) {
     const int w = (int)(idx % W), r = (int)((idx / W) % R), c = (int)(idx / ((int64_t)W * R));
     float acc = 0.f;
     for (int h = 0; h < H; ++h) acc += gm8[((int64_t)c * H + h) * W + w] * U[r * H + h];
     T2[idx] = acc;
   }
 }
-
-__global__ void __launch_bounds__(256)
-gbias_finish_kernel(const float* __restrict__ T1, const float* __restrict__ T2,
-                    const float* __restrict__ A, const float* __restrict__ U,
-                    float* __restrict__ gA, float* __restrict__ gU, float* __restrict__ gV, int Cin,
-                    int R, int H, int W) {
+__global__ void __launch_bounds__(256)
+gbias_t2_kernel(const float* __restrict__ gm8, const float* __restrict__ U, float* __restrict__ T2,
+                int Cin, int R, int H, int W) {
+  gbias_t2_body(gm8, U, T2, Cin, R, H, W, blockIdx.x, gridDim.x);
+}
+
+__device__ __forceinline__ void
+gbias_finish_body(const float* __restrict__ T1, const float* __restrict__ T2,
+                  const float* __restrict__ A, const float* __restrict__ U,
+                  float* __restrict__ gA, float* __restrict__ gU, float* __restrict__ gV, int Cin,
+                  int R, int H, int W, int bx) {
   const int nA = Cin * R, nU = R * H, nV = R * W;
   const int wavesA = (nA + 3) / 4;
-  if ((int)blockIdx.x < wavesA) {
-    const int idx = blockIdx.x * 4 + (threadIdx.x >> 6), lane = threadIdx.x & 63;
+  if (bx < wavesA) {
+    const int idx = bx * 4 + (threadIdx.x >> 6), lane = threadIdx.x & 63;
     if (idx >= nA) return;
     const int c = idx / R, r = idx - c * R;
     float acc = 0.f;
@@ -236,7 +279,7 @@
     if (lane == 0) gA[idx] = acc;
     return;
   }
-  const int idx = ((int)blockIdx.x - wavesA) * 256 + threadIdx.x;
+  const int idx = (bx - wavesA) * 256 + threadIdx.x;
   if (idx < nU) {
     const int r = idx / H, h = idx - r * H;
     float acc = 0.f;
@@ -248,6 +291,13 @@
     for (int c = 0; c < Cin; ++c) acc += T2[((int64_t)c * R + r) * W + w] * A[c * R + r];
     gV[j] = acc;
   }
+}
+__global__ void __launch_bounds__(256)
+gbias_finish_kernel(const float* __restrict__ T1, const float* __restrict__ T2,
+                    const float* __restrict__ A, const float* __restrict__ U,
+                    float* __restrict__ gA, float* __restrict__ gU, float* __restrict__ gV, int Cin,
+                    int R, int H, int W) {
+  gbias_finish_body(T1, T2, A, U, gA, gU, gV, Cin, R, H, W, blockIdx.x);
 }
 
 template <bool BWD, bool O16 = false>
@@ -441,6 +491,119 @@
   }
   hipLaunchKernelGGL(gbias_gpw_kernel, dim3(Co * Cin), dim3(256), 0, st, gmap, m8, gPw, Cin, P);
 }
+bool gpw_takes_rows(int Cin, int64_t P) {
+  return GBIAS_GPW_ROWS && Cin <= 8 && P % 4 == 0 && P >= GBIAS_GPW_ROWS_MINP;
+}
+
+constexpr int GB_MAX = 64;
+enum { GK_M8, GK_M8ROWS, GK_MIX, GK_GPW4, GK_GPW2, GK_GPW, GK_GM8_8, GK_GM8_16, GK_GM8_MIX, GK_T1, GK_T2, GK_FIN, GK_COUNT };
+constexpr uint32_t GB_PLAN_MAGIC = 0x50424750u;
+struct GbPlanHeader {
+  uint32_t magic;
+  int n;
+  int64_t fwd_floats, grad_floats, ws_floats;
+  int total[GK_COUNT];
+  int pad[12];
+};
+struct GbInst {
+  const float *A, *U, *V, *Pw;
+  int Cin, Co, R, H, W, pad;
+  int64_t m8_off, map_off;
+  int64_t gA_off, gU_off, gV_off, gPw_off;
+  int64_t ws_off;
+  int64_t pad2[2];
+};
+static_assert(sizeof(GbPlanHeader) == 128 && sizeof(GbInst) == 128, "GlobalBias plan layout");
+struct GbPtrs { const float* p[GB_MAX]; };
+
+__device__ __forceinline__ int gb_find(const int* __restrict__ starts, int n, int vb) {
+  __shared__ int found;
+  for (int j = threadIdx.x; j < n; j += blockDim.x)
+    if (vb >= starts[j] && vb < starts[j + 1]) found = j;
+  __syncthreads();
+  return __builtin_amdgcn_readfirstlane(found);
+}
+
+template <int ROWS>
+__global__ void __launch_bounds__(256)
+gbias_m8_multi_kernel(const GbInst* __restrict__ inst, const int* __restrict__ starts, int n, float* __restrict__ out) {
+  const int i = gb_find(starts, n, blockIdx.x);
+  const GbInst g = inst[i];
+  const int local = blockIdx.x - starts[i];
+  const int nbx = (g.W + 63) / 64, nby = (g.H + ROWS - 1) / ROWS;
+  const int bx = local % nbx, t = local / nbx, by = t % nby, bz = t / nby;
+  float* dst = out + (g.Pw ? g.m8_off : g.map_off);
+  if constexpr (ROWS == 1) gbias_m8_body(g.A, g.U, g.V, dst, g.Cin, g.R, g.H, g.W, bx, by, bz);
+  else gbias_m8_rows_body<ROWS>(g.A, g.U, g.V, dst, g.Cin, g.R, g.H, g.W, bx, by, bz);
+}
+
+__global__ void __launch_bounds__(256)
+gbias_mix_multi_kernel(const GbInst* __restrict__ inst, const int* __restrict__ starts, int n, float* __restrict__ out) {
+  const int i = gb_find(starts, n, blockIdx.x);
+  const GbInst g = inst[i];
+  const int local = blockIdx.x - starts[i];
+  const int64_t P = (int64_t)g.H * g.W;
+  const int nbx = (int)((P + 255) / 256);
+  small_mix_body(g.Pw, g.Cin, 1, out + g.m8_off, out + g.map_off, g.Co, g.Cin, P, local % nbx, local / nbx);
+}
+
+template <int RW>
+__global__ void __launch_bounds__(256)
+gbias_gpw_multi_kernel(const GbInst* __restrict__ inst, const int* __restrict__ starts, int n, GbPtrs gm,
+                       const float* __restrict__ fwd, float* __restrict__ grads) {
+  const int i = gb_find(starts, n, blockIdx.x);
+  const float* gmap = gm.p[i];
+  if (!gmap) return;
+  const GbInst g = inst[i];
+  const int local = blockIdx.x - starts[i];
+  const int64_t P = (int64_t)g.H * g.W;
+  if constexpr (RW == 0) gbias_gpw_body(gmap, fwd + g.m8_off, grads + g.gPw_off, g.Cin, P, local);
+  else gbias_gpw_rows_body<RW, 8>(gmap, fwd + g.m8_off, grads + g.gPw_off, g.Cin, g.Co, P / 4, local);
+}
+
+template <int CIN>
+__global__ void __launch_bounds__(CIN ? 64 * GM8_SLICES : 256)
+gbias_gm8_multi_kernel(const GbInst* __restrict__ inst, const int* __restrict__ starts, int n, GbPtrs gm,
+                       float* __restrict__ ws) {
+  const int i = gb_find(starts, n, blockIdx.x);
+  const float* gmap = gm.p[i];
+  if (!gmap) return;
+  const GbInst g = inst[i];
+  const int local = blockIdx.x - starts[i];
+  const int64_t P = (int64_t)g.H * g.W;
+  if constexpr (CIN == 0) {
+    const int nbx = (int)((P + 255) / 256);
+    small_mix_body(g.Pw, 1, g.Cin, gmap, ws + g.ws_off, g.Cin, g.Co, P, local % nbx, local / nbx);
+  } else {
+    gbias_gm8_body<CIN>(g.Pw, gmap, ws + g.ws_off, g.Cin, g.Co, P, local);
+  }
+}
+
+template <int STAGE>
+__global__ void __launch_bounds__(256)
+gbias_adj_multi_kernel(const GbInst* __restrict__ inst, const int* __restrict__ starts, int n, GbPtrs gm,
+                       float* __restrict__ grads, float* __restrict__ ws) {
+  const int i = gb_find(starts, n, blockIdx.x);
+  const float* gmap = gm.p[i];
+  if (!gmap) return;
+  const GbInst g = inst[i];
+  const int local = blockIdx.x - starts[i];
+  float* gm8 = ws + g.ws_off;
+  float* T1 = gm8 + (int64_t)g.Cin * g.H * g.W;
+  float* T2 = T1 + (int64_t)g.Cin * g.R * g.H;
+  const float* src = g.Pw ? gm8 : gmap;
+  if constexpr (STAGE == 1) gbias_t1_body(src, g.V, T1, g.Cin, g.R, g.H, g.W, local);
+  else if constexpr (STAGE == 2) gbias_t2_body(src, g.U, T2, g.Cin, g.R, g.H, g.W, local, starts[i + 1] - starts[i]);
+  else gbias_finish_body(T1, T2, g.A, g.U, grads + g.gA_off, grads + g.gU_off, grads + g.gV_off, g.Cin, g.R, g.H, g.W, local);
+}
+
+inline const GbInst* gb_insts(const void* plan) {
+  return reinterpret_cast<const GbInst*>(static_cast<const char*>(plan) + sizeof(GbPlanHeader));
+}
+inline const int* gb_starts(const void* plan, int n, int k) {
+  return reinterpret_cast<const int*>(gb_insts(plan) + n) + (size_t)k * (n + 1);
+}
+inline int64_t gb_align(int64_t floats) { return (floats + 63) & ~(int64_t)63; }
 
 }
 
@@ -506,6 +669,150 @@
   return 0;
 }
 
+extern "C" size_t paradis_global_bias_multi_plan_bytes(int n) {
+  if (n < 1 || n > GB_MAX) return 0;
+  return (sizeof(GbPlanHeader) + (size_t)n * sizeof(GbInst) + (size_t)GK_COUNT * (n + 1) * sizeof(int) + 15) & ~(size_t)15;
+}
+
+extern "C" int paradis_global_bias_multi_plan(const paradis_gbias_desc* desc, int n, void* plan) {
+  PD_REQUIRE(desc != nullptr && plan != nullptr && n >= 1 && n <= GB_MAX,
+             "global_bias_multi_plan: bad arguments (1 .. %d instances)", GB_MAX);
+  GbPlanHeader* hd = static_cast<GbPlanHeader*>(plan);
+  GbInst* inst = const_cast<GbInst*>(gb_insts(plan));
+  int64_t fwd = 0, grad = 0, ws = 0, blocks[GK_COUNT] = {0};
+  for (int i = 0; i < n; ++i) {
+    const paradis_gbias_desc& d = desc[i];
+    PD_REQUIRE(d.Cin >= 1 && d.Co >= 1 && d.R >= 1 && d.H >= 1 && d.W >= 1, "global_bias_multi_plan: bad shape (instance %d)", i);
+    PD_REQUIRE(d.A != nullptr && d.U != nullptr && d.V != nullptr, "global_bias_multi_plan: null parameter (instance %d)", i);
+    PD_REQUIRE(d.Pw != nullptr || d.Cin == d.Co, "global_bias_multi_plan: projection required when Cin != Co (instance %d)", i);
+    PD_REQUIRE(d.H <= 65535 && d.Cin <= 65535 && d.Co <= 65535, "global_bias_multi_plan: grid too large (instance %d)", i);
+    const int64_t P = (int64_t)d.H * d.W;
+    GbInst& g = inst[i];
+    g.A = d.A; g.U = d.U; g.V = d.V; g.Pw = d.Pw;
+    g.Cin = d.Cin; g.Co = d.Co; g.R = d.R; g.H = d.H; g.W = d.W; g.pad = 0;
+    g.pad2[0] = g.pad2[1] = 0;
+    g.m8_off = -1;
+    if (d.Pw) { g.m8_off = fwd; fwd += gb_align(d.Cin * P); }
+    g.map_off = fwd; fwd += gb_align(d.Co * P);
+    g.gA_off = grad; grad += gb_align((int64_t)d.Cin * d.R);
+    g.gU_off = grad; grad += gb_align((int64_t)d.R * d.H);
+    g.gV_off = grad; grad += gb_align((int64_t)d.R * d.W);
+    g.gPw_off = -1;
+    if (d.Pw) { g.gPw_off = grad; grad += gb_align((int64_t)d.Co * d.Cin); }
+    g.ws_off = ws;
+    ws += gb_align(d.Cin * P + (int64_t)d.Cin * d.R * d.H + (int64_t)d.Cin * d.R * d.W);
+    int64_t nb[GK_COUNT] = {0};
+    const int64_t nbx = (d.W + 63) / 64;
+    if (P >= (1 << 17) && d.R <= GM8_MAXR) nb[GK_M8ROWS] = nbx * ((d.H + 7) / 8) * d.Cin;
+    else nb[GK_M8] = nbx * d.H * d.Cin;
+    if (d.Pw) {
+      nb[GK_MIX] = ((P + 255) / 256) * d.Co;
+      if (gpw_takes_rows(d.Cin, P)) {
+        if (d.Co >= 1024) nb[GK_GPW4] = (d.Co + 3) / 4;
+        else nb[GK_GPW2] = (d.Co + 1) / 2;
+      } else {
+        nb[GK_GPW] = (int64_t)d.Co * d.Cin;
+      }
+      if (d.Cin <= 8) nb[GK_GM8_8] = (P + 63) / 64;
+      else if (d.Cin <= 16) nb[GK_GM8_16] = (P + 63) / 64;
+      else nb[GK_GM8_MIX] = ((P + 255) / 256) * d.Cin;
+    }
+    nb[GK_T1] = ((int64_t)d.Cin * d.R * d.H * 64 + 255) / 256;
+    nb[GK_T2] = stream_blocks((int64_t)d.Cin * d.R * d.W);
+    nb[GK_FIN] = (d.Cin * d.R + 3) / 4 + (d.R * d.H + d.R * d.W + 255) / 256;
+    for (int k = 0; k < GK_COUNT; ++k) {
+      const_cast<int*>(gb_starts(plan, n, k))[i] = (int)blocks[k];
+      blocks[k] += nb[k];
+      PD_REQUIRE(blocks[k] < ((int64_t)1 << 30), "global_bias_multi_plan: instance list too large");
+    }
+  }
+  for (int k = 0; k < GK_COUNT; ++k) {
+    const_cast<int*>(gb_starts(plan, n, k))[n] = (int)blocks[k];
+    hd->total[k] = (int)blocks[k];
+  }
+  hd->magic = GB_PLAN_MAGIC;
+  hd->n = n;
+  hd->fwd_floats = fwd; hd->grad_floats = grad; hd->ws_floats = ws;
+  for (int& p : hd->pad) p = 0;
+  return 0;
+}
+
+extern "C" int paradis_global_bias_multi_offsets(const void* plan, int64_t* out) {
+  PD_REQUIRE(plan != nullptr && out != nullptr, "global_bias_multi_offsets: bad arguments");
+  const GbPlanHeader* hd = static_cast<const GbPlanHeader*>(plan);
+  PD_REQUIRE(hd->magic == GB_PLAN_MAGIC && hd->n >= 1 && hd->n <= GB_MAX, "global_bias_multi_offsets: not a plan");
+  const GbInst* inst = gb_insts(plan);
+  for (int i = 0; i < hd->n; ++i) {
+    const GbInst& g = inst[i];
+    const int64_t v[7] = {g.m8_off, g.map_off, g.gA_off, g.gU_off, g.gV_off, g.gPw_off, g.ws_off};
+    for (int k = 0; k < 7; ++k) out[7 * i + k] = v[k];
+  }
+  out[7 * hd->n] = hd->fwd_floats; out[7 * hd->n + 1] = hd->grad_floats; out[7 * hd->n + 2] = hd->ws_floats;
+  return 0;
+}
+
+extern "C" size_t paradis_global_bias_multi_bwd_ws_bytes(const void* plan) {
+  const GbPlanHeader* hd = static_cast<const GbPlanHeader*>(plan);
+  if (!hd || hd->magic != GB_PLAN_MAGIC) return 0;
+  return (size_t)hd->ws_floats * sizeof(float) + 256;
+}
+
+extern "C" int paradis_global_bias_multi_fwd(const void* plan_host, const void* plan_dev, float* out, void* stream) {
+  PD_REQUIRE(plan_host != nullptr && plan_dev != nullptr && out != nullptr, "global_bias_multi_fwd: bad arguments");
+  const GbPlanHeader* hd = static_cast<const GbPlanHeader*>(plan_host);
+  PD_REQUIRE(hd->magic == GB_PLAN_MAGIC && hd->n >= 1 && hd->n <= GB_MAX, "global_bias_multi_fwd: not a plan");
+  PD_REQUIRE(aligned16(out), "global_bias_multi_fwd: buffer not 16-byte aligned");
+  hipStream_t st = (hipStream_t)stream;
+  const int n = hd->n;
+  const GbInst* inst = gb_insts(plan_dev);
+  if (hd->total[GK_M8])
+    hipLaunchKernelGGL(gbias_m8_multi_kernel<1>, dim3(hd->total[GK_M8]), dim3(256), 0, st, inst, gb_starts(plan_dev, n, GK_M8), n, out);
+  if (hd->total[GK_M8ROWS])
+    hipLaunchKernelGGL(gbias_m8_multi_kernel<8>, dim3(hd->total[GK_M8ROWS]), dim3(256), 0, st, inst,
+                       gb_starts(plan_dev, n, GK_M8ROWS), n, out);
+  if (hd->total[GK_MIX])
+    hipLaunchKernelGGL(gbias_mix_multi_kernel, dim3(hd->total[GK_MIX]), dim3(256), 0, st, inst, gb_starts(plan_dev, n, GK_MIX), n, out);
+  PD_CHECK_LAUNCH("global_bias_multi_fwd");
+  return 0;
+}
+
+extern "C" int paradis_global_bias_multi_bwd(const void* plan_host, const void* plan_dev, const float* const* gmaps,
+                                             const float* fwd, float* grads, void* workspace, void* stream) {
+  PD_REQUIRE(plan_host != nullptr && plan_dev != nullptr && gmaps != nullptr && fwd != nullptr && grads != nullptr &&
+                 workspace != nullptr,
+             "global_bias_multi_bwd: bad arguments");
+  const GbPlanHeader* hd = static_cast<const GbPlanHeader*>(plan_host);
+  PD_REQUIRE(hd->magic == GB_PLAN_MAGIC && hd->n >= 1 && hd->n <= GB_MAX, "global_bias_multi_bwd: not a plan");
+  PD_REQUIRE(aligned16(fwd) && aligned16(grads) && aligned16(workspace), "global_bias_multi_bwd: buffers not 16-byte aligned");
+  const int n = hd->n;
+  GbPtrs gm;
+  bool any = false;
+  for (int i = 0; i < GB_MAX; ++i) {
+    gm.p[i] = i < n ? gmaps[i] : nullptr;
+    PD_REQUIRE(aligned16(gm.p[i]), "global_bias_multi_bwd: map gradient %d not 16-byte aligned", i);
+    any = any || gm.p[i] != nullptr;
+  }
+  if (!any) return 0;
+  hipStream_t st = (hipStream_t)stream;
+  const GbInst* inst = gb_insts(plan_dev);
+  float* ws = static_cast<float*>(workspace);
+#define GB_LAUNCH(kernel, k, threads, ...)                                                                            \
+  if (hd->total[k])                                                                                                   \
+    hipLaunchKernelGGL(kernel, dim3(hd->total[k]), dim3(threads), 0, st, inst, gb_starts(plan_dev, n, k), n, gm, __VA_ARGS__)
+  GB_LAUNCH(gbias_gpw_multi_kernel<4>, GK_GPW4, 256, fwd, grads);
+  GB_LAUNCH(gbias_gpw_multi_kernel<2>, GK_GPW2, 256, fwd, grads);
+  GB_LAUNCH(gbias_gpw_multi_kernel<0>, GK_GPW, 256, fwd, grads);
+  GB_LAUNCH(gbias_gm8_multi_kernel<8>, GK_GM8_8, 64 * GM8_SLICES, ws);
+  GB_LAUNCH(gbias_gm8_multi_kernel<16>, GK_GM8_16, 64 * GM8_SLICES, ws);
+  GB_LAUNCH(gbias_gm8_multi_kernel<0>, GK_GM8_MIX, 256, ws);
+  GB_LAUNCH(gbias_adj_multi_kernel<1>, GK_T1, 256, grads, ws);
+  GB_LAUNCH(gbias_adj_multi_kernel<2>, GK_T2, 256, grads, ws);
+  GB_LAUNCH(gbias_adj_multi_kernel<3>, GK_FIN, 256, grads, ws);
+#undef GB_LAUNCH
+  PD_CHECK_LAUNCH("global_bias_multi_bwd");
+  return 0;
+}
+
 extern "C" int paradis_act_fwd(const float* x, float* y, int64_t n, int act, void* stream) {
   PD_REQUIRE(n >= 0 && act >= 0 && act <= 2, "act_fwd: bad arguments");
   if (n == 0) return 0;
diff --git a/paradis_model_amd/model/blocks.py b/paradis_model_amd/model/blocks.py
--- a/paradis_model_amd/model/blocks.py
+++ b/paradis_model_amd/model/blocks.py
@@ -116,13 +116,23 @@
                            if input_dim != output_dim else None)
 
     def bias_terms(self):
+        if self.fuses_projection():
+            m8 = None if torch.compiler.is_compiling() else ops.step_batch_map(self, True)
+            if m8 is None:
+                m8 = ops.global_bias_m8(self.A, self.U, self.V)
+            return None, (m8, self.projection.weight)
+        return self.bias_map(), None
+
+    def fuses_projection(self) -> bool:
         big = self.U.shape[1] * self.V.shape[1] >= FUSE_BIAS_PROJECTION_MIN_POINTS
-        if (FUSE_BIAS_PROJECTION and big and self.projection is not None and self.input_dim <= 16
-                and self.output_dim % 4 == 0):
-            return None, (ops.global_bias_m8(self.A, self.U, self.V), self.projection.weight)
-        return self.bias_map(), None
+        return bool(FUSE_BIAS_PROJECTION and big and self.projection is not None and self.input_dim <= 16
+                    and self.output_dim % 4 == 0)
 
     def bias_map(self) -> torch.Tensor:
+        if not torch.compiler.is_compiling():
+            bmap = ops.step_batch_map(self, False)
+            if bmap is not None:
+                return bmap
         pw = self.projection.weight if self.projection is not None else None
         return ops.global_bias_map(self.A, self.U, self.V, pw)
 
diff --git a/paradis_model_amd/model/paradis.py b/paradis_model_amd/model/paradis.py
--- a/paradis_model_amd/model/paradis.py
+++ b/paradis_model_amd/model/paradis.py
@@ -4,7 +4,7 @@
 
 from .. import ops
 from .advection import NeuralSemiLagrangian
-from .blocks import GMBlock, PhysicalDownsample, SepConv
+from .blocks import CLinear, GlobalBias, GMBlock, PhysicalDownsample, SepConv
 from .padding import GeoCyclicPadding
 
 EARTH_ROTATION_RATE = 7.29212e-5
@@ -68,6 +68,7 @@
         self.num_common_features, self.n_inputs = datamodule.num_common_features, cfg.dataset.n_time_inputs
         self.n_static = len(cfg.features.input.constants)
 
+        self._modules_compiled = False
         self.gradient_checkpoint = bool(cfg.compute.get("gradient_checkpointing", False))
         self.step_fn = self._checkpointed_step if self.gradient_checkpoint else self._layer_step
 
@@ -110,6 +111,7 @@
         return checkpoint(self._layer_step, i, h, hs, use_reentrant=False)
 
     def _compile(self):
+        self._modules_compiled = True
         self._layer_step = torch.compile(self._layer_step)
         self.static_encoder = torch.compile(self.static_encoder)
         self.input_proj = torch.compile(self.input_proj)
@@ -135,7 +137,34 @@
         hidden = self.reaction[i](hidden, residual=hidden, x_extra=hidden_static)
         return hidden
 
+    def _step_batch_lists(self):
+        lists = self.__dict__.get("_step_lists")
+        if lists is None:
+            weights, seen, gbias = [], set(), []
+            for m in self.modules():
+                w = m.conv.weight if isinstance(m, CLinear) else (m.pointwise.weight if isinstance(m, SepConv) else None)
+                if w is not None and id(w) not in seen:
+                    seen.add(id(w))
+                    weights.append(w)
+                if isinstance(m, GlobalBias):
+                    gbias.append(m)
+            lists = self.__dict__["_step_lists"] = (weights, gbias, {})
+        return lists
+
     def forward(self, fields):
+        if torch.compiler.is_compiling() or not ops.STEP_BATCH or self._modules_compiled or not fields.is_cuda:
+            return self._forward(fields)
+        weights, gbias, cache = self._step_batch_lists()
+        maps = [] if (self.gradient_checkpoint and torch.is_grad_enabled()) else [
+            (m, m.A, m.U, m.V, m.projection.weight if m.projection is not None else None, m.fuses_projection())
+            for m in gbias]
+        token = ops.step_batch_begin(cache, weights, maps)
+        try:
+            return self._forward(fields)
+        finally:
+            ops.step_batch_end(token)
+
+    def _forward(self, fields):
         hidden = self._apply_checkpoint(self.input_proj, fields)
         hidden_static = self._apply_checkpoint(self.static_encoder, fields[:, -self.n_static:])
 
diff --git a/paradis_model_amd/ops.py b/paradis_model_amd/ops.py
--- a/paradis_model_amd/ops.py
+++ b/paradis_model_amd/ops.py
@@ -1,5 +1,6 @@
 from __future__ import annotations
 
+import ctypes
 import os
 import threading
 import weakref
@@ -1034,6 +1035,11 @@
 
 def _split_image(weight: Tensor, Co: int, Ci: int, transpose: bool, scheme: int, want_wt: bool = False):
     if not FROZEN_WEIGHTS:
+        st = getattr(_TLS, "step", None)
+        if st is not None and not transpose:
+            ent = st.images.get((weight.data_ptr(), Co, Ci, scheme))
+            if ent is not None and (not want_wt or ent[1] is not None):
+                return ent[0], (ent[1] if want_wt else None)
         return _build_images(weight, Co, Ci, transpose, scheme, want_wt)
     key = (id(weight), transpose, scheme)
     ver = _version_of(weight)
@@ -1459,6 +1465,197 @@
     return (y, z) if defer_act_grad else y
 
 
+STEP_BATCH = os.environ.get("PARADIS_STEP_BATCH", "1") != "0"
+GBIAS_MULTI_MAX = 64
+
+
+class _GbiasDesc(ctypes.Structure):
+    _fields_ = [("A", ctypes.c_void_p), ("U", ctypes.c_void_p), ("V", ctypes.c_void_p), ("Pw", ctypes.c_void_p),
+                ("Cin", ctypes.c_int), ("Co", ctypes.c_int), ("R", ctypes.c_int), ("H", ctypes.c_int), ("W", ctypes.c_int)]
+
+
+def _sub(buf: Tensor, offset: int, shape) -> Tensor:
+    return torch.empty(0, dtype=buf.dtype, device=buf.device).set_(buf.untyped_storage(), offset, tuple(shape))
+
+
+def _device_table(host, device) -> Tensor:
+    return torch.frombuffer(bytearray(host.raw), dtype=torch.uint8).to(device)
+
+
+class _ImagePlan:
+
+    def __init__(self, weights, scheme: int, with_t: bool):
+        n = len(weights)
+        self.key = self.key_of(weights, scheme, with_t)
+        self.shapes = [(w.shape[0], w.numel() // w.shape[0]) for w in weights]
+        W = (ctypes.c_void_p * n)(*[w.data_ptr() for w in weights])
+        M = (ctypes.c_int * n)(*[co for co, _ in self.shapes])
+        K = (ctypes.c_int * n)(*[ci for _, ci in self.shapes])
+        self.host = ctypes.create_string_buffer(lib.paradis_pw_gemm_split_multi_plan_bytes(n))
+        offs = (ctypes.c_size_t * (2 * n))()
+        total = ctypes.c_size_t(0)
+        check(lib.paradis_pw_gemm_split_multi_plan(W, M, K, n, scheme, 1 if with_t else 0, self.host, offs,
+                                                   ctypes.byref(total)), "pw_gemm_split_multi_plan")
+        self.scheme, self.with_t, self.nbytes = scheme, with_t, int(total.value)
+        self.offsets = [(int(offs[2 * i]), int(offs[2 * i + 1]) if with_t else None) for i in range(n)]
+        self.sizes = [(lib.paradis_pw_gemm_split_bytes(co, ci, scheme), lib.paradis_pw_gemm_split_bytes(ci, co, scheme))
+                      for co, ci in self.shapes]
+        self.ptrs = [w.data_ptr() for w in weights]
+        self.dev = _device_table(self.host, weights[0].device)
+
+    @staticmethod
+    def key_of(weights, scheme, with_t):
+        return (scheme, with_t, tuple((w.data_ptr(), tuple(w.shape)) for w in weights))
+
+    def run(self) -> dict:
+        buf = torch.empty(self.nbytes, dtype=torch.uint8, device=self.dev.device)
+        check(lib.paradis_pw_gemm_split_weights_multi(self.host, dptr(self.dev), dptr(buf), stream_ptr()),
+              "pw_gemm_split_weights_multi")
+        out = {}
+        for ptr, (co, ci), (off, off_t), (nb, nb_t) in zip(self.ptrs, self.shapes, self.offsets, self.sizes):
+            out[(ptr, co, ci, self.scheme)] = (buf[off:off + nb], buf[off_t:off_t + nb_t] if off_t is not None else None)
+        return out
+
+
+class _GbiasPlan:
+
+    def __init__(self, insts):
+        n = len(insts)
+        self.key = self.key_of(insts)
+        desc = (_GbiasDesc * n)()
+        self.shapes = []
+        for d, (A, U, V, Pw) in zip(desc, insts):
+            d.A, d.U, d.V, d.Pw = A.data_ptr(), U.data_ptr(), V.data_ptr(), (Pw.data_ptr() if Pw is not None else None)
+            d.Cin, d.R, d.H, d.W = A.shape[0], A.shape[1], U.shape[1], V.shape[1]
+            d.Co = Pw.shape[0] if Pw is not None else d.Cin
+            self.shapes.append((d.Cin, d.Co, d.R, d.H, d.W, Pw is not None))
+        self.n = n
+        self.host = ctypes.create_string_buffer(lib.paradis_global_bias_multi_plan_bytes(n))
+        check(lib.paradis_global_bias_multi_plan(desc, n, self.host), "global_bias_multi_plan")
+        offs = (ctypes.c_int64 * (7 * n + 3))()
+        check(lib.paradis_global_bias_multi_offsets(self.host, offs), "global_bias_multi_offsets")
+        self.offs = [tuple(int(offs[7 * i + k]) for k in range(7)) for i in range(n)]
+        self.fwd_floats, self.grad_floats = int(offs[7 * n]), int(offs[7 * n + 1])
+        self.ws_floats = (lib.paradis_global_bias_multi_bwd_ws_bytes(self.host) + 3) // 4
+        self.dev = _device_table(self.host, insts[0][0].device)
+
+    @staticmethod
+    def key_of(insts):
+        return tuple((t.data_ptr(), tuple(t.shape)) if t is not None else None for inst in insts for t in inst)
+
+    def forward(self):
+        buf = torch.empty(self.fwd_floats, dtype=torch.float32, device=self.dev.device)
+        check(lib.paradis_global_bias_multi_fwd(self.host, dptr(self.dev), dptr(buf), stream_ptr()), "global_bias_multi_fwd")
+        return [_sub(buf, o[1], (co, h, w)) for o, (_, co, _, h, w, _) in zip(self.offs, self.shapes)], buf
+
+    def backward(self, buf: Tensor, gmaps):
+        n = self.n
+        gm = (ctypes.c_void_p * n)()
+        keep = []
+        for i, g in enumerate(gmaps):
+            if g is None:
+                continue
+            g = g.contiguous() if g.dtype == torch.float32 else g.float().contiguous()
+            if g.data_ptr() % 16:
+                g = g.clone()
+            keep.append(g)
+            gm[i] = g.data_ptr()
+        out = []
+        if not keep:
+            for *_, proj in self.shapes:
+                out += [None] * (4 if proj else 3)
+            return out
+        grads = torch.empty(self.grad_floats, dtype=torch.float32, device=buf.device)
+        ws = torch.empty(self.ws_floats, dtype=torch.float32, device=buf.device)
+        check(lib.paradis_global_bias_multi_bwd(self.host, dptr(self.dev), gm, dptr(buf), dptr(grads), dptr(ws),
+                                                stream_ptr()), "global_bias_multi_bwd")
+        for g, o, (cin, co, r, h, w, proj) in zip(gmaps, self.offs, self.shapes):
+            if g is None:
+                out += [None] * (4 if proj else 3)
+                continue
+            out += [_sub(grads, o[2], (cin, r)), _sub(grads, o[3], (r, h)), _sub(grads, o[4], (r, w))]
+            if proj:
+                out.append(_sub(grads, o[5], (co, cin)))
+        return out
+
+
+class _GlobalBiasMulti(torch.autograd.Function):
+
+    @staticmethod
+    def forward(ctx, plan, *params):
+        maps, buf = plan.forward()
+        ctx.plan, ctx.buf = plan, buf
+        ctx.set_materialize_grads(False)
+        return tuple(maps)
+
+    @staticmethod
+    def backward(ctx, *gmaps):
+        return (None, *ctx.plan.backward(ctx.buf, gmaps))
+
+
+class _StepBatch:
+    __slots__ = ("images", "maps", "prev")
+
+    def __init__(self):
+        self.images, self.maps, self.prev = {}, {}, None
+
+
+def _plan_for(cache: dict, slot, cls, key, *args):
+    plan = cache.get(slot)
+    if plan is not None and plan.key == key:
+        return plan
+    if torch.cuda.is_current_stream_capturing():
+        return None
+    plan = cache[slot] = cls(*args)
+    return plan
+
+
+def step_batch_begin(cache: dict, weights, gbias) -> Optional[_StepBatch]:
+    if not STEP_BATCH or not _all_plain(()):
+        return None
+    st = _StepBatch()
+    scheme = autocast_scheme(GEMM_SCHEME)
+    ok = lambda t: t.is_cuda and t.dtype == torch.float32 and t.is_contiguous()
+    if weights and scheme in _PAIRED_SCHEMES and not FROZEN_WEIGHTS and all(ok(w) for w in weights):
+        with_t = torch.is_grad_enabled()
+        plan = _plan_for(cache, ("images", scheme, with_t), _ImagePlan, _ImagePlan.key_of(weights, scheme, with_t),
+                         weights, scheme, with_t)
+        if plan is not None:
+            st.images = plan.run()
+    if gbias and all(ok(t) for _, *ts, _f in gbias for t in ts if t is not None):
+        for c0 in range(0, len(gbias), GBIAS_MULTI_MAX):
+            chunk = gbias[c0:c0 + GBIAS_MULTI_MAX]
+            insts = [(A, U, V, None if fused else Pw) for _, A, U, V, Pw, fused in chunk]
+            plan = _plan_for(cache, ("gbias", c0), _GbiasPlan, _GbiasPlan.key_of(insts), insts)
+            if plan is None:
+                continue
+            params = [t for inst in insts for t in inst if t is not None]
+            if torch.is_grad_enabled() and any(t.requires_grad for t in params):
+                maps = _GlobalBiasMulti.apply(plan, *params)
+            else:
+                maps = plan.forward()[0]
+            for (mod, *_, fused), m in zip(chunk, maps):
+                st.maps[id(mod)] = (m, fused)
+    if not st.images and not st.maps:
+        return None
+    st.prev = getattr(_TLS, "step", None)
+    _TLS.step = st
+    return st
+
+
+def step_batch_end(st: Optional[_StepBatch]) -> None:
+    if st is not None:
+        _TLS.step = st.prev
+
+
+def step_batch_map(module, fused: bool) -> Optional[Tensor]:
+    st = getattr(_TLS, "step", None)
+    if st is None:
+        return None
+    ent = st.maps.get(id(module))
+    return ent[0] if (ent is not None and ent[1] == fused) else None
+
+
 @_define("activation(Tensor x, int act) -> Tensor")
 def _activation(x, act):
     _f32(x)
```

New measurement: 214.2 samples/s, median of 6. Within noise of the previous version (+0.8%).
